# vnminin/phylomap

Measured on AMD Instinct MI355X. Metric: stochastic-map realisations/sec (branches x sites sampled/s), higher is better.
Workload: dtype f64; 1 GPU; C3: sumstatMCMC_bigtree sweep, 4-state Q, 10000-tip synthetic tree, Omega*mean(t_b)=4; n_states=4, n_tips=10000, branches=19998, replicas_total=16384, max_iters_provisioned=63, parallelism=replica-sharded x1 (weak), one RCCL all-reduce of the statistics

## Files before the change

### include/phylomap_hip.h

```cpp
#ifndef PHYLOMAP_HIP_H
#define PHYLOMAP_HIP_H

#include <stdint.h>

#ifdef __cplusplus
extern "C" {
#endif

#define PHM_VERSION 300
#define PHM_MAX_DEVICES 8

typedef enum phm_status {
  PHM_OK = 0,
  PHM_ERR_BAD_INPUT = 1,
  PHM_ERR_UNSUPPORTED = 2,
  PHM_ERR_NO_DEVICE = 3,
  PHM_ERR_OOM = 4,
  PHM_ERR_ZERO_PROB = 5,
  PHM_ERR_CAPACITY = 6,
  PHM_ERR_UNIF_CAP = 7,
  PHM_ERR_STATE = 8
} phm_status;

typedef enum phm_variant {
  PHM_MCMC = 0,
  PHM_MCMC_BIGTREE = 1,
  PHM_MCMC_SPARSE = 2,
  PHM_MCMC_KS = 3
  ,
  PHM_MCMC_BF = 4
  ,
  PHM_MCMC_MT = 5
  ,
  PHM_MCMC_KSMT = 6
} phm_variant;

typedef struct phm_tree {
  int32_t n_tips;
  int32_t n_node;
  int32_t n_edge;
  const int32_t* edge;
  const double*  edge_length;
  const int32_t* states;
  const int32_t* map_off;
  const double*  maps;
  const int32_t* mapnames;
} phm_tree;

typedef struct phm_model {
  int32_t n_states;
  const double* Q;
  const double* pid;
  const double* B;
  double Omega;
  int32_t variant;
} phm_model;

typedef enum phm_mapping { PHM_MAP_AUTO = 0, PHM_MAP_REPLICAS = 1, PHM_MAP_BRANCHES = 2, PHM_MAP_TILES = 3 } phm_mapping;

typedef struct phm_options {
  uint64_t seed;
  int32_t n_replicas;
  int32_t replica_offset;
  int32_t reduce;
  int32_t tips_per_replica;
  int32_t device;
  int32_t iters_per_launch;
  double  cap_tail;
  int32_t mapping;
  int32_t storage;
  int32_t rescale_pruning;
  int32_t no_recovery;
  int32_t sparse_chains;
  int32_t n_devices;
  int32_t devices[PHM_MAX_DEVICES];
  int32_t reserved[3];
} phm_options;

typedef struct phm_debug_options {
  int32_t pruning_form;
  int32_t phase_timing;
  int32_t fail_recovery;
  int32_t branch_group;
  int32_t level_groups;
  int32_t q_timing;
  double  pade_pivot_min;
  int32_t expect_chunk;
  int32_t reserved[3];
} phm_debug_options;

typedef struct phm_info {
  int32_t n_states, n_edge, n_replicas, n_replicas_padded, n_cols, max_iters;
  int64_t device_bytes;
  int64_t rows_per_replica;
  int64_t seg_read;
  int64_t seg_written;
  double  last_run_ms;
  int32_t last_run_launches;
  int32_t iters_done;
  int32_t recoveries;
  int32_t mapping;
  int32_t sparse_chains;
  int32_t reserved;
} phm_info;

typedef struct phm_engine phm_engine;

int32_t     phm_version(void);
int32_t     phm_struct_size(int32_t which);
int32_t     phm_device_count(void);
const char* phm_last_error(void);
const char* phm_status_string(int32_t status);
int32_t     phm_set_debug_options(const phm_debug_options* dbg);
double      phm_last_kernel_ms(void);

int32_t phm_maketreelistMCMC(
    const phm_tree* x, int32_t n_states, const double* Q, const double* pid, const double* B, double Omega,
    const int32_t* nen, const int32_t* nodelist, int32_t root, int32_t N,
    const phm_options* opt, double* out);
int32_t phm_maketreelistMCMC_bigtree(
    const phm_tree* x, int32_t n_states, const double* Q, const double* pid, const double* B, double Omega,
    const int32_t* nen, const int32_t* nodelist, int32_t root, int32_t N,
    const phm_options* opt, double* out);
int32_t phm_SPARSEmaketreelistMCMC(
    const phm_tree* x, int32_t n_states, const double* Q, const double* pid, const double* B, double Omega,
    const int32_t* nen, const int32_t* nodelist, int32_t root, int32_t N,
    const phm_options* opt, double* out);
int32_t phm_maketreelistMCMCks_sweep(
    const phm_tree* x, int32_t n_states, const double* Q, const double* pid, const double* B, double Omega,
    const int32_t* nen, const int32_t* nodelist, int32_t root, int32_t N,
    const phm_options* opt, double* out);
int32_t phm_maketreelistMCMCbf_sweep(
    const phm_tree* x, int32_t n_states, const double* Q, const double* pid, const double* B, double Omega,
    const int32_t* nen, const int32_t* nodelist, int32_t root, int32_t N,
    const phm_options* opt, double* out);
int32_t phm_maketreelistMCMCbf(
    const phm_tree* x, int32_t n_states, const double* Q, const double* pid, const double* B, double Omega,
    const int32_t* nen, const int32_t* nodelist, int32_t root, int32_t N, const double* prior, int32_t n_prior,
    const phm_options* opt, double* out);
int32_t phm_maketreelistMCMCks(
    const phm_tree* x, int32_t n_states, const double* Q, const double* pid, const double* B, double Omega,
    const int32_t* nen, const int32_t* nodelist, int32_t root, int32_t N, const double* prior, int32_t n_prior,
    const phm_options* opt, double* out);
int32_t phm_maketreelistMCMC2sDICt(
    const phm_tree* x, int32_t n_states, const double* Q, const double* pid, const double* B, double Omega,
    const int32_t* nen, const int32_t* nodelist, int32_t root, int32_t N, const double* prior, int32_t n_prior,
    const phm_options* opt, double* out);
int32_t phm_maketreelistMCMCksDICt(
    const phm_tree* x, int32_t n_states, const double* Q, const double* pid, const double* B, double Omega,
    const int32_t* nen, const int32_t* nodelist, int32_t root, int32_t N, const double* prior, int32_t n_prior,
    const phm_options* opt, double* out);
int32_t phm_maketreelistMCMCmt(
    const phm_tree* trees, int32_t n_trees, int32_t n_states, const double* Q, const double* pid, const double* B,
    double Omega, const int32_t* nen_m, const int32_t* nodelist_m, const int32_t* roots, int32_t N, const double* prior,
    int32_t n_prior, const phm_options* opt, double* out);
int32_t phm_maketreelistMCMCksmt(
    const phm_tree* trees, int32_t n_trees, int32_t n_states, const double* Q, const double* pid, const double* B,
    double Omega, const int32_t* nen_m, const int32_t* nodelist_m, const int32_t* roots, int32_t N, const double* prior,
    int32_t n_prior, const phm_options* opt, double* out);
int32_t phm_maketreelistEXP(
    const phm_tree* x, int32_t n_states, const double* Q, const double* pid,
    const int32_t* nen, const int32_t* nodelist, int32_t root, int32_t N,
    const double* lefts, const double* rights, const double* d,
    const phm_options* opt, double* out);

int32_t phm_simulate_histories(const phm_tree* x, int32_t n_states, const double* Q, const double* pid,
                               const int32_t* observe, const phm_options* opt,
                               int32_t* tips, int32_t* nodes, double* stats);

int32_t phm_simulate_histories_maps(const phm_tree* x, int32_t n_states, const double* Q, const double* pid,
                                    const int32_t* observe, const phm_options* opt,
                                    int32_t* tips, int32_t* nodes, double* stats,
                                    int64_t* map_off, int64_t map_cap, double* map_dwell, int32_t* map_state);
int32_t phm_maketreelistEXP_maps(const phm_tree* x, int32_t n, const double* Q, const double* pid, const int32_t* nen,
                                 const int32_t* nodelist, int32_t root, int32_t N, const double* lefts, const double* rights,
                                 const double* d, const phm_options* opt, double* out,
                                 int64_t* map_off, int64_t map_cap, double* map_dwell, int32_t* map_state);

int32_t phm_maketreelistMCMC_maps(int32_t variant, const phm_tree* x, int32_t n_states, const double* Q, const double* pid,
                                  const double* B, double Omega, const int32_t* nen, const int32_t* nodelist, int32_t root, int32_t N,
                                  const int32_t* map_iters, int32_t n_map_iters, const phm_options* opt, double* out,
                                  int64_t* map_off, int64_t map_cap, double* map_dwell, int32_t* map_state);

int32_t phm_expected_stats(const phm_tree* x, int32_t n_states, const double* Q, const double* pid,
                           const int32_t* observe, const phm_options* opt,
                           double* stats, double* loglik, double* branch_stats, double* node_post);

int32_t phm_expected_through_time(const phm_tree* x, int32_t n_states, const double* Q, const double* pid,
                                  const int32_t* observe, const phm_options* opt,
                                  int32_t n_bounds, const double* bounds,
                                  double* occupancy,
                                  double* bin_stats,
                                  int64_t n_points, const int32_t* point_edge, const double* point_pos,
                                  double* point_post,
                                  double* loglik);

int32_t phm_loglik_models(const phm_tree* x, int32_t n_states, int32_t n_models, const double* Q, const double* pid, int32_t n_pid,
                          const int32_t* observe, const int32_t* site_of_model, const phm_options* opt, double* out);

int32_t phm_expected_stats_models(const phm_tree* x, int32_t n_states, int32_t n_models, const double* Q, const double* pid,
                                  int32_t n_pid, const int32_t* observe, const int32_t* site_of_model, const phm_options* opt,
                                  double* stats, double* loglik);

int32_t phm_sample_histories_models(const phm_tree* x, int32_t n_states, int32_t n_models, const double* Q, const double* pid,
                                    int32_t n_pid, const int32_t* observe, const int32_t* site_of_model, int32_t draws,
                                    const phm_options* opt, double* stats, double* loglik, int32_t* nodes,
                                    int64_t* map_off, int64_t map_cap, double* map_dwell, int32_t* map_state);

int32_t phm_ancestral_models(const phm_tree* x, int32_t n_states, int32_t n_models, const double* Q, const double* pid,
                             int32_t n_pid, const int32_t* observe, const int32_t* site_of_model,
                             const int32_t* node_sel, int32_t n_sel, const phm_options* opt,
                             double* loglik, double* node_post, int32_t* joint_states, double* joint_logp);

int32_t phm_simulate_histories_models(const phm_tree* x, int32_t n_states, int32_t n_models, const double* Q, const double* pid,
                                      int32_t n_pid, const int32_t* observe, int32_t replicates, const phm_options* opt,
                                      int32_t* tips, int32_t* nodes, double* stats,
                                      int64_t* map_off, int64_t map_cap, double* map_dwell, int32_t* map_state);

int32_t phm_gibbs_rates(const phm_tree* x, int32_t n_states, const int32_t* index, int32_t n_params, int32_t n_chains,
                        const double* theta0, const double* prior, int32_t n_prior, double theta_max, const double* pid,
                        int32_t n_pid, const int32_t* observe, const int32_t* site_of_chain, int32_t iters, int32_t thin,
                        const phm_options* opt, double* theta, double* loglik, double* stats, int32_t* rejected,
                        int32_t* chain_status);

int32_t phm_qupdate_apply(int32_t variant, int32_t n_states, double* Q, double Omega, const double* prior, int32_t n_prior,
                          const double* row, uint64_t seed, uint32_t iter);

int32_t phm_sparse_kernel_source(int32_t n_states, const double* M, char* buf, int32_t cap);

int32_t phm_tree_orders(int32_t n_tips, int32_t n_edge, const int32_t* edge, int32_t* nen, int32_t* nodelist,
                        int32_t* root);

int32_t phm_expm_eigen(int32_t n_states, const double* lefts, const double* rights, const double* d,
                       const double* t, int32_t n_t, int32_t device, double* out, double* kernel_ms);
int32_t phm_expm_eigen_mfma(int32_t n_states, const double* lefts, const double* rights, const double* d,
                            const double* t, int32_t n_t, int32_t device, double* out, double* kernel_ms);
int32_t phm_expm_pade(int32_t n_states, const double* Q, const double* t, int32_t n_t, int32_t device,
                      double* out, double* kernel_ms);

int32_t phm_expm_pade_mfma(int32_t n_states, const double* Q, const double* t, int32_t n_t, int32_t device,
                           double* out, double* kernel_ms);

int32_t phm_engine_create(const phm_tree* x, const phm_model* model, const phm_options* opt,
                          int32_t max_iters, phm_engine** out);
int32_t phm_engine_create_multi(const phm_tree* trees, int32_t n_trees, const phm_model* model, const phm_options* opt,
                                int32_t max_iters, phm_engine** out);
int32_t phm_engine_run(phm_engine* e, int32_t n_iters, void* hip_stream);
int32_t phm_engine_sync(phm_engine* e);
int32_t phm_engine_read_stats(phm_engine* e, int32_t iter0, int32_t n, double* out);
int32_t phm_engine_reduced_stats_device(phm_engine* e, int32_t iter0, int32_t n, void* hip_stream, void** out_dev);
int32_t phm_engine_time_pruning(phm_engine* e, int32_t n_iters, void* hip_stream, double* ms_out);
int32_t phm_engine_set_model(phm_engine* e, const double* Q);
int32_t phm_engine_dump(phm_engine* e, int32_t replica, int32_t* seg_count, double* seg_dwell, int32_t seg_cap,
                        int32_t* node_states, double* PL);
int32_t phm_engine_info(phm_engine* e, phm_info* info);
int32_t phm_engine_phase_ms(phm_engine* e, double* out4);
void    phm_engine_destroy(phm_engine* e);

#ifdef __cplusplus
}
#endif
#endif
```

### phylomap_amd/_lib.py

```python
from __future__ import annotations

import ctypes as C
import os

import numpy as np

_HERE = os.path.dirname(os.path.abspath(__file__))
LIB_PATH = os.environ.get("PHM_LIB", os.path.join(_HERE, "libphylomap_hip.so"))

PHM_OK = 0
STATUS = {0: "PHM_OK", 1: "PHM_ERR_BAD_INPUT", 2: "PHM_ERR_UNSUPPORTED", 3: "PHM_ERR_NO_DEVICE", 4: "PHM_ERR_OOM",
          5: "PHM_ERR_ZERO_PROB", 6: "PHM_ERR_CAPACITY", 7: "PHM_ERR_UNIF_CAP", 8: "PHM_ERR_STATE"}
PHM_MCMC, PHM_MCMC_BIGTREE, PHM_MCMC_SPARSE, PHM_MCMC_KS, PHM_MCMC_BF, PHM_MCMC_MT, PHM_MCMC_KSMT = 0, 1, 2, 3, 4, 5, 6

EXPORTS = [
    "phm_version", "phm_struct_size", "phm_device_count", "phm_last_error", "phm_status_string",
    "phm_maketreelistMCMC", "phm_maketreelistMCMC_bigtree", "phm_SPARSEmaketreelistMCMC", "phm_maketreelistEXP",
    "phm_maketreelistMCMCks_sweep", "phm_maketreelistMCMCbf_sweep", "phm_maketreelistMCMCbf", "phm_maketreelistMCMCks", "phm_maketreelistMCMC2sDICt", "phm_maketreelistMCMCksDICt", "phm_engine_set_model", "phm_qupdate_apply",
    "phm_expm_eigen", "phm_expm_eigen_mfma", "phm_expm_pade", "phm_expm_pade_mfma",
    "phm_engine_create", "phm_engine_run", "phm_engine_sync", "phm_engine_read_stats", "phm_engine_dump",
    "phm_engine_info", "phm_engine_destroy", "phm_engine_reduced_stats_device",
    "phm_engine_time_pruning", "phm_tree_orders",
    "phm_engine_create_multi", "phm_maketreelistMCMCmt", "phm_maketreelistMCMCksmt", "phm_engine_phase_ms",
    "phm_last_kernel_ms", "phm_set_debug_options", "phm_sparse_kernel_source", "phm_simulate_histories",
    "phm_expected_stats", "phm_simulate_histories_maps", "phm_maketreelistEXP_maps", "phm_maketreelistMCMC_maps",
    "phm_expected_through_time", "phm_loglik_models", "phm_expected_stats_models", "phm_sample_histories_models",
    "phm_gibbs_rates", "phm_ancestral_models", "phm_simulate_histories_models",
]


class PhmError(RuntimeError):
    def __init__(self, status, message):
        super().__init__(f"{STATUS.get(status, status)}: {message}")
        self.status = status


class Tree(C.Structure):
    _fields_ = [("n_tips", C.c_int32), ("n_node", C.c_int32), ("n_edge", C.c_int32),
                ("edge", C.POINTER(C.c_int32)), ("edge_length", C.POINTER(C.c_double)),
                ("states", C.POINTER(C.c_int32)), ("map_off", C.POINTER(C.c_int32)),
                ("maps", C.POINTER(C.c_double)), ("mapnames", C.POINTER(C.c_int32))]


class Model(C.Structure):
    _fields_ = [("n_states", C.c_int32), ("Q", C.POINTER(C.c_double)), ("pid", C.POINTER(C.c_double)),
                ("B", C.POINTER(C.c_double)), ("Omega", C.c_double), ("variant", C.c_int32)]


PHM_MAX_DEVICES = 8


class Options(C.Structure):
    _fields_ = [("seed", C.c_uint64), ("n_replicas", C.c_int32), ("replica_offset", C.c_int32),
                ("reduce", C.c_int32), ("tips_per_replica", C.c_int32), ("device", C.c_int32),
                ("iters_per_launch", C.c_int32), ("cap_tail", C.c_double), ("mapping", C.c_int32), ("storage", C.c_int32),
                ("rescale_pruning", C.c_int32), ("no_recovery", C.c_int32), ("sparse_chains", C.c_int32),
                ("n_devices", C.c_int32), ("devices", C.c_int32 * PHM_MAX_DEVICES), ("reserved", C.c_int32 * 3)]


class DebugOptions(C.Structure):
    _fields_ = [("pruning_form", C.c_int32), ("phase_timing", C.c_int32), ("fail_recovery", C.c_int32),
                ("branch_group", C.c_int32), ("level_groups", C.c_int32), ("q_timing", C.c_int32),
                ("pade_pivot_min", C.c_double), ("expect_chunk", C.c_int32), ("reserved", C.c_int32 * 3)]


class Info(C.Structure):
    _fields_ = [("n_states", C.c_int32), ("n_edge", C.c_int32), ("n_replicas", C.c_int32),
                ("n_replicas_padded", C.c_int32), ("n_cols", C.c_int32), ("max_iters", C.c_int32),
                ("device_bytes", C.c_int64), ("rows_per_replica", C.c_int64), ("seg_read", C.c_int64),
                ("seg_written", C.c_int64), ("last_run_ms", C.c_double), ("last_run_launches", C.c_int32),
                ("iters_done", C.c_int32), ("recoveries", C.c_int32), ("mapping", C.c_int32), ("sparse_chains", C.c_int32),
                ("reserved", C.c_int32)]


def _p(a, t):
    return a.ctypes.data_as(C.POINTER(t)) if a is not None else None


_lib = None


def load():
    global _lib
    if _lib is None:
        if not os.path.exists(LIB_PATH):
            raise RuntimeError(f"{LIB_PATH} is missing: run `python -c 'import __graft_entry__ as g; g.build()'` "
                               "or `make`; phylomap_amd has no CPU fallback")
        L = C.CDLL(LIB_PATH)
        L.phm_last_error.restype = C.c_char_p
        L.phm_status_string.restype = C.c_char_p
        L.phm_status_string.argtypes = [C.c_int32]
        L.phm_last_kernel_ms.restype = C.c_double
        L.phm_engine_create.argtypes = [C.POINTER(Tree), C.POINTER(Model), C.POINTER(Options), C.c_int32,
                                        C.POINTER(C.c_void_p)]
        L.phm_engine_create_multi.argtypes = [C.POINTER(Tree), C.c_int32, C.POINTER(Model), C.POINTER(Options), C.c_int32,
                                              C.POINTER(C.c_void_p)]
        L.phm_engine_run.argtypes = [C.c_void_p, C.c_int32, C.c_void_p]
        L.phm_engine_sync.argtypes = [C.c_void_p]
        L.phm_engine_read_stats.argtypes = [C.c_void_p, C.c_int32, C.c_int32, C.POINTER(C.c_double)]
        L.phm_engine_dump.argtypes = [C.c_void_p, C.c_int32, C.POINTER(C.c_int32), C.POINTER(C.c_double), C.c_int32,
                                      C.POINTER(C.c_int32), C.POINTER(C.c_double)]
        L.phm_engine_info.argtypes = [C.c_void_p, C.POINTER(Info)]
        L.phm_tree_orders.argtypes = [C.c_int32, C.c_int32, C.POINTER(C.c_int32), C.POINTER(C.c_int32),
                                      C.POINTER(C.c_int32), C.POINTER(C.c_int32)]
        L.phm_engine_time_pruning.argtypes = [C.c_void_p, C.c_int32, C.c_void_p, C.POINTER(C.c_double)]
        L.phm_engine_reduced_stats_device.argtypes = [C.c_void_p, C.c_int32, C.c_int32, C.c_void_p,
                                                      C.POINTER(C.c_void_p)]
        L.phm_engine_phase_ms.argtypes = [C.c_void_p, C.POINTER(C.c_double)]
        L.phm_engine_destroy.argtypes = [C.c_void_p]
        L.phm_engine_destroy.restype = None
        mc = [C.POINTER(Tree), C.c_int32, C.POINTER(C.c_double), C.POINTER(C.c_double), C.POINTER(C.c_double),
              C.c_double, C.POINTER(C.c_int32), C.POINTER(C.c_int32), C.c_int32, C.c_int32, C.POINTER(Options),
              C.POINTER(C.c_double)]
        L.phm_maketreelistMCMC.argtypes = mc
        L.phm_maketreelistMCMC_bigtree.argtypes = mc
        L.phm_SPARSEmaketreelistMCMC.argtypes = mc
        L.phm_maketreelistMCMCks_sweep.argtypes = mc
        L.phm_maketreelistMCMCbf_sweep.argtypes = mc
        mcq = mc[:10] + [C.POINTER(C.c_double), C.c_int32] + mc[10:]
        L.phm_maketreelistMCMCbf.argtypes = mcq
        L.phm_maketreelistMCMCks.argtypes = mcq
        L.phm_maketreelistMCMC2sDICt.argtypes = mcq
        L.phm_maketreelistMCMCksDICt.argtypes = mcq
        mt = [C.POINTER(Tree), C.c_int32, C.c_int32, C.POINTER(C.c_double), C.POINTER(C.c_double), C.POINTER(C.c_double),
              C.c_double, C.POINTER(C.c_int32), C.POINTER(C.c_int32), C.POINTER(C.c_int32), C.c_int32,
              C.POINTER(C.c_double), C.c_int32, C.POINTER(Options), C.POINTER(C.c_double)]
        L.phm_maketreelistMCMCmt.argtypes = mt
        L.phm_maketreelistMCMCksmt.argtypes = mt
        L.phm_engine_set_model.argtypes = [C.c_void_p, C.POINTER(C.c_double)]
        L.phm_qupdate_apply.argtypes = [C.c_int32, C.c_int32, C.POINTER(C.c_double), C.c_double, C.POINTER(C.c_double),
                                        C.c_int32, C.POINTER(C.c_double), C.c_uint64, C.c_uint32]
        L.phm_maketreelistEXP.argtypes = [C.POINTER(Tree), C.c_int32, C.POINTER(C.c_double), C.POINTER(C.c_double),
                                          C.POINTER(C.c_int32), C.POINTER(C.c_int32), C.c_int32, C.c_int32,
                                          C.POINTER(C.c_double), C.POINTER(C.c_double), C.POINTER(C.c_double),
                                          C.POINTER(Options), C.POINTER(C.c_double)]
        L.phm_expm_eigen.argtypes = [C.c_int32, C.POINTER(C.c_double), C.POINTER(C.c_double), C.POINTER(C.c_double),
                                     C.POINTER(C.c_double), C.c_int32, C.c_int32, C.POINTER(C.c_double),
                                     C.POINTER(C.c_double)]
        L.phm_expm_eigen_mfma.argtypes = L.phm_expm_eigen.argtypes
        L.phm_expm_pade_mfma.argtypes = [C.c_int32, C.POINTER(C.c_double), C.POINTER(C.c_double), C.c_int32, C.c_int32,
                                         C.POINTER(C.c_double), C.POINTER(C.c_double)]
        L.phm_expm_pade.argtypes = [C.c_int32, C.POINTER(C.c_double), C.POINTER(C.c_double), C.c_int32, C.c_int32,
                                    C.POINTER(C.c_double), C.POINTER(C.c_double)]
        L.phm_set_debug_options.argtypes = [C.POINTER(DebugOptions)]
        L.phm_simulate_histories.argtypes = [C.POINTER(Tree), C.c_int32, C.POINTER(C.c_double), C.POINTER(C.c_double),
                                             C.POINTER(C.c_int32), C.POINTER(Options), C.POINTER(C.c_int32),
                                             C.POINTER(C.c_int32), C.POINTER(C.c_double)]
        L.phm_simulate_histories_maps.argtypes = L.phm_simulate_histories.argtypes + [
            C.POINTER(C.c_int64), C.c_int64, C.POINTER(C.c_double), C.POINTER(C.c_int32)]
        L.phm_maketreelistEXP_maps.argtypes = L.phm_maketreelistEXP.argtypes + [
            C.POINTER(C.c_int64), C.c_int64, C.POINTER(C.c_double), C.POINTER(C.c_int32)]
        L.phm_maketreelistMCMC_maps.argtypes = [C.c_int32] + mc[:10] + [C.POINTER(C.c_int32), C.c_int32] + mc[10:] + [
            C.POINTER(C.c_int64), C.c_int64, C.POINTER(C.c_double), C.POINTER(C.c_int32)]
        L.phm_expected_stats.argtypes = [C.POINTER(Tree), C.c_int32, C.POINTER(C.c_double), C.POINTER(C.c_double),
                                         C.POINTER(C.c_int32), C.POINTER(Options), C.POINTER(C.c_double),
                                         C.POINTER(C.c_double), C.POINTER(C.c_double), C.POINTER(C.c_double)]
        L.phm_expected_through_time.argtypes = [C.POINTER(Tree), C.c_int32, C.POINTER(C.c_double), C.POINTER(C.c_double),
                                                C.POINTER(C.c_int32), C.POINTER(Options), C.c_int32, C.POINTER(C.c_double),
                                                C.POINTER(C.c_double), C.POINTER(C.c_double), C.c_int64, C.POINTER(C.c_int32),
                                                C.POINTER(C.c_double), C.POINTER(C.c_double), C.POINTER(C.c_double)]
        L.phm_loglik_models.argtypes = [C.POINTER(Tree), C.c_int32, C.c_int32, C.POINTER(C.c_double), C.POINTER(C.c_double),
                                        C.c_int32, C.POINTER(C.c_int32), C.POINTER(C.c_int32), C.POINTER(Options),
                                        C.POINTER(C.c_double)]
        L.phm_expected_stats_models.argtypes = [C.POINTER(Tree), C.c_int32, C.c_int32, C.POINTER(C.c_double),
                                                C.POINTER(C.c_double), C.c_int32, C.POINTER(C.c_int32), C.POINTER(C.c_int32),
                                                C.POINTER(Options), C.POINTER(C.c_double), C.POINTER(C.c_double)]
        L.phm_sample_histories_models.argtypes = [C.POINTER(Tree), C.c_int32, C.c_int32, C.POINTER(C.c_double),
                                                  C.POINTER(C.c_double), C.c_int32, C.POINTER(C.c_int32), C.POINTER(C.c_int32),
                                                  C.c_int32, C.POINTER(Options), C.POINTER(C.c_double), C.POINTER(C.c_double),
                                                  C.POINTER(C.c_int32), C.POINTER(C.c_int64), C.c_int64, C.POINTER(C.c_double),
                                                  C.POINTER(C.c_int32)]
        L.phm_gibbs_rates.argtypes = [C.POINTER(Tree), C.c_int32, C.POINTER(C.c_int32), C.c_int32, C.c_int32,
                                      C.POINTER(C.c_double), C.POINTER(C.c_double), C.c_int32, C.c_double, C.POINTER(C.c_double),
                                      C.c_int32, C.POINTER(C.c_int32), C.POINTER(C.c_int32), C.c_int32, C.c_int32,
                                      C.POINTER(Options), C.POINTER(C.c_double), C.POINTER(C.c_double), C.POINTER(C.c_double),
                                      C.POINTER(C.c_int32), C.POINTER(C.c_int32)]
        L.phm_ancestral_models.argtypes = [C.POINTER(Tree), C.c_int32, C.c_int32, C.POINTER(C.c_double), C.POINTER(C.c_double),
                                           C.c_int32, C.POINTER(C.c_int32), C.POINTER(C.c_int32), C.POINTER(C.c_int32), C.c_int32,
                                           C.POINTER(Options), C.POINTER(C.c_double), C.POINTER(C.c_double),
                                           C.POINTER(C.c_int32), C.POINTER(C.c_double)]
        L.phm_simulate_histories_models.argtypes = [C.POINTER(Tree), C.c_int32, C.c_int32, C.POINTER(C.c_double),
                                                    C.POINTER(C.c_double), C.c_int32, C.POINTER(C.c_int32), C.c_int32,
                                                    C.POINTER(Options), C.POINTER(C.c_int32), C.POINTER(C.c_int32),
                                                    C.POINTER(C.c_double), C.POINTER(C.c_int64), C.c_int64,
                                                    C.POINTER(C.c_double), C.POINTER(C.c_int32)]
        L.phm_sparse_kernel_source.argtypes = [C.c_int32, C.POINTER(C.c_double), C.c_char_p, C.c_int32]
        for which, mirror in enumerate((Options, Info, Tree, Model, DebugOptions)):
            if L.phm_struct_size(which) != C.sizeof(mirror):
                raise RuntimeError(f"{LIB_PATH}: {mirror.__name__} is {L.phm_struct_size(which)} bytes in the library, "
                                   f"{C.sizeof(mirror)} in phylomap_amd/_lib.py (stale build? run make)")
        _lib = L
    return _lib


def check(status):
    if status != PHM_OK:
        raise PhmError(status, load().phm_last_error().decode())


class FlatTree:

    def __init__(self, z, states=None):
        edge = np.asarray(z["edge"], dtype=np.int32)
        if edge.ndim != 2 or edge.shape[1] != 2:
            raise ValueError("z['edge'] must be E x 2")
        self.E = edge.shape[0]
        st = z["states"] if states is None else states
        self.states = np.ascontiguousarray(np.asarray(st).round(), dtype=np.int32)
        self.T = int(np.asarray(z["states"]).shape[-1])
        self.edge = np.asfortranarray(edge).reshape(-1, order="F").copy()
        el = z.get("edge.length")
        self.edge_length = None if el is None else np.ascontiguousarray(el, dtype=np.float64)
        lens = [len(m) for m in z["maps"]]
        self.map_off = np.concatenate([[0], np.cumsum(lens)]).astype(np.int32)
        self.maps = np.ascontiguousarray(np.concatenate([np.asarray(m, dtype=np.float64) for m in z["maps"]]))
        self.mapnames = np.ascontiguousarray(np.concatenate([np.asarray(m) for m in z["mapnames"]]), dtype=np.int32)
        self.c = Tree(self.T, int(z["Nnode"]), self.E, _p(self.edge, C.c_int32), _p(self.edge_length, C.c_double),
                      _p(self.states.reshape(-1), C.c_int32), _p(self.map_off, C.c_int32), _p(self.maps, C.c_double),
                      _p(self.mapnames, C.c_int32))


class FlatTreeList:

    def __init__(self, treelist):
        if len(treelist) < 1:
            raise ValueError("treelist is empty")
        self.trees = [FlatTree(z) for z in treelist]
        self.n = len(self.trees)
        self.c = (Tree * self.n)(*[t.c for t in self.trees])
        self.E, self.T = self.trees[0].E, self.trees[0].T


def tree_orders(z):
    edge = np.asarray(z["edge"], dtype=np.int32)
    E = edge.shape[0]
    flat = np.asfortranarray(edge).reshape(-1, order="F").copy()
    T = int(z["Nnode"]) + 1
    nen = np.zeros(E, dtype=np.int32)
    nodelist = np.zeros(max(int(z["Nnode"]) - 1, 1), dtype=np.int32)
    root = C.c_int32(0)
    check(load().phm_tree_orders(T, E, _p(flat, C.c_int32), _p(nen, C.c_int32), _p(nodelist, C.c_int32), C.byref(root)))
    return nen, nodelist[: int(z["Nnode"]) - 1], int(root.value)


def sparse_kernel_source(M):
    Mf = np.asfortranarray(np.asarray(M, dtype=np.float64))
    L = load()
    need = L.phm_sparse_kernel_source(Mf.shape[0], _p(Mf, C.c_double), None, 0)
    if need < 0:
        check(1)
    buf = C.create_string_buffer(need)
    L.phm_sparse_kernel_source(Mf.shape[0], _p(Mf, C.c_double), buf, need)
    return buf.value.decode()


MAPPING = {"auto": 0, "replicas": 1, "branches": 2, "tiles": 3}


def set_debug_options(**kw):
    d = DebugOptions()
    for k, v in kw.items():
        setattr(d, k, float(v) if k == "pade_pivot_min" else int(v))
    check(load().phm_set_debug_options(C.byref(d)))


_DEBUG_KEYS = ("pruning_form", "phase_timing", "fail_recovery", "branch_group", "level_groups", "q_timing", "pade_pivot_min",
               "expect_chunk")


def make_options(seed=0, n_replicas=1, replica_offset=0, reduce=False, tips_per_replica=False, device=-1,
                 iters_per_launch=0, cap_tail=0.0, storage=0, mapping="auto", rescale=False, recover=True,
                 sparse_chains=0, devices=None, **debug):
    unknown = set(debug) - set(_DEBUG_KEYS)
    if unknown:
        raise TypeError(f"unknown option(s) {sorted(unknown)}")
    set_debug_options(**debug)
    o = Options()
    o.seed = int(seed) & 0xFFFFFFFFFFFFFFFF
    o.n_replicas, o.replica_offset, o.reduce = int(n_replicas), int(replica_offset), int(bool(reduce))
    o.storage = int(storage)
    o.mapping = MAPPING[mapping] if isinstance(mapping, str) else int(mapping)
    o.rescale_pruning = int(bool(rescale))
    o.no_recovery = 0 if recover else 1
    o.sparse_chains = int(sparse_chains)
    o.tips_per_replica, o.device, o.iters_per_launch, o.cap_tail = int(bool(tips_per_replica)), int(device), int(iters_per_launch), float(cap_tail)
    if devices is not None:
        devs = list(range(int(devices))) if np.isscalar(devices) else [int(d) for d in devices]
        if len(devs) > PHM_MAX_DEVICES:
            raise ValueError(f"at most {PHM_MAX_DEVICES} devices")
        o.n_devices = len(devs)
        for i, d in enumerate(devs):
            o.devices[i] = d
    return o


class Engine:

    def __init__(self, z, Q, pid, Omega, max_iters, variant=PHM_MCMC, B=None, states=None, **opt):
        L = load()
        self.Q = np.asfortranarray(np.asarray(Q, dtype=np.float64))
        self.n = self.Q.shape[0]
        self.pid = np.ascontiguousarray(pid, dtype=np.float64)
        self.B = None if B is None else np.asfortranarray(np.asarray(B, dtype=np.float64))
        self.opt = make_options(**opt)
        self.model = Model(self.n, _p(self.Q, C.c_double), _p(self.pid, C.c_double), _p(self.B, C.c_double),
                           float(Omega), int(variant))
        self.h = C.c_void_p()
        n_trees = 1
        if isinstance(z, (list, tuple)):
            if states is not None:
                raise ValueError("a list of trees carries its own tip states")
            self.ft = FlatTreeList(z)
            n_trees = self.ft.n
            check(L.phm_engine_create_multi(self.ft.c, n_trees, C.byref(self.model), C.byref(self.opt), int(max_iters),
                                            C.byref(self.h)))
        else:
            self.ft = FlatTree(z, states)
            check(L.phm_engine_create(C.byref(self.ft.c), C.byref(self.model), C.byref(self.opt), int(max_iters),
                                      C.byref(self.h)))
        self.cols = self.n + self.n * (self.n - 1)
        if int(variant) in (PHM_MCMC_KS, PHM_MCMC_KSMT):
            self.cols = self.n + self.n * self.n + 2 + 3 * (self.n // 2 - 1) + 1
        if int(variant) in (PHM_MCMC_BF, PHM_MCMC_MT):
            self.cols = self.n + self.n * self.n + 3
        self.S = max(1, int(self.opt.n_replicas)) * n_trees
        self.reduce = bool(self.opt.reduce)

    def run(self, n_iters, stream=None):
        check(load().phm_engine_run(self.h, int(n_iters), C.c_void_p(stream) if stream else None))

    def set_model(self, Q):
        Qc = np.asfortranarray(np.asarray(Q, dtype=np.float64))
        check(load().phm_engine_set_model(self.h, _p(Qc, C.c_double)))

    def sync(self):
        check(load().phm_engine_sync(self.h))

    def info(self):
        i = Info()
        check(load().phm_engine_info(self.h, C.byref(i)))
        return i

    def stats(self, iter0, n):
        if self.reduce:
            out = np.zeros((n, self.cols), order="F")
            check(load().phm_engine_read_stats(self.h, int(iter0), int(n), _p(out, C.c_double)))
            return out
        buf = np.zeros((self.S, self.cols, n))
        check(load().phm_engine_read_stats(self.h, int(iter0), int(n), _p(buf, C.c_double)))
        return buf.transpose(0, 2, 1)

    def reduced_stats_device(self, iter0, n, stream=None):
        ptr = C.c_void_p()
        check(load().phm_engine_reduced_stats_device(self.h, int(iter0), int(n), C.c_void_p(stream) if stream else None,
                                                     C.byref(ptr)))
        return ptr.value

    def phase_ms(self):
        out = (C.c_double * 4)()
        check(load().phm_engine_phase_ms(self.h, out))
        return [float(v) for v in out]

    def time_pruning(self, n_iters, stream=None):
        ms = C.c_double(0.0)
        check(load().phm_engine_time_pruning(self.h, int(n_iters), C.c_void_p(stream) if stream else None, C.byref(ms)))
        return ms.value

    def dump(self, replica=0, seg_cap=512):
        E, T, n = self.ft.E, self.ft.T, self.n
        seg_count = np.zeros(E, dtype=np.int32)
        seg_dwell = np.zeros((E, seg_cap))
        node_states = np.zeros(2 * T - 1, dtype=np.int32)
        PL = np.zeros((2 * T - 1, n))
        check(load().phm_engine_dump(self.h, int(replica), _p(seg_count, C.c_int32), _p(seg_dwell, C.c_double),
                                     int(seg_cap), _p(node_states, C.c_int32), _p(PL, C.c_double)))
        return {"seg_count": seg_count, "seg_dwell": seg_dwell, "node_states": node_states, "PL": PL}

    def close(self):
        if self.h:
            load().phm_engine_destroy(self.h)
            self.h = C.c_void_p()

    def __del__(self):
        try:
            self.close()
        except Exception:
            pass
```

### phylomap_amd/csrc/phm_engine.cpp

```cpp
#include "phm_internal.h"

namespace {

int tree_levels(const phm::Schedule& s) {
  std::vector<int32_t> depth(s.n_node, 0);
  int levels = 1;
  for (const phm::DownStep& d : s.down)
    if (d.child >= 0) { depth[d.child] = depth[d.parent] + 1; levels = std::max(levels, depth[d.child] + 1); }
  return levels;
}
bool deep_tree(const phm::Schedule& s) {
  int lg2 = 0;
  while ((1 << lg2) < s.n_node + 1) ++lg2;
  return tree_levels(s) > 4 * lg2 + 32;
}

inline int narrow_auto_max_replicas(const phm::Schedule& s) {
  const int levels = tree_levels(s);
  const double E = (double)s.n_edge;
  const double cap = (0.0048 * levels + 6e-6 * E - 0.01) / (6.5e-7 * E);
  return (int)std::max(8.0, std::min(4096.0, cap));
}
constexpr int TILES_AUTO_MAX_REPLICAS = 262144;
inline int wbranch_auto_max_replicas(const phm::Schedule& s) {
// ... 223 lines not shown
        for (int t = 0; t < nt; ++t) th.emplace_back(rows_of, (int)((int64_t)ktab * t / nt), (int)((int64_t)ktab * (t + 1) / nt));
        for (std::thread& t : th) t.join();
      }
      HIPCHK(hipMemcpy(e->d_wt_totL.p, blk.data(), sizeof(double) * blk.size(), hipMemcpyHostToDevice));
    }
    {
      const bool ks = ks_layout(e->variant);
      std::vector<int16_t> pair_slot((size_t)n * n, (int16_t)-1);
      std::vector<int32_t> slot_col;
      for (int a = 0; a < n; ++a)
        for (int c = 0; c < n; ++c)
          if ((ks || a != c) && e->hB2[(size_t)a * n + c] != 0.0) {
            pair_slot[(size_t)a * n + c] = (int16_t)slot_col.size();
            slot_col.push_back(ks ? a * n + c : a * (n - 1) + (c > a ? c - 1 : c));
          }
      int n_slots = (int)slot_col.size();
      if (n > 32 || n_slots > phm::WT_MAX_SLOTS) { n_slots = 0; std::fill(pair_slot.begin(), pair_slot.end(), (int16_t)-1); }
      slot_col.resize(phm::WT_MAX_SLOTS, 0);
      e->pwt.n_slots = n_slots;
      HIPCHK(hipMemcpy(e->d_wt_pair_slot.p, pair_slot.data(), sizeof(int16_t) * pair_slot.size(), hipMemcpyHostToDevice));
      HIPCHK(hipMemcpy(e->d_wt_slot_col.p, slot_col.data(), sizeof(int32_t) * slot_col.size(), hipMemcpyHostToDevice));
    }
    HIPCHK(hipMemcpy(e->d_Bc.p, e->hBc.data(), sizeof(double) * n * n, hipMemcpyHostToDevice));
    HIPCHK(hipMemcpy(e->d_scale.p, e->hscale.data(), sizeof(double) * n, hipMemcpyHostToDevice));
    {
      auto half_bandwidth = [&](const std::vector<double>& M) {
        int hb = 0;
        for (int i = 0; i < n; ++i)
          for (int j = 0; j < n; ++j) if (M[(size_t)i * n + j] != 0.0) hb = std::max(hb, std::abs(i - j));
        return hb;
      };
      auto usable = [&](int hb) { return e->sparse_req != 2 && n <= phm::WT_BAND_NMAX && hb >= 1 && hb <= phm::WT_BAND_MAX && 2 * hb + 1 < n; };
      const int hbc = half_bandwidth(e->hBc), hb2 = half_bandwidth(e->hB2);
      e->pwt.band_up = usable(hbc) ? hbc : 0;
      e->pwt.band_draw = usable(hb2) ? hb2 : 0;
      e->wt_sparse.kernel = nullptr;
      if (!e->pwt.band_up && e->sparse_req != 2 && n <= phm::RTC_SPARSE_NMAX) {
        std::vector<int32_t> rp(1, 0), cj;
        std::vector<double> cv;
        for (int i = 0; i < n; ++i) {
          for (int j = 0; j < n; ++j) if (e->hBc[(size_t)i * n + j] != 0.0) { cj.push_back(j); cv.push_back(e->hBc[(size_t)i * n + j]); }
          rp.push_back((int32_t)cj.size());
        }
        if ((double)cj.size() <= phm::RTC_SPARSE_MAX_FILL * n * n) {
          std::string rerr;
          const phm::SparseUpKernel* k = phm::rtc_sparse_up_kernel(n, rp, cj, rerr);
          if (!k && e->sparse_req == 1) return fail(PHM_ERR_UNSUPPORTED, "sparse_chains = 1: " + rerr);
          if (k) {
            if (!e->d_wt_coef.p) HIPCHK(e->d_wt_coef.alloc(sizeof(double) * (size_t)n * n));
            HIPCHK(hipMemcpy(e->d_wt_coef.p, cv.data(), sizeof(double) * cv.size(), hipMemcpyHostToDevice));
            phm::RtcUpParams& r = e->wt_sparse.params;
            const phm::WtParams& w = e->pwt;
            r.n_states = n; r.ldt = w.ldt; r.n_tips = w.n_tips; r.n_node = w.n_node; r.n_edge = w.n_edge; r.n_tiles = w.n_tiles;
            r.normalise = w.normalise; r.tips_per_replica = w.tips_per_replica; r.tip_masks = w.tip_masks; r.klong = w.klong;
            r.up = reinterpret_cast<const phm::RtcUpStep*>(w.up); r.up_order = w.up_order; r.colL = w.colL; r.maskL = w.maskL; r.tips = w.tips;
            r.mcount = w.mcount; r.PL = w.PL; r.err = w.err; r.coef = e->d_wt_coef.as<double>();
            e->wt_sparse.kernel = k;
          }
        }
      }
      if (e->sparse_req == 1 && !e->pwt.band_up && !e->wt_sparse.kernel)
        return fail(PHM_ERR_UNSUPPORTED, "sparse_chains = 1: the sparse pruning kernels take n <= 32 states and a chain matrix that is banded (half-bandwidth <= 2) or at most half full");
      std::memset(&e->wt_band, 0, sizeof e->wt_band);
      if (e->pwt.band_up) {
        const int hb = e->pwt.band_up, w = 2 * hb + 1;
        for (int i = 0; i < n; ++i)
          for (int d = 0; d < w; ++d) { const int j = i + d - hb; if (j >= 0 && j < n) e->wt_band.c[i * w + d] = e->hBc[(size_t)i * n + j]; }
      }
      std::vector<double> b2band((size_t)n * (2 * phm::WT_BAND_MAX + 1), 0.0);
      if (e->pwt.band_draw) {
        const int hb = e->pwt.band_draw, w = 2 * hb + 1;
        for (int i = 0; i < n; ++i)
          for (int d = 0; d < w; ++d) { const int j = i + d - hb; if (j >= 0 && j < n) b2band[(size_t)i * w + d] = e->hB2[(size_t)i * n + j]; }
      }
      HIPCHK(hipMemcpy(e->d_wt_B2band.p, b2band.data(), sizeof(double) * b2band.size(), hipMemcpyHostToDevice));
    }
    return PHM_OK;
  }
  if (replicas) {
    HIPCHK(hipMemcpy(e->d_col.p, col.data(), sizeof(double) * col.size(), hipMemcpyHostToDevice));
    HIPCHK(hipMemcpy(e->d_row.p, row.data(), sizeof(double) * row.size(), hipMemcpyHostToDevice));
    HIPCHK(hipMemcpy(e->d_mask.p, maskpow.data(), sizeof(double) * maskpow.size(), hipMemcpyHostToDevice));
  } else {
    const size_t nc = col.size(), nr = row.size(), nm = maskpow.size();
    HIPCHK(e->pin_up.reserve(sizeof(double) * (nc + nr + nm)));
    double* stage = e->pin_up.as<double>();
    std::memcpy(stage, col.data(), sizeof(double) * nc);
    std::memcpy(stage + nc, row.data(), sizeof(double) * nr);
    std::memcpy(stage + nc + nr, maskpow.data(), sizeof(double) * nm);
    if (e->mapping == PHM_MAP_BRANCHES && !e->wide()) {
      HIPCHK(hipMemcpyAsync(e->d_nw_colL.p, stage, sizeof(double) * (nc + nr + nm), hipMemcpyHostToDevice, e->last_stream));
    } else {
      HIPCHK(hipMemcpyAsync(e->d_nw_colL.p, stage, sizeof(double) * nc, hipMemcpyHostToDevice, e->last_stream));
      HIPCHK(hipMemcpyAsync(e->d_nw_rowL.p, stage + nc, sizeof(double) * nr, hipMemcpyHostToDevice, e->last_stream));
      HIPCHK(hipMemcpyAsync(e->d_nw_maskL.p, stage + nc + nr, sizeof(double) * nm, hipMemcpyHostToDevice, e->last_stream));
    }
    HIPCHK(wait_stream(e->last_stream));
  }
  if (e->wide()) {
    HIPCHK(hipMemcpy(e->d_B2.p, e->hB2.data(), sizeof(double) * n * n, hipMemcpyHostToDevice));
    HIPCHK(hipMemcpy(e->d_Bc.p, e->hBc.data(), sizeof(double) * n * n, hipMemcpyHostToDevice));
    HIPCHK(hipMemcpy(e->d_scale.p, e->hscale.data(), sizeof(double) * n, hipMemcpyHostToDevice));
  }
  if (e->wide() && !replicas) {
    auto ellpack = [&](const std::vector<double>& M, DevBuf& dcol, DevBuf& dval, int32_t& w_out) -> int32_t {
      int w = 0;
      for (int i = 0; i < n; ++i) {
        int cnt = 0;
        for (int j = 0; j < n; ++j) cnt += M[(size_t)i * n + j] != 0.0;
        w = std::max(w, cnt);
      }
      w_out = (w >= 1 && w <= phm::WB_ELL_MAX && 3 * w <= n) ? w : 0;
      if (!w_out) return PHM_OK;
      std::vector<int32_t> ec((size_t)n * w);
      std::vector<double> ev((size_t)n * w, 0.0);
      for (int i = 0; i < n; ++i) {
        int t = 0;
        for (int j = 0; j < n; ++j) if (M[(size_t)i * n + j] != 0.0) { ec[(size_t)i * w + t] = j; ev[(size_t)i * w + t] = M[(size_t)i * n + j]; ++t; }
        for (; t < w; ++t) ec[(size_t)i * w + t] = i;
      }
      HIPCHK(hipMemcpy(dcol.p, ec.data(), sizeof(int32_t) * ec.size(), hipMemcpyHostToDevice));
      HIPCHK(hipMemcpy(dval.p, ev.data(), sizeof(double) * ev.size(), hipMemcpyHostToDevice));
      return PHM_OK;
    };
    { int32_t st = ellpack(e->hBc, e->d_ell_col, e->d_ell_val, e->pwb.ell_w); if (st) return st; }
    {
      int hb = 0;
      for (int i = 0; i < n; ++i)
        for (int j = 0; j < n; ++j) if (e->hBc[(size_t)i * n + j] != 0.0) hb = std::max(hb, std::abs(i - j));
      e->pwb.band_hb = (e->pwb.ell_w > 0 && hb >= 1 && hb <= 2 && e->sparse_req != 2) ? hb : 0;
    }
    { int32_t st = ellpack(e->hB2, e->d_ell2_col, e->d_ell2_val, e->pwb.ell2_w); if (st) return st; }
  }
  auto refresh = [&](auto& p) {
    for (int i = 0; i < n * n; ++i) { p.B2[i] = e->hB2[i]; p.Bc[i] = e->hBc[i]; }
    for (int i = 0; i < n; ++i) { p.scale[i] = e->hscale[i]; p.pid[i] = e->hpid[i]; }
  };
  small_n(e, [&](auto& sp) { refresh(sp.rep); refresh(sp.br); refresh(sp.tl); });
  return PHM_OK;
}

template <int NS>
void fill_narrow_params(phm_engine* e, phm::NarrowParams<NS>& p, const phm_options& o) {
  fill_common(e, o, p);
  p.klong = e->nw_klong; p.n_wide = e->nw_n_wide; p.cluster_async = e->nw_cluster_async;
  p.total_cap = e->nw_total_cap;
  p.cl_nodes = e->d_nw_cl_nodes.as<phm::ClusterNode>(); p.cl_item_off = e->d_nw_cl_item_off.as<int32_t>();
  p.cl_lvl_ptr = e->d_nw_cl_lvl_ptr.as<int32_t>(); p.cl_lvl_off = e->d_nw_cl_lvl_off.as<int32_t>();
  p.down_lv = e->d_nw_down_lv.as<phm::DownStep>(); p.walk_off = e->d_nw_walk_off.as<int32_t>();
  p.edge_parent = e->d_nw_edge_parent.as<int32_t>(); p.dmap_edge = e->d_nw_dmap_edge.as<uint16_t>();
  p.branch_order = e->d_nw_border.as<int32_t>(); p.off = e->d_nw_off.as<int64_t>();
  {
    const size_t tab = (size_t)e->nw_klong * NS * NS;
    p.colL = e->d_nw_colL.as<double>(); p.rowL = p.colL + tab; p.maskL = p.colL + 2 * tab;
  }
  p.tips = e->d_tips.as<uint8_t>();
  p.mcount = e->d_nw_mcount.as<int32_t>(); p.dw[0] = e->d_nw_dwA.as<double>(); p.dw[1] = e->d_nw_dwB.as<double>();
  p.PL = e->d_PL.as<double>(); p.nstate = e->d_nstate.as<uint8_t>(); p.part = e->d_nw_part.as<double>();
  p.rowbuf = e->d_nw_rowbuf.as<double>();
  p.dmap = e->d_nw_dmap.as<uint16_t>();
  p.host_row = nullptr;
  if (e->S == 1 && !e->reduce && e->pin_row.reserve(sizeof(double) * (e->dcols + 2)) == hipSuccess) {
    void* dp = nullptr;
    if (hipHostGetDevicePointer(&dp, e->pin_row.p, 0) == hipSuccess) p.host_row = reinterpret_cast<double*>(dp);
  }
}

int32_t build_level_orders(phm_engine* e) {
  const phm::Schedule& s = e->sched;
  const int E = s.n_edge;
  std::vector<int32_t> up_order, down_order, node_order;
  phm::height_levels(s.up, up_order, e->nw_up_off);
  phm::depth_levels(s, down_order, e->nw_down_off);
  phm::node_depth_levels(s, node_order, e->nw_node_off);
  HIPCHK(upload(e->d_nw_up_order, up_order)); HIPCHK(upload(e->d_nw_down_order, down_order)); HIPCHK(upload(e->d_nw_node_order, node_order));
  if (!e->wide()) {
    std::vector<int32_t> walk;
    phm::depth_levels(s, walk, e->nw_walk_off, true);
    std::vector<phm::DownStep> walk_lv;
    walk_lv.reserve(E);
    for (int k : walk) walk_lv.push_back(s.down[k]);
    for (int k : down_order) if (s.down[k].child < 0) walk_lv.push_back(s.down[k]);
    std::vector<int32_t> edge_parent(E);
    for (int i = 0; i < E; ++i) edge_parent[s.down[i].edge] = s.down[i].parent;
    HIPCHK(upload(e->d_nw_down_lv, walk_lv));
    HIPCHK(upload(e->d_nw_walk_off, e->nw_walk_off));
    HIPCHK(upload(e->d_nw_edge_parent, edge_parent));
  }
  HIPCHK(upload(e->d_nw_up_off, e->nw_up_off)); HIPCHK(upload(e->d_nw_down_off, e->nw_down_off));
  return PHM_OK;
}

int32_t narrow_setup(phm_engine* e, const phm_tree* x, const phm_model* model, const phm_options& o, int32_t max_iters) {
  const phm::Schedule& s = e->sched;
  const int E = s.n_edge, T = s.n_tips, Nn = s.n_node, n = e->n, S = e->S;
  const SlotPlan sp = plan_slots(e, x, model->Omega, o, max_iters);
  e->nw_off = sp.off;
  int n_wide = 0;
  for (int b = 0; b < E; ++b)
    if (expected_segments(x, b, model->Omega) >= phm::NARROW_WIDE_SEGMENTS) ++n_wide;
  e->nw_n_wide = std::max(n_wide, std::min(E / 16, phm::NARROW_LONG));
  e->nw_cluster_async = e->dbg.pruning_form == 2 || (e->dbg.pruning_form == 0 && n_wide > 0);

  if (e->tips_per_replica) {
    e->tips_host.resize((size_t)S * T);
    for (int r = 0; r < S; ++r) for (int t = 0; t < T; ++t) e->tips_host[(size_t)r * T + t] = (uint8_t)(x->states[(size_t)r * T + t] - 1);
  } else {
    single_tree_tips(e, x);
  }

  const size_t dw_bytes = sizeof(double) * (size_t)S * e->nw_total_cap;
  const size_t tab = (size_t)e->nw_klong * n * n;
  size_t free_b = 0, total_b = 0;
  HIPCHK(hipMemGetInfo(&free_b, &total_b));
  const size_t part_cols = e->wide() ? (size_t)n + 1 : (size_t)n + n * n + 1;
  const size_t n_dw = e->wide() ? 3 : 2;
  const size_t dmap_bytes = e->wide() ? (((size_t)S * E * n <= (256u << 20)) ? (size_t)S * E * n : 0) : 2 * sizeof(uint16_t) * (size_t)S * E;
  const size_t small_bytes = (size_t)S * (E * (sizeof(int32_t) + 2) + (size_t)Nn * (sizeof(double) * n + 1)) + sizeof(phm::ClusterNode) * (size_t)Nn + 16 * (size_t)E;
  const size_t need = n_dw * dw_bytes + (e->wide() ? (size_t)S * e->nw_total_cap : 0) + stats_bytes(e) + dmap_bytes + small_bytes +
                      sizeof(double) * (3 * tab + (size_t)S * E * part_cols + (e->wide() ? 2 * (size_t)S * e->dcols : 0));
  if (int32_t st = check_hbm(need, free_b)) return st;
  HIPCHK(upload(e->d_up, s.up)); HIPCHK(upload(e->d_down, s.down));
  if (int32_t st = build_level_orders(e)) return st;
  HIPCHK(upload(e->d_nw_border, sp.order)); HIPCHK(upload(e->d_nw_off, e->nw_off));
  if (e->wide()) {
    HIPCHK(e->d_nw_colL.alloc(sizeof(double) * tab)); HIPCHK(e->d_nw_rowL.alloc(sizeof(double) * tab));
    HIPCHK(e->d_nw_maskL.alloc(sizeof(double) * (size_t)e->nw_klong * 2 * n));
  } else {
    HIPCHK(e->d_nw_colL.alloc(sizeof(double) * (2 * tab + (size_t)e->nw_klong * 2 * n)));
  }
  HIPCHK(upload(e->d_tips, e->tips_host));
  HIPCHK(e->d_nw_mcount.alloc(sizeof(int32_t) * (size_t)S * E));
  HIPCHK(e->d_nw_dwA.alloc(dw_bytes)); HIPCHK(e->d_nw_dwB.alloc(dw_bytes));
  if (e->wide()) {
    HIPCHK(e->d_nw_mstate.alloc((size_t)S * e->nw_total_cap));
    HIPCHK(e->d_nw_mlen.alloc(dw_bytes));
    HIPCHK(e->d_nw_estate.alloc((size_t)S * E * 2));
  }
  HIPCHK(e->d_PL.alloc(sizeof(double) * (size_t)S * Nn * n));
  HIPCHK(e->d_nstate.alloc((size_t)S * Nn));
  HIPCHK(e->d_nw_part.alloc(sizeof(double) * (size_t)S * E * part_cols));
  HIPCHK(e->d_nw_rowbuf.alloc(sizeof(double) * (size_t)S * e->dcols));
  if (!e->wide()) {
    HIPCHK(e->d_nw_dmap.alloc(sizeof(uint16_t) * (size_t)S * E));
    HIPCHK(e->d_nw_dmap_edge.alloc(sizeof(uint16_t) * (size_t)S * E));
    phm::ClusterPlan plan;
    phm::build_cluster_plan(s, phm::NARROW_CLUSTER_NODES, plan);
    if (int32_t st = upload_cluster_plan(e, plan, true)) return st;
  }
  if (int32_t st = alloc_stats(e)) return st;
  e->bytes = (int64_t)(n_dw * dw_bytes + e->d_nw_mstate.bytes + e->d_nw_part.bytes + e->d_PL.bytes + e->d_stats.bytes + e->d_red.bytes +
                       sizeof(double) * 3 * tab + e->d_nw_mcount.bytes + e->d_nw_dmap.bytes + e->d_nw_dmap_edge.bytes + e->d_nw_cl_nodes.bytes +
                       (e->wide() ? dmap_bytes : 0));
  HIPCHK(hipMemset(e->d_nstate.p, 0, e->d_nstate.bytes));
  {
    std::vector<double> init((size_t)e->nw_total_cap, 0.0);
    std::vector<int32_t> m0(E);
    for (int b = 0; b < E; ++b) {
      m0[b] = x->map_off[b + 1] - x->map_off[b];
      std::memcpy(&init[(size_t)e->nw_off[b]], x->maps + x->map_off[b], sizeof(double) * m0[b]);
    }
    for (int r = 0; r < S; ++r) {
      HIPCHK(hipMemcpy(e->d_nw_dwA.as<double>() + (size_t)r * e->nw_total_cap, init.data(), sizeof(double) * init.size(), hipMemcpyHostToDevice));
      HIPCHK(hipMemcpy(e->d_nw_mcount.as<int32_t>() + (size_t)r * E, m0.data(), sizeof(int32_t) * E, hipMemcpyHostToDevice));
    }
  }
  small_n(e, [&](auto& p) { fill_narrow_params(e, p.br, o); });
  if (e->wide()) {
    HIPCHK(e->d_wb_cnt.alloc(sizeof(double) * (size_t)S * e->dcols));
    if ((size_t)S * s.n_edge * n <= (256u << 20)) HIPCHK(e->d_nw_dmap.alloc((size_t)S * s.n_edge * n));
    HIPCHK(hipMemset(e->d_wb_cnt.p, 0, e->d_wb_cnt.bytes));
    HIPCHK(e->d_B2.alloc(sizeof(double) * n * n)); HIPCHK(e->d_Bc.alloc(sizeof(double) * n * n));
    HIPCHK(e->d_ell_col.alloc(sizeof(int32_t) * n * phm::WB_ELL_MAX)); HIPCHK(e->d_ell_val.alloc(sizeof(double) * n * phm::WB_ELL_MAX));
    HIPCHK(e->d_ell2_col.alloc(sizeof(int32_t) * n * phm::WB_ELL_MAX)); HIPCHK(e->d_ell2_val.alloc(sizeof(double) * n * phm::WB_ELL_MAX));
    HIPCHK(e->d_scale.alloc(sizeof(double) * n)); HIPCHK(upload(e->d_pid, e->hpid));
    phm::WideBranchParams& p = e->pwb;
    fill_common(e, o, p);
    p.n_states = n; p.sparse = (e->variant == PHM_MCMC_SPARSE); p.count_self = p.ks; p.klong = e->nw_klong;
    p.total_cap = e->nw_total_cap;
    p.B2 = e->d_B2.as<double>(); p.Bc = e->d_Bc.as<double>(); p.scale = e->d_scale.as<double>(); p.pid = e->d_pid.as<double>();
    p.ell_w = 0; p.band_hb = 0; p.ell_col = e->d_ell_col.as<int32_t>(); p.ell_val = e->d_ell_val.as<double>();
    p.ell2_w = 0; p.ell2_col = e->d_ell2_col.as<int32_t>(); p.ell2_val = e->d_ell2_val.as<double>();
    p.up = e->d_up.as<phm::UpStep>(); p.down = e->d_down.as<phm::DownStep>();
    p.up_order = e->d_nw_up_order.as<int32_t>(); p.down_order = e->d_nw_down_order.as<int32_t>();
    p.up_off = e->d_nw_up_off.as<int32_t>(); p.down_off = e->d_nw_down_off.as<int32_t>();
    p.branch_order = e->d_nw_border.as<int32_t>(); p.off = e->d_nw_off.as<int64_t>();
    p.colL = e->d_nw_colL.as<double>(); p.rowL = e->d_nw_rowL.as<double>(); p.maskL = e->d_nw_maskL.as<double>();
    p.tips = e->d_tips.as<uint8_t>(); p.mcount = e->d_nw_mcount.as<int32_t>();
    p.dw[0] = e->d_nw_dwA.as<double>(); p.dw[1] = e->d_nw_dwB.as<double>(); p.mlen = e->d_nw_mlen.as<double>();
    p.mstate = e->d_nw_mstate.as<uint8_t>(); p.estate = e->d_nw_estate.as<uint8_t>();
    p.PL = e->d_PL.as<double>(); p.nstate = e->d_nstate.as<uint8_t>(); p.part = e->d_nw_part.as<double>();
    p.cnt = e->d_wb_cnt.as<double>(); p.rowbuf = e->d_nw_rowbuf.as<double>();
    p.dmap = e->d_nw_dmap.as<uint8_t>();
  }
  return PHM_OK;
}

inline int tiles_cnt_copies(int tiles) {
  int c = 1;
  while (c < 64 && c * tiles < 512) c *= 2;
  return c;
}

template <int NS>
void fill_tile_params(phm_engine* e, phm::TileParams<NS>& p, const phm_options& o) {
  fill_common(e, o, p);
  p.klong = e->nw_klong;
  p.group = (int32_t)std::max<int64_t>(1, std::min<int64_t>(16, (int64_t)e->tiles * p.n_edge / 65536));
  p.n_groups = (p.n_edge + p.group - 1) / p.group;
  p.n_chunks = (p.n_groups + phm::TILES_CHUNK - 1) / phm::TILES_CHUNK;
  p.rows = e->nw_total_cap;
  p.up = e->d_up.as<phm::UpStep>();
  p.up_order = e->d_nw_up_order.as<int32_t>(); p.node_order = e->d_nw_node_order.as<int32_t>();
  p.branch_order = e->d_nw_border.as<int32_t>(); p.slot = e->d_tl_slot.as<int32_t>();
  p.cl_nodes = e->d_nw_cl_nodes.as<phm::ClusterNode>();
  p.cl_lvl_ptr = e->d_nw_cl_lvl_ptr.as<int32_t>(); p.cl_lvl_off = e->d_nw_cl_lvl_off.as<int32_t>();
  p.colL = e->d_nw_colL.as<double>(); p.rowL = e->d_nw_rowL.as<double>(); p.maskL = e->d_nw_maskL.as<double>();
  p.tips = e->d_tips.as<uint8_t>(); p.mcount = e->d_mcount.as<uint16_t>();
  p.dw[0] = e->d_dw0.as<double>(); p.dw[1] = e->d_dw1.as<double>();
  p.estate = e->d_tl_estate.as<uint8_t>(); p.PL = e->d_PL.as<double>(); p.nstate = e->d_nstate.as<uint8_t>();
  p.mstate = e->d_wt_mstate.p ? e->d_wt_mstate.as<uint8_t>() : nullptr;
  p.pdw = e->d_tl_pdw.as<double>(); p.pchunk = e->d_tl_pchunk.as<double>(); p.cnt = e->d_tl_cnt.as<uint32_t>();
  p.cnt_copies = tiles_cnt_copies(e->tiles);
  p.pseg = e->d_tl_pseg.as<uint32_t>(); p.segprev = e->d_tl_segprev.as<uint32_t>();
}

int32_t tile_slots(phm_engine* e, const SlotPlan& sp) {
  const int E = e->sched.n_edge;
  e->tl_slot.assign(E + 1, 0);
  for (int b = 0; b < E; ++b) {
    if (sp.cap[b] >= (1 << 23)) return fail(PHM_ERR_UNSUPPORTED, "branch too long: a slot of the (tile, branch) mapping exceeds 4 GB");
    if (sp.off[b + 1] > 0x7fffff00ll / 64) return fail(PHM_ERR_UNSUPPORTED, "tree too large: dwell rows per replica tile exceed 32-bit indexing");
    e->tl_slot[b + 1] = (int32_t)sp.off[b + 1];
  }
  return PHM_OK;
}

int32_t tiles_setup(phm_engine* e, const phm_tree* x, const phm_model* model, const phm_options& o, int32_t max_iters) {
  const phm::Schedule& s = e->sched;
  const int E = s.n_edge, Nn = s.n_node, n = e->n, tiles = e->tiles;
  const SlotPlan sp = plan_slots(e, x, model->Omega, o, max_iters);
  if (int32_t st = tile_slots(e, sp)) return st;
  const int64_t rows = e->rows;
  single_tree_tips(e, x);

  const int n_chunks = (E + phm::TILES_CHUNK - 1) / phm::TILES_CHUNK;
  const size_t dw_bytes = sizeof(double) * (size_t)tiles * rows * 64;
  const size_t tab = (size_t)e->nw_klong * n * n;
  const size_t pdw_bytes = sizeof(double) * (size_t)tiles * E * n * 64;
  const size_t pl_bytes = sizeof(double) * (size_t)tiles * Nn * n * 64;
#ifndef PHM_TILES_LONG_SEGMENTS
#define PHM_TILES_LONG_SEGMENTS 48.0
#endif
  const bool long_paths = sp.max_seg > PHM_TILES_LONG_SEGMENTS;
  const size_t ms_bytes = long_paths ? (size_t)tiles * rows * 64 : 0;
  size_t free_b = 0, total_b = 0;
  HIPCHK(hipMemGetInfo(&free_b, &total_b));
  const size_t need = 2 * dw_bytes + ms_bytes + pdw_bytes + pl_bytes + stats_bytes(e) + sizeof(double) * 3 * tab + (size_t)tiles * (4 * (size_t)E + Nn) * 64;
  if (int32_t st = check_hbm(need, free_b)) return st;
  HIPCHK(upload(e->d_up, s.up)); HIPCHK(upload(e->d_down, s.down));
  if (int32_t st = build_level_orders(e)) return st;
  HIPCHK(upload(e->d_nw_border, sp.order)); HIPCHK(upload(e->d_tl_slot, e->tl_slot));
  HIPCHK(e->d_nw_colL.alloc(sizeof(double) * tab)); HIPCHK(e->d_nw_rowL.alloc(sizeof(double) * tab));
  HIPCHK(e->d_nw_maskL.alloc(sizeof(double) * (size_t)e->nw_klong * 2 * n));
  HIPCHK(upload(e->d_tips, e->tips_host));
  HIPCHK(e->d_mcount.alloc(sizeof(uint16_t) * (size_t)tiles * E * 64));
  HIPCHK(e->d_dw0.alloc(dw_bytes)); HIPCHK(e->d_dw1.alloc(dw_bytes));
  if (long_paths) HIPCHK(e->d_wt_mstate.alloc(ms_bytes));
  HIPCHK(e->d_tl_estate.alloc((size_t)tiles * E * 64));
  HIPCHK(e->d_PL.alloc(pl_bytes));
  HIPCHK(e->d_nstate.alloc((size_t)tiles * Nn * 64));
  HIPCHK(e->d_tl_pdw.alloc(pdw_bytes));
  HIPCHK(e->d_tl_pchunk.alloc(sizeof(double) * (size_t)tiles * n_chunks * n * 64));
  HIPCHK(e->d_tl_cnt.alloc(sizeof(uint32_t) * (size_t)tiles * tiles_cnt_copies(tiles) * n * n * 64));
  HIPCHK(e->d_tl_pseg.alloc(sizeof(uint32_t) * (size_t)tiles * n_chunks * 64)); HIPCHK(e->d_tl_segprev.alloc(sizeof(uint32_t) * tiles));
  if (int32_t st = alloc_stats(e)) return st;
  e->bytes = (int64_t)(2 * dw_bytes + ms_bytes + pdw_bytes + pl_bytes + e->d_stats.bytes + e->d_red.bytes + e->d_mcount.bytes + e->d_tl_pchunk.bytes +
                       sizeof(double) * 3 * tab);
  HIPCHK(hipMemset(e->d_nstate.p, 0, e->d_nstate.bytes));
  HIPCHK(hipMemset(e->d_tl_cnt.p, 0, e->d_tl_cnt.bytes));
  if (int32_t st = init_tile_paths(e, x)) return st;
  {
    std::vector<uint32_t> segprev(tiles);
    for (int t = 0; t < tiles; ++t) segprev[t] = (uint32_t)((int64_t)x->map_off[E] * std::min(64, e->S - t * 64));
    HIPCHK(hipMemcpy(e->d_tl_segprev.p, segprev.data(), e->d_tl_segprev.bytes, hipMemcpyHostToDevice));
  }
  e->nw_tier_off.clear();
  const bool deep = deep_tree(s);
  if (e->dbg.level_groups >= 2 || (e->dbg.level_groups == 0 && (deep || (int64_t)tiles * Nn <= phm::TILES_CL_MAX_WORK))) {
    phm::ClusterPlan plan;
    if (e->dbg.level_groups == 3 || (e->dbg.level_groups == 0 && deep)) phm::build_cluster_plan(s, phm::TILES_CL_NODES, plan);
    else phm::build_band_plan(s, TILES_CL_BAND, plan);
    if (int32_t st = upload_cluster_plan(e, plan, false)) return st;
  }
  small_n(e, [&](auto& p) { fill_tile_params(e, p.tl, o); });
  return PHM_OK;
}

int32_t wtiles_setup(phm_engine* e, const phm_tree* x, const phm_model* model, const phm_options& o, int32_t max_iters) {
  const phm::Schedule& s = e->sched;
  const int E = s.n_edge, Nn = s.n_node, n = e->n, tiles = e->tiles;
  const SlotPlan sp = plan_slots(e, x, model->Omega, o, max_iters);
  if (int32_t st = tile_slots(e, sp)) return st;
  const int64_t rows = e->rows;
  single_tree_tips(e, x);

  const int ldt = (n + 1) & ~1;
  if ((uint64_t)e->nw_klong * n * ldt * sizeof(double) >= (1ull << 32))
    return fail(PHM_ERR_UNSUPPORTED, "branch too long for the lane-per-replica mapping: a chain table would exceed 4 GB");
  const size_t dw_bytes = sizeof(double) * (size_t)tiles * rows * 64;
  const size_t tab = (size_t)e->nw_klong * n * ldt;
  const size_t pl_bytes = sizeof(double) * (size_t)tiles * Nn * n * 64;
  const size_t cnt_bytes = sizeof(uint32_t) * (size_t)tiles * n * n * 64;
  size_t free_b = 0, total_b = 0;
  HIPCHK(hipMemGetInfo(&free_b, &total_b));
  const int nblk = (n + 7) / 8, ldb = (nblk + 1) & ~1;
  const size_t tot_bytes = sizeof(double) * (size_t)e->nw_klong * n * n * ldb;
  const size_t acc_bytes = sizeof(unsigned long long) * (size_t)tiles * (n + 1) * 64;
  const size_t red_bytes = e->reduce ? sizeof(double) * (size_t)max_iters * e->dcols : 0;
  const size_t need = 2 * dw_bytes + dw_bytes / 8 + pl_bytes + cnt_bytes + stats_bytes(e) + tot_bytes + acc_bytes + red_bytes + sizeof(double) * 3 * tab +
                      (size_t)tiles * (5 * (size_t)E + Nn + 8 * (size_t)n) * 64;
  if (int32_t st = check_hbm(need, free_b)) return st;
  HIPCHK(upload(e->d_up, s.up)); HIPCHK(upload(e->d_down, s.down));
  if (int32_t st = build_level_orders(e)) return st;
  e->nw_tier_off.clear();
  if (n <= 32 && (e->dbg.level_groups >= 2 || (e->dbg.level_groups == 0 && deep_tree(s)))) {
    phm::ClusterPlan plan;
    phm::build_cluster_plan(s, phm::TILES_CL_NODES, plan);
    if (int32_t st = upload_cluster_plan(e, plan, false)) return st;
  }
  HIPCHK(upload(e->d_nw_border, sp.order)); HIPCHK(upload(e->d_tl_slot, e->tl_slot));
  HIPCHK(e->d_nw_colL.alloc(sizeof(double) * tab)); HIPCHK(e->d_nw_rowL.alloc(sizeof(double) * tab));
  HIPCHK(e->d_nw_maskL.alloc(sizeof(double) * (size_t)e->nw_klong * 2 * ldt));
  HIPCHK(e->d_wt_B2.alloc(sizeof(double) * (size_t)n * ldt)); HIPCHK(e->d_Bc.alloc(sizeof(double) * n * n));
  HIPCHK(e->d_wt_B2band.alloc(sizeof(double) * (size_t)n * (2 * phm::WT_BAND_MAX + 1)));
  HIPCHK(e->d_wt_totL.alloc(tot_bytes));
  HIPCHK(e->d_wt_pair_slot.alloc(sizeof(int16_t) * (size_t)n * n)); HIPCHK(e->d_wt_slot_col.alloc(sizeof(int32_t) * phm::WT_MAX_SLOTS));
  HIPCHK(e->d_scale.alloc(sizeof(double) * n)); HIPCHK(upload(e->d_pid, e->hpid));
  HIPCHK(upload(e->d_tips, e->tips_host));
  HIPCHK(e->d_mcount.alloc(sizeof(uint16_t) * (size_t)tiles * E * 64));
  HIPCHK(e->d_dw0.alloc(dw_bytes)); HIPCHK(e->d_dw1.alloc(dw_bytes));
  HIPCHK(e->d_tl_estate.alloc(sizeof(uint16_t) * (size_t)tiles * E * 64));
  HIPCHK(e->d_wt_mstate.alloc((size_t)tiles * rows * 64));
  HIPCHK(e->d_PL.alloc(pl_bytes));
  HIPCHK(e->d_nstate.alloc((size_t)tiles * Nn * 64));
  HIPCHK(e->d_tl_cnt.alloc(cnt_bytes));
  HIPCHK(e->d_wt_dwfx.alloc(sizeof(unsigned long long) * (size_t)tiles * n * 64));
  HIPCHK(e->d_wt_segacc.alloc(sizeof(unsigned long long) * (size_t)tiles * 64));
  if (e->reduce) {
    HIPCHK(e->d_wt_dwfx_tile.alloc(sizeof(unsigned long long) * (size_t)tiles * n * 16));
    HIPCHK(e->d_wt_cnt_tile.alloc(sizeof(uint32_t) * (size_t)tiles * n * n));
    HIPCHK(hipMemset(e->d_wt_dwfx_tile.p, 0, e->d_wt_dwfx_tile.bytes));
    HIPCHK(hipMemset(e->d_wt_cnt_tile.p, 0, e->d_wt_cnt_tile.bytes));
  }
  if (int32_t st = alloc_stats(e)) return st;
  e->bytes = (int64_t)(2 * dw_bytes + e->d_wt_mstate.bytes + pl_bytes + cnt_bytes + e->d_stats.bytes + e->d_red.bytes + e->d_mcount.bytes + e->d_tl_estate.bytes +
                       e->d_nstate.bytes + e->d_wt_dwfx.bytes + e->d_wt_segacc.bytes + e->d_wt_totL.bytes + sizeof(double) * 3 * tab);
  HIPCHK(hipMemset(e->d_nstate.p, 0, e->d_nstate.bytes));
  HIPCHK(hipMemset(e->d_tl_cnt.p, 0, e->d_tl_cnt.bytes));
  HIPCHK(hipMemset(e->d_wt_dwfx.p, 0, e->d_wt_dwfx.bytes));
  HIPCHK(hipMemset(e->d_wt_segacc.p, 0, e->d_wt_segacc.bytes));
  if (int32_t st = init_tile_paths(e, x)) return st;
  phm::WtParams& p = e->pwt;
  fill_common(e, o, p);
  p.n_states = n; p.ldt = ldt;
  p.klong = e->nw_klong;
  p.group = (int32_t)std::max<int64_t>(1, std::min<int64_t>(8, (int64_t)tiles * E / 65536));
  if (e->dbg.branch_group > 0) p.group = std::min(64, (int)e->dbg.branch_group);
  p.n_groups = (E + p.group - 1) / p.group;
  p.up_form = e->dbg.pruning_form & 3; p.band_up = 0; p.band_draw = 0; p.B2band = e->d_wt_B2band.as<double>();
  p.cl_nodes = e->nw_tier_off.empty() ? nullptr : e->d_nw_cl_nodes.as<phm::ClusterNode>();
  p.cl_lvl_ptr = e->d_nw_cl_lvl_ptr.as<int32_t>(); p.cl_lvl_off = e->d_nw_cl_lvl_off.as<int32_t>();
  e->sparse_req = o.sparse_chains;
  p.rows = rows;
  {
    int ex = 0;
    (void)std::frexp(std::max(sp.tree_len, 1.0), &ex);
    p.fx_scale = std::ldexp(1.0, 60 - ex); p.fx_inv = std::ldexp(1.0, ex - 60);
  }
  p.B2 = e->d_wt_B2.as<double>(); p.Bc = e->d_Bc.as<double>(); p.scale = e->d_scale.as<double>(); p.pid = e->d_pid.as<double>();
  p.up = e->d_up.as<phm::UpStep>(); p.down = e->d_down.as<phm::DownStep>();
  p.up_order = e->d_nw_up_order.as<int32_t>(); p.down_order = e->d_nw_down_order.as<int32_t>();
  p.branch_order = e->d_nw_border.as<int32_t>(); p.slot = e->d_tl_slot.as<int32_t>();
  p.colL = e->d_nw_colL.as<double>(); p.rowL = e->d_nw_rowL.as<double>(); p.maskL = e->d_nw_maskL.as<double>();
  p.blkL = e->d_wt_totL.as<double>(); p.nblk = nblk; p.ldb = ldb;
  p.n_slots = 0; p.pair_slot = e->d_wt_pair_slot.as<int16_t>(); p.slot_col = e->d_wt_slot_col.as<int32_t>();
  p.tips = e->d_tips.as<uint8_t>(); p.mcount = e->d_mcount.as<uint16_t>();
  p.dw[0] = e->d_dw0.as<double>(); p.dw[1] = e->d_dw1.as<double>();
  p.estate = e->d_tl_estate.as<uint16_t>(); p.PL = e->d_PL.as<double>(); p.nstate = e->d_nstate.as<uint8_t>();
  p.mstate = e->d_wt_mstate.as<uint8_t>();
  p.dwfx = e->d_wt_dwfx.as<unsigned long long>(); p.cnt = e->d_tl_cnt.as<uint32_t>();
  p.segacc = e->d_wt_segacc.as<unsigned long long>();
  p.dwfx_tile = e->reduce ? e->d_wt_dwfx_tile.as<unsigned long long>() : nullptr;
  p.cnt_tile = e->reduce ? e->d_wt_cnt_tile.as<uint32_t>() : nullptr;
  return PHM_OK;
}

int32_t replicas_setup(phm_engine* e, const phm_tree* trees, const phm_model* model, const phm_options& o) {
  const phm::Schedule& s = e->sched;
  const phm_tree* x = trees;
  const int E = s.n_edge, T = s.n_tips, n = e->n, n_trees = e->n_trees, max_iters = e->max_iters;
  int64_t rows = 0;
  std::vector<std::vector<int32_t>> init_row(n_trees, std::vector<int32_t>(E));
  std::vector<int64_t> init_rows(n_trees, 0);
  for (int j = 0; j < n_trees; ++j) {
    const phm_tree* xt = &trees[j];
    int64_t rows_j = 0, max_q = 0;
    double sum_lambda = 0.0;
    for (int k = 0; k < E; ++k) {
      const phm::DownStep& d = e->scheds[j].down[k];
      double tb = 0.0;
      for (int i = xt->map_off[d.edge]; i < xt->map_off[d.edge + 1]; ++i) tb += xt->maps[i];
      int m0 = xt->map_off[d.edge + 1] - xt->map_off[d.edge];
      if (e->wide() && m0 > phm::wide_maxseg(n))
        return fail(PHM_ERR_UNSUPPORTED, "the replica mapping for 5..64 states holds at most " + std::to_string(phm::wide_maxseg(n)) +
                                         " segments per branch (a path of " + std::to_string(m0) + " was given); use PHM_MAP_TILES or PHM_MAP_BRANCHES (the automatic choice for one tree)");
      init_row[j][k] = (int32_t)init_rows[j];
      init_rows[j] += m0;
      int q = phm::poisson_capacity(model->Omega * tb, o.cap_tail > 0.0 ? o.cap_tail : 1e-3);
      rows_j += (int64_t)std::max(q, m0 + q - 1) * e->cap_boost;
      max_q = std::max<int64_t>(max_q, (int64_t)std::max(q, m0 + q - 1) * e->cap_boost);
      sum_lambda += model->Omega * tb;
    }
    rows_j = std::max(rows_j, init_rows[j]) + max_q + (int64_t)(6.0 * 0.7 * std::sqrt(sum_lambda)) + 64;
    rows = std::max(rows, rows_j);
  }
  if (rows * 64 > 0x7fffff00ll) return fail(PHM_ERR_UNSUPPORTED, "tree too large: dwell rows per replica tile exceed 32-bit indexing");
  e->rows = rows;

  if (e->wide() && n_trees == 1) {
    size_t free_now = 0, total_now = 0;
    HIPCHK(hipMemGetInfo(&free_now, &total_now));
    int rpt = 64;
    while (rpt > 1 && (e->S + rpt / 2 - 1) / (rpt / 2) <= 8192) rpt /= 2;
    auto tile_bytes = [&](int r) {
      const size_t tl = (size_t)(e->S + r - 1) / r;
      return tl * (sizeof(double) * ((size_t)rows * 64 + (size_t)s.n_node * n * 64) + 3 * (size_t)E * 64) +
             sizeof(double) * (size_t)max_iters * e->dcols * (e->reduce ? tl : tl * 64);
    };
    while (rpt < 64 && tile_bytes(rpt) > free_now / 4) rpt *= 2;
    e->rpt = rpt;
    e->tiles = (e->S + rpt - 1) / rpt; e->S_pad = e->tiles * 64; e->tpt = e->tiles;
  }

  if (n_trees > 1) {
    e->tips_host.assign((size_t)e->tiles * T * 64, 0);
    for (int tl = 0; tl < e->tiles; ++tl)
      for (int t = 0; t < T; ++t)
        std::memset(&e->tips_host[((size_t)tl * T + t) * 64], trees[tl / e->tpt].states[t] - 1, 64);
  } else {
    single_tree_tips(e, x);
  }

  if (!e->wide() && ((uint64_t)rows * 512u >= (1ull << 32) || (uint64_t)s.n_node * n * 512u >= (1ull << 32) ||
                   (uint64_t)s.n_edge * 128u >= (1ull << 32)))
    return fail(PHM_ERR_UNSUPPORTED, "tree too large for the replica layout (a tile's dwell stream or PL rows exceed 4 GB); use mapping=tiles");

  e->nw_klong = e->wide() ? phm::wide_maxseg(n) + 1 : (int)std::min<int64_t>(65536, rows + 1);
  const size_t ktab = std::max(e->nw_klong, e->wide() ? phm::WIDE_KTAB : phm::MCMC_KTAB);

  const size_t dw_bytes = sizeof(double) * (size_t)e->tiles * rows * 64;
  size_t free_b = 0, total_b = 0;
  HIPCHK(hipMemGetInfo(&free_b, &total_b));
  e->ring = e->wide() || n_trees > 1 || o.storage == 1 || (o.storage != 2 && 2 * dw_bytes > free_b / 3);
  size_t need = (e->ring ? 1 : 2) * dw_bytes + stats_bytes(e) + sizeof(double) * (size_t)e->tiles * s.n_node * n * 64 +
                (size_t)e->tiles * (s.n_node + 2 * (size_t)E) * 64 + e->tips_host.size();
  if (int32_t st = check_hbm(need, free_b)) return st;
  HIPCHK(e->d_up.alloc(sizeof(phm::UpStep) * s.up.size() * n_trees));
  HIPCHK(e->d_down.alloc(sizeof(phm::DownStep) * s.down.size() * n_trees));
  HIPCHK(e->d_roots.alloc(sizeof(int32_t) * n_trees));
  HIPCHK(e->d_col.alloc(sizeof(double) * ktab * n * n));
  HIPCHK(e->d_row.alloc(sizeof(double) * ktab * n * n));
  HIPCHK(e->d_mask.alloc(sizeof(double) * ktab * 2 * n));

  HIPCHK(upload(e->d_tips, e->tips_host));
  HIPCHK(e->d_mcount.alloc(sizeof(uint16_t) * (size_t)e->tiles * E * 64));
  HIPCHK(e->d_dw0.alloc(dw_bytes));
  HIPCHK(e->d_cursor.alloc(sizeof(int32_t) * 2 * e->tiles));
  if (!e->ring) HIPCHK(e->d_dw1.alloc(dw_bytes));
  HIPCHK(e->d_PL.alloc(sizeof(double) * (size_t)e->tiles * s.n_node * n * 64));
  HIPCHK(e->d_nstate.alloc((size_t)e->tiles * s.n_node * 64));
  if (int32_t st = alloc_stats(e)) return st;
  e->bytes = (int64_t)(e->d_up.bytes + e->d_down.bytes + e->d_col.bytes + e->d_row.bytes + e->d_tips.bytes + e->d_mcount.bytes +
                       e->d_dw0.bytes + e->d_dw1.bytes + e->d_cursor.bytes + e->d_PL.bytes + e->d_nstate.bytes + e->d_stats.bytes + e->d_red.bytes);

  for (int j = 0; j < n_trees; ++j) {
    const phm::Schedule& sj = e->scheds[j];
    HIPCHK(hipMemcpy(e->d_up.as<phm::UpStep>() + (size_t)j * sj.up.size(), sj.up.data(), sizeof(phm::UpStep) * sj.up.size(), hipMemcpyHostToDevice));
    HIPCHK(hipMemcpy(e->d_down.as<phm::DownStep>() + (size_t)j * sj.down.size(), sj.down.data(), sizeof(phm::DownStep) * sj.down.size(), hipMemcpyHostToDevice));
    HIPCHK(hipMemcpy(e->d_roots.as<int32_t>() + j, &sj.root, sizeof(int32_t), hipMemcpyHostToDevice));
  }
  HIPCHK(hipMemset(e->d_nstate.p, 0, e->d_nstate.bytes));

  {
    std::vector<int32_t> cur(2 * (size_t)e->tiles);
    for (int j = 0; j < n_trees; ++j) {
      const phm_tree* xt = &trees[j];
      DevBuf d_off, d_maps, d_irow;
      HIPCHK(upload(d_irow, init_row[j]));
      HIPCHK(upload(d_off, xt->map_off, E + 1)); HIPCHK(upload(d_maps, xt->maps, xt->map_off[E]));
      const size_t tile0 = (size_t)j * e->tpt;
      HIPCHK(phm::launch_mcmc_init(E, e->tpt, rows, e->d_down.as<phm::DownStep>() + (size_t)j * E, d_irow.as<int32_t>(), d_off.as<int32_t>(),
                                   d_maps.as<double>(), e->d_dw0.as<double>() + tile0 * rows * 64, e->d_mcount.as<uint16_t>() + tile0 * E * 64, nullptr));
      HIPCHK(hipDeviceSynchronize());
      for (int t = 0; t < e->tpt; ++t) { cur[2 * (tile0 + t)] = 0; cur[2 * (tile0 + t) + 1] = e->ring ? (int32_t)(init_rows[j] % rows) : 0; }
    }
    HIPCHK(hipMemcpy(e->d_cursor.p, cur.data(), e->d_cursor.bytes, hipMemcpyHostToDevice));
  }

  if (e->wide()) {
    HIPCHK(upload(e->d_B2, e->hB2)); HIPCHK(upload(e->d_Bc, e->hBc));
    HIPCHK(upload(e->d_scale, e->hscale)); HIPCHK(upload(e->d_pid, e->hpid));
    phm::WideParams& p = e->pw;
    fill_common(e, o, p);
    p.n_rep = n_trees > 1 ? e->S_tree : e->S;
    p.tiles_per_tree = n_trees > 1 ? e->tpt : 0; p.roots = e->d_roots.as<int32_t>(); p.rep_stride = e->rpt;
    p.n_states = n; p.ktab = std::max(e->nw_klong, phm::WIDE_KTAB); p.sparse = (e->variant == PHM_MCMC_SPARSE); p.count_self = p.ks;
    p.maskpow = e->d_mask.as<double>();
    p.rows = e->rows;
    p.B2 = e->d_B2.as<double>(); p.Bc = e->d_Bc.as<double>(); p.scale = e->d_scale.as<double>(); p.pid = e->d_pid.as<double>();
    p.up = e->d_up.as<phm::UpStep>(); p.down = e->d_down.as<phm::DownStep>();
    p.colpow = e->d_col.as<double>(); p.rowpow = e->d_row.as<double>();
    p.tips = e->d_tips.as<uint8_t>(); p.mcount = e->d_mcount.as<uint16_t>();
    p.dwell0 = e->d_dw0.as<double>(); p.cursor = e->d_cursor.as<int32_t>();
    p.PL = e->d_PL.as<double>(); p.nstate = e->d_nstate.as<uint8_t>();
  }
  small_n(e, [&](auto& p) { fill_params(e, p.rep, o); });
  return PHM_OK;
}

phm_engine* live(phm_engine* e) {
  while (e && e->fwd) e = e->fwd;
  return e;
}
inline int32_t dead_engine() { return fail(PHM_ERR_CAPACITY, "the engine outgrew its dwell capacity and could not be rebuilt; destroy it and create a new one (larger cap_tail margin, fewer replicas)"); }

std::shared_ptr<SavedInput> save_input(const phm_tree* trees, int32_t n_trees, const phm_model* model, const phm_options& o, int32_t max_iters) {
  auto sv = std::make_shared<SavedInput>();
  const int n = model->n_states;
  sv->trees.resize(n_trees);
  sv->flat.resize(n_trees);
  for (int j = 0; j < n_trees; ++j) {
    const phm_tree& x = trees[j];
    SavedInput::TreeCopy& c = sv->trees[j];
    const size_t E = (size_t)x.n_edge, nt = (size_t)x.n_tips * (o.tips_per_replica ? std::max(1, o.n_replicas) : 1);
    c.edge.assign(x.edge, x.edge + 2 * E);
    c.states.assign(x.states, x.states + nt);
    c.map_off.assign(x.map_off, x.map_off + E + 1);
    c.maps.assign(x.maps, x.maps + x.map_off[E]);
    c.mapnames.assign(x.mapnames, x.mapnames + x.map_off[E]);
    if (x.edge_length) c.edge_length.assign(x.edge_length, x.edge_length + E);
    c.t = x;
    c.t.edge = c.edge.data(); c.t.states = c.states.data(); c.t.map_off = c.map_off.data(); c.t.maps = c.maps.data();
    c.t.mapnames = c.mapnames.data(); c.t.edge_length = x.edge_length ? c.edge_length.data() : nullptr;
    sv->flat[j] = c.t;
  }
  sv->Q.assign(model->Q, model->Q + (size_t)n * n);
  sv->pid.assign(model->pid, model->pid + n);
  if (model->B) sv->B.assign(model->B, model->B + (size_t)n * n);
  sv->model = *model;
  sv->model.Q = sv->Q.data(); sv->model.pid = sv->pid.data(); sv->model.B = model->B ? sv->B.data() : nullptr;
  sv->opt = o;
  sv->max_iters = max_iters;
  return sv;
}

}

extern "C" {

int32_t phm_version(void) { return PHM_VERSION; }

int32_t phm_struct_size(int32_t which) {
  switch (which) {
    case 0: return (int32_t)sizeof(phm_options);
    case 1: return (int32_t)sizeof(phm_info);
    case 2: return (int32_t)sizeof(phm_tree);
    case 3: return (int32_t)sizeof(phm_model);
    case 4: return (int32_t)sizeof(phm_debug_options);
    default: return -1;
  }
}

int32_t phm_set_debug_options(const phm_debug_options* dbg) {
  if (dbg) g_phm_debug = *dbg; else g_phm_debug = phm_debug_options{};
  return PHM_OK;
}

int32_t phm_device_count(void) {
  int n = 0;
  if (hipGetDeviceCount(&n) != hipSuccess) return 0;
  return n;
}

const char* phm_last_error(void) { return g_phm_err.c_str(); }

const char* phm_status_string(int32_t s) {
  switch (s) {
    case PHM_OK: return "ok";
    case PHM_ERR_BAD_INPUT: return "bad input";
    case PHM_ERR_UNSUPPORTED: return "unsupported";
    case PHM_ERR_NO_DEVICE: return "no HIP device / HIP failure";
    case PHM_ERR_OOM: return "out of device memory";
    case PHM_ERR_ZERO_PROB: return "zero probability vector";
    case PHM_ERR_CAPACITY: return "branch capacity exceeded";
    case PHM_ERR_UNIF_CAP: return "uniformisation jump cap exceeded";
    case PHM_ERR_STATE: return "invalid engine state";
    default: return "unknown";
  }
}

int32_t phm_engine_create(const phm_tree* x, const phm_model* model, const phm_options* opt_in, int32_t max_iters,
                          phm_engine** out) {
  return phm_engine_create_multi(x, 1, model, opt_in, max_iters, out);
}

int32_t phm_engine_create_multi(const phm_tree* trees, int32_t n_trees, const phm_model* model, const phm_options* opt_in,
                                int32_t max_iters, phm_engine** out) {
  return phm_engine_create_impl(trees, n_trees, model, opt_in, g_phm_debug, 0, max_iters, out);
}

}

int32_t phm_engine_create_impl(const phm_tree* trees, int32_t n_trees, const phm_model* model, const phm_options* opt_in,
                               const phm_debug_options& dbg, int boost_log2, int32_t max_iters, phm_engine** out) {
  if (!out) return fail(PHM_ERR_BAD_INPUT, "out is NULL");
  *out = nullptr;
  if (!trees || !model) return fail(PHM_ERR_BAD_INPUT, "tree/model is NULL");
  if (n_trees < 1) return fail(PHM_ERR_BAD_INPUT, "n_trees must be >= 1");
  const phm_tree* x = trees;
  phm_options o = resolve_options(opt_in);
  if (o.n_replicas <= 0) o.n_replicas = 1;
  const int n = model->n_states;
  if (n < 2) return fail(PHM_ERR_BAD_INPUT, "n_states must be >= 2");
  if (n > 64) return fail(PHM_ERR_UNSUPPORTED, "this build has MCMC kernels for n_states <= 64 only");
  if (!model->Q || !model->pid) return fail(PHM_ERR_BAD_INPUT, "model: Q/pid missing");
  if (model->variant < PHM_MCMC || model->variant > PHM_MCMC_KSMT) return fail(PHM_ERR_BAD_INPUT, "unknown variant");
  if (hidden_rates(model->variant) && (n & 1)) return fail(PHM_ERR_BAD_INPUT, "sumstatMCMCks needs a hidden-rates Q of even size n = 2k+2 (src/phylomap.cpp:1820)");
  if (model->variant == PHM_MCMC_MT && n != 2) return fail(PHM_ERR_BAD_INPUT, "sumstatMCMCmt is a two-state model (hard-wired columns, src/phylomap.cpp:2169-2173)");
  if (n_trees > 1 && (o.reduce || o.tips_per_replica)) return fail(PHM_ERR_UNSUPPORTED, "a list of trees takes neither reduce nor tips_per_replica");
  if (max_iters < 1) return fail(PHM_ERR_BAD_INPUT, "max_iters must be >= 1");
  if (!(model->Omega > 0.0) || !std::isfinite(model->Omega)) return fail(PHM_ERR_BAD_INPUT, "Omega must be positive");
  int32_t st = PHM_OK;
  for (int j = 0; j < n_trees; ++j) {
    if (trees[j].n_tips != x->n_tips || trees[j].n_edge != x->n_edge || trees[j].n_node != x->n_node)
      return fail(PHM_ERR_BAD_INPUT, "every tree of the list must have the same number of tips and edges (src/phylomap.cpp:2275-2287)");
    st = validate_tree_paths(&trees[j], n, o.tips_per_replica ? o.n_replicas : 1);
    if (st) return st;
  }

  std::vector<double> B2v, Bcv, scalev, pidv(n), qp;
  st = compute_model(model->variant, n, model->Q, model->B, model->Omega, B2v, Bcv, scalev, qp);
  if (st) return st;
  for (int i = 0; i < n; ++i) {
    pidv[i] = model->pid[i];
    if (!(pidv[i] >= 0.0) || !std::isfinite(pidv[i])) return fail(PHM_ERR_BAD_INPUT, "pid must be non-negative");
  }

  phm_engine* e = new phm_engine();
  std::unique_ptr<phm_engine> guard(e);
  e->n = n; e->cols = n + n * (n - 1); e->variant = model->variant;
  e->dcols = e->cols;
  if (ks_layout(e->variant)) {
    const int k = hidden_rates(e->variant) ? n / 2 - 1 : 0;
    e->cols = n + n * n + 2 + 3 * k + 1;
    e->dcols = n + n * n + 1;
  }
  e->qparams = qp;
  e->Omega = model->Omega;
  e->hB2 = B2v; e->hBc = Bcv; e->hscale = scalev; e->hpid = pidv;
  e->n_trees = n_trees; e->S_tree = o.n_replicas; e->tpt = (o.n_replicas + 63) / 64;
  e->S = n_trees * o.n_replicas; e->tiles = n_trees * e->tpt; e->S_pad = e->tiles * 64;
  e->max_iters = max_iters; e->reduce = o.reduce ? 1 : 0;
  e->ipl = o.iters_per_launch > 0 ? o.iters_per_launch : 8;
  e->tips_per_replica = o.tips_per_replica != 0 || n_trees > 1;
  e->dbg = dbg;
  e->phase_timing = dbg.phase_timing != 0;
  e->normalise = normalised_variant(e->variant) || (o.rescale_pruning != 0 && (e->variant == PHM_MCMC || e->variant == PHM_MCMC_SPARSE));
  e->cap_boost = 1 << std::max(0, std::min(10, boost_log2));
  e->recover = o.no_recovery == 0;
  if (e->recover) { e->saved = save_input(trees, n_trees, model, o, max_iters); e->saved->dbg = dbg; }

  std::string serr;
  e->scheds.resize(n_trees);
  for (int j = 0; j < n_trees; ++j)
    if (!phm::build_schedule(x->n_tips, x->n_node, x->n_edge, trees[j].edge, e->scheds[j], serr)) return fail(PHM_ERR_BAD_INPUT, "tree: " + serr);
  e->sched = e->scheds[0];
  phm::Schedule& s = e->sched;
  st = select_device(o.device);
  if (st) return st;
  HIPCHK(hipGetDevice(&e->device));
  const int E = s.n_edge;

  const bool one_small = !e->wide() && n_trees == 1;
  const int map_req = o.mapping;
  const bool auto_map = map_req == PHM_MAP_AUTO && o.storage == 0;
  if ((map_req == 2 || map_req == 3) && n_trees != 1) return fail(PHM_ERR_UNSUPPORTED, "the branch-parallel mappings take a single tree");
  int mapping = PHM_MAP_REPLICAS;
  if (e->wide()) {
    if (n_trees == 1 && (map_req == 3 || (auto_map && e->S > wbranch_auto_max_replicas(s)))) mapping = PHM_MAP_TILES;
    else if (n_trees == 1 && (map_req == 2 || auto_map)) mapping = PHM_MAP_BRANCHES;
  } else {
    int narrow_cap = narrow_auto_max_replicas(s);
    bool long_paths = false;
    if (one_small && auto_map) {
      double max_seg = 0.0, tot_seg = 0.0;
      for (int b = 0; b < E; ++b) {
        const double seg = expected_segments(x, b, model->Omega);
        max_seg = std::max(max_seg, seg); tot_seg += seg;
      }
      if (max_seg > 64.0) narrow_cap = std::max(narrow_cap, (int)std::min(65535.0, 1.35e-3 * max_seg / (4.4e-8 * tot_seg)));
      long_paths = max_seg > 64.0;
    }
    if (one_small && (map_req == 2 || (auto_map && e->S <= narrow_cap))) mapping = PHM_MAP_BRANCHES;
    else if (one_small && (map_req == 3 || (auto_map && (long_paths || e->S <= TILES_AUTO_MAX_REPLICAS)))) mapping = PHM_MAP_TILES;
  }
  if (mapping == PHM_MAP_BRANCHES && e->S > 65535) {
    if (!auto_map) return fail(PHM_ERR_UNSUPPORTED, "the one-lane-per-branch / wave-per-(replica, branch) mappings take at most 65 535 replicas");
    mapping = (e->wide() || e->S <= TILES_AUTO_MAX_REPLICAS) ? PHM_MAP_TILES : PHM_MAP_REPLICAS;
  }
  if (mapping == PHM_MAP_BRANCHES) {
    st = narrow_setup(e, x, model, o, max_iters);
    if (st == PHM_ERR_OOM && auto_map) { mapping = PHM_MAP_TILES; st = PHM_OK; }
  }
  if (mapping == PHM_MAP_TILES) {
    st = e->wide() ? wtiles_setup(e, x, model, o, max_iters) : tiles_setup(e, x, model, o, max_iters);
    if (st == PHM_ERR_OOM && auto_map) { mapping = PHM_MAP_REPLICAS; st = PHM_OK; }
  }
  e->mapping = mapping;
  if (mapping == PHM_MAP_REPLICAS) st = replicas_setup(e, trees, model, o);
  if (st) return st;
  st = upload_model(e);
  if (st) return st;
  HIPCHK(hipEventCreate(&e->ev0));
  HIPCHK(hipEventCreate(&e->ev1));
  *out = guard.release();
  return PHM_OK;
}

extern "C" {

int32_t phm_engine_run(phm_engine* e, int32_t n_iters, void* hip_stream) {
  e = live(e);
  if (!e) return fail(PHM_ERR_STATE, "engine is NULL");
  if (e->dead) return dead_engine();
  if (n_iters < 0 || e->iters_done + n_iters > e->max_iters) return fail(PHM_ERR_STATE, "iteration range exceeds max_iters");
  HIPCHK(hipSetDevice(e->device));
  hipStream_t stream = reinterpret_cast<hipStream_t>(hip_stream);
  HIPCHK(hipEventRecord(e->ev0, stream));
  int launches = 0;
  hipError_t le = hipSuccess;
  if (e->mapping == PHM_MAP_BRANCHES) {
    for (int i = 0; i < n_iters && le == hipSuccess; ++i) {
      const int it = e->iters_done + i;
      small_n(e, [&](auto& p) { le = phm::launch_narrow_sweep(p.br, e->nw_tier_off, e->nw_walk_off, it, stream, i > 0); });
      if (e->wide()) le = phm::launch_wbranch_sweep(e->pwb, e->nw_up_off, e->nw_down_off, it, stream);
      launches += (int)(e->nw_up_off.size() + e->nw_down_off.size()) + 2;
    }
    if (n_iters > 0 && le == hipSuccess)
      small_n(e, [&](auto& p) { le = phm::launch_narrow_stats(p.br, e->iters_done + n_iters - 1, stream); });
    HIPCHK(le);
  } else if (e->mapping == PHM_MAP_TILES) {
    e->phase_iters = 0;
    if (e->phase_timing) {
      while ((int)e->phase_ev.size() < 5 * n_iters) { hipEvent_t ev; HIPCHK(hipEventCreate(&ev)); e->phase_ev.push_back(ev); }
      e->phase_iters = n_iters;
    }
    for (int i = 0; i < n_iters && le == hipSuccess; ++i) {
      const int it = e->iters_done + i;
      hipEvent_t* pev = e->phase_timing ? &e->phase_ev[5 * (size_t)i] : nullptr;
      phm::McmcMapsLaunch ml;
      const bool rec = e->maps.mode != phm::MAPS_OFF && it < (int)e->maps.j_of_iter.size() && e->maps.j_of_iter[it] >= 0;
      if (rec) { ml.mode = e->maps.mode; ml.j = e->maps.j_of_iter[it]; ml.J = e->maps.J; ml.dev = e->maps.dev; ++launches; }
      const phm::McmcMapsLaunch* mlp = rec ? &ml : nullptr;
      small_n(e, [&](auto& p) { le = phm::launch_tiles_sweep(p.tl, e->nw_up_off, e->nw_node_off, e->nw_tier_off, it, stream, pev, mlp); });
      if (e->wide()) le = phm::launch_wtiles_sweep(e->pwt, e->wt_band, e->wt_sparse, e->nw_up_off, e->nw_down_off, e->nw_tier_off, it, stream, pev, mlp);
      const bool clusters = !e->nw_tier_off.empty();
      const int tiers = (int)e->nw_tier_off.size() - 1;
      if (clusters && e->wide())
        launches += (e->pwt.band_up > 0 && !e->wt_sparse.kernel ? tiers : (int)e->nw_up_off.size() - 1) + tiers + 4;
      else
        launches += clusters ? 2 * tiers + 3
                             : (int)(e->nw_up_off.size() + e->nw_down_off.size()) + 2;
    }
    HIPCHK(le);
  } else {
    for (int done = 0; done < n_iters;) {
      int chunk = std::min(e->ipl, n_iters - done);
      small_n(e, [&](auto& p) { le = phm::launch_mcmc(p.rep, e->iters_done + done, chunk, stream); });
      if (e->wide()) le = phm::launch_mcmc_wide(e->pw, e->iters_done + done, chunk, stream);
      HIPCHK(le);
      done += chunk;
      ++launches;
    }
  }
  HIPCHK(hipEventRecord(e->ev1, stream));
  for (int i = 0; i < n_iters; ++i) e->qhist.push_back(e->qparams);
  e->iters_done += n_iters;
  bool host_row = false;
  if (e->mapping == PHM_MAP_BRANCHES) small_n(e, [&](auto& p) { host_row = p.br.host_row != nullptr; });
  e->epi_iter = (host_row && n_iters > 0) ? e->iters_done - 1 : -1;
  e->last_stream = stream;
  e->timing_pending = true;
  e->last_launches = launches;
  return PHM_OK;
}

static int32_t recover_capacity(phm_engine* e) {
  const int T = e->iters_done;
  std::shared_ptr<SavedInput> sv = e->saved;
  hipStream_t stream = e->last_stream;
  int boost_log2 = 0;
  while ((1 << boost_log2) < e->cap_boost) ++boost_log2;
  if (boost_log2 >= 8) return fail(PHM_ERR_CAPACITY, "a branch outgrew its dwell capacity after 8 doublings of the slots");
  e->release_device();
  e->dead = true;
  phm_options o = sv->opt;
  phm_engine* r = nullptr;
  const std::vector<std::pair<int32_t, std::vector<double>>> hist = sv->model_hist;
  int32_t st = phm_engine_create_impl(sv->flat.data(), (int32_t)sv->flat.size(), &sv->model, &o, sv->dbg, boost_log2 + 1, sv->max_iters, &r);
  if (!st && sv->dbg.fail_recovery) {
    delete r; r = nullptr;
    st = fail(PHM_ERR_OOM, "phm_debug_options.fail_recovery is set");
  }
  if (st) return (st == PHM_ERR_OOM) ? fail(PHM_ERR_CAPACITY, "a branch outgrew its dwell capacity and larger slots do not fit in HBM: " + g_phm_err) : st;
  r->recoveries = e->recoveries + 1;
  r->maps = e->maps;
  if (r->maps.mode == phm::MAPS_WRITE && r->maps.dev.bad_row)
    st = hipMemsetAsync(r->maps.dev.bad_row, 0xFF, sizeof(unsigned long long), stream) == hipSuccess ? PHM_OK : fail(PHM_ERR_NO_DEVICE, "hipMemsetAsync failed");
  size_t h = 0;
  for (int it = 0; it < T && !st;) {
    while (!st && h < hist.size() && hist[h].first <= it) { st = phm_engine_set_model(r, hist[h].second.data()); ++h; }
    if (st) break;
    const int next = (h < hist.size()) ? std::min(T, hist[h].first) : T;
    st = phm_engine_run(r, next - it, stream);
    it = next;
  }
  while (!st && h < hist.size()) { st = phm_engine_set_model(r, hist[h].second.data()); ++h; }
  if (!st) st = phm_engine_sync(r);
  if (st) { const std::string msg = g_phm_err; delete r; return fail(st, "capacity recovery failed, the engine is no longer usable: " + msg); }
  e->fwd = r;
  e->dead = false;
  return PHM_OK;
}

int32_t phm_engine_sync(phm_engine* e) {
  e = live(e);
  if (!e) return fail(PHM_ERR_STATE, "engine is NULL");
  if (e->dead) return dead_engine();
  HIPCHK(hipSetDevice(e->device));
  HIPCHK(wait_stream(e->last_stream));
  if (e->timing_pending) {
    float ms = 0.f;
    HIPCHK(hipEventElapsedTime(&ms, e->ev0, e->ev1));
    e->last_ms = ms;
    e->timing_pending = false;
    for (double& v : e->phase_ms) v = 0.0;
    for (int i = 0; i < e->phase_iters; ++i)
      for (int ph = 0; ph < 4; ++ph) {
        float pm = 0.f;
        HIPCHK(hipEventElapsedTime(&pm, e->phase_ev[5 * (size_t)i + ph], e->phase_ev[5 * (size_t)i + ph + 1]));
        e->phase_ms[ph] += pm;
      }
  }
  if (e->epi_iter == e->iters_done - 1 && e->epi_iter >= 0) {
    const double* hr = e->pin_row.as<double>();
    const uint32_t derr = (uint32_t)hr[e->dcols + 1];
    e->seg_total = (unsigned long long)hr[e->dcols];
    if ((derr & phm::DERR_CAPACITY) && !(derr & ~phm::DERR_CAPACITY) && e->recover && e->saved) return recover_capacity(e);
    return device_status(derr);
  }
  HIPCHK(e->pin_status.reserve(16));
  HIPCHK(hipMemcpyAsync(e->pin_status.p, e->d_err.p, sizeof(uint32_t), hipMemcpyDeviceToHost, e->last_stream));
  HIPCHK(hipMemcpyAsync(e->pin_status.as<unsigned char>() + 8, e->d_seg.p, sizeof(unsigned long long), hipMemcpyDeviceToHost, e->last_stream));
  HIPCHK(wait_stream(e->last_stream));
  uint32_t derr = 0;
  std::memcpy(&derr, e->pin_status.p, sizeof derr);
  std::memcpy(&e->seg_total, e->pin_status.as<unsigned char>() + 8, sizeof(unsigned long long));
  const bool wide_replicas = e->wide() && e->mapping == PHM_MAP_REPLICAS;
  if ((derr & phm::DERR_CAPACITY) && !(derr & ~phm::DERR_CAPACITY) && e->recover && e->saved && !wide_replicas) return recover_capacity(e);
  if ((derr & phm::DERR_CAPACITY) && wide_replicas)
    return fail(PHM_ERR_CAPACITY, "a branch outgrew the replica mapping for 5..64 states (at most " + std::to_string(phm::wide_maxseg(e->n)) +
                                  " segments per branch and replica, or the dwell ring); use PHM_MAP_TILES or PHM_MAP_BRANCHES (the automatic choice for one tree)");
  return device_status(derr);
}

int32_t phm_engine_read_stats(phm_engine* e, int32_t iter0, int32_t n, double* out) {
  e = live(e);
  if (!e || !out) return fail(PHM_ERR_STATE, "engine/out is NULL");
  if (e->dead) return dead_engine();
  if (iter0 < 0 || n < 0 || iter0 + n > e->iters_done) return fail(PHM_ERR_STATE, "statistics requested for iterations that have not run");
  if (n == 0) return PHM_OK;
  HIPCHK(hipSetDevice(e->device));
  HIPCHK(wait_stream(e->last_stream));
  const int cols = e->cols, dcols = e->dcols;
  if (e->reduce) {
    HIPCHK(phm::launch_stats_reduce(e->d_stats.as<double>() + (size_t)iter0 * e->tiles * dcols, n, e->tiles, dcols,
                                      e->d_red.as<double>(), e->last_stream));
    std::vector<double> h((size_t)n * dcols);
    HIPCHK(hipMemcpyAsync(h.data(), e->d_red.p, sizeof(double) * h.size(), hipMemcpyDeviceToHost, e->last_stream));
    HIPCHK(hipStreamSynchronize(e->last_stream));
    result_matrix(e, iter0, n, out, [&](int i, int c) { return h[(size_t)i * dcols + c]; });
  } else {
    const size_t hn = (size_t)n * dcols * e->S_pad;
    std::vector<double> hv;
    const double* h;
    if (n == 1 && iter0 == e->epi_iter && e->S == 1) {
      hv.assign(hn, 0.0);
      for (int c = 0; c < dcols; ++c) hv[(size_t)c * e->S_pad + e->pad_index(0)] = e->pin_row.as<double>()[c];
      h = hv.data();
    } else if (sizeof(double) * hn <= (1u << 20)) {
      HIPCHK(e->pin_down.reserve(sizeof(double) * hn));
      HIPCHK(hipMemcpyAsync(e->pin_down.p, e->d_stats.as<double>() + (size_t)iter0 * dcols * e->S_pad, sizeof(double) * hn, hipMemcpyDeviceToHost, e->last_stream));
      HIPCHK(wait_stream(e->last_stream));
      h = e->pin_down.as<double>();
    } else if (2 * (int64_t)e->S <= e->S_pad) {
      std::vector<int32_t> pick(e->S);
      for (int r = 0; r < e->S; ++r) pick[r] = e->pad_index(r);
      DevBuf d_pick, d_pack;
      const size_t n_rows = (size_t)n * dcols;
      HIPCHK(d_pick.alloc(sizeof(int32_t) * pick.size())); HIPCHK(d_pack.alloc(sizeof(double) * n_rows * e->S));
      HIPCHK(hipMemcpyAsync(d_pick.p, pick.data(), d_pick.bytes, hipMemcpyHostToDevice, e->last_stream));
      HIPCHK(phm::launch_stats_gather(e->d_stats.as<double>() + (size_t)iter0 * dcols * e->S_pad, (int64_t)n_rows, e->S_pad, e->S, d_pick.as<int32_t>(),
                                      d_pack.as<double>(), e->last_stream));
      hv.resize(n_rows * e->S);
      HIPCHK(hipMemcpyAsync(hv.data(), d_pack.p, sizeof(double) * hv.size(), hipMemcpyDeviceToHost, e->last_stream));
      HIPCHK(hipStreamSynchronize(e->last_stream));
      for (int r = 0; r < e->S; ++r)
        result_matrix(e, iter0, n, out + (size_t)r * cols * n, [&](int i, int c) { return hv[((size_t)i * dcols + c) * e->S + r]; });
      return PHM_OK;
    } else {
      hv.resize(hn);
      HIPCHK(hipMemcpy(hv.data(), e->d_stats.as<double>() + (size_t)iter0 * dcols * e->S_pad, sizeof(double) * hn, hipMemcpyDeviceToHost));
      h = hv.data();
    }
    for (int r = 0; r < e->S; ++r) {
      const int pr = e->pad_index(r);
      result_matrix(e, iter0, n, out + (size_t)r * cols * n, [&](int i, int c) { return h[((size_t)i * dcols + c) * e->S_pad + pr]; });
    }
  }
  return PHM_OK;
}

}

int32_t phm_engine_fold_reduced(phm_engine* e, int32_t iter0, int32_t n, std::vector<double>& acc) {
  e = live(e);
  if (!e) return fail(PHM_ERR_STATE, "engine is NULL");
  if (e->dead) return dead_engine();
  if (!e->reduce) return fail(PHM_ERR_STATE, "engine was not created with reduce = 1");
  if (iter0 < 0 || n < 1 || iter0 + n > e->iters_done) return fail(PHM_ERR_STATE, "statistics requested for iterations that have not run");
  HIPCHK(hipSetDevice(e->device));
  HIPCHK(wait_stream(e->last_stream));
  const size_t cnt = (size_t)n * e->dcols;
  if (!acc.empty() && acc.size() != cnt) return fail(PHM_ERR_STATE, "fold: accumulator size mismatch");
  const double* init = nullptr;
  DevBuf dinit;
  if (!acc.empty()) {
    HIPCHK(dinit.alloc(sizeof(double) * cnt));
    HIPCHK(hipMemcpyAsync(dinit.p, acc.data(), sizeof(double) * cnt, hipMemcpyHostToDevice, e->last_stream));
    init = dinit.as<double>();
  }
  HIPCHK(phm::launch_stats_reduce(e->d_stats.as<double>() + (size_t)iter0 * e->tiles * e->dcols, n, e->tiles, e->dcols,
                                    e->d_red.as<double>() + (size_t)iter0 * e->dcols, e->last_stream, init));
  acc.resize(cnt);
  HIPCHK(hipMemcpyAsync(acc.data(), e->d_red.as<double>() + (size_t)iter0 * e->dcols, sizeof(double) * cnt, hipMemcpyDeviceToHost, e->last_stream));
  HIPCHK(hipStreamSynchronize(e->last_stream));
  return PHM_OK;
}

int32_t phm_engine_finish_reduced(phm_engine* e, int32_t iter0, int32_t n, const std::vector<double>& acc, double* out) {
  e = live(e);
  if (!e || !out) return fail(PHM_ERR_STATE, "engine/out is NULL");
  const int dcols = e->dcols;
  if (acc.size() != (size_t)n * dcols) return fail(PHM_ERR_STATE, "fold: accumulator size mismatch");
  result_matrix(e, iter0, n, out, [&](int i, int c) { return acc[(size_t)i * dcols + c]; });
  return PHM_OK;
}

extern "C" {

int32_t phm_engine_dump(phm_engine* e, int32_t replica, int32_t* seg_count, double* seg_dwell, int32_t seg_cap,
                        int32_t* node_states, double* PL) {
  e = live(e);
  if (!e) return fail(PHM_ERR_STATE, "engine is NULL");
  if (e->dead) return dead_engine();
  if (replica < 0 || replica >= e->S) return fail(PHM_ERR_BAD_INPUT, "replica out of range");
  HIPCHK(hipSetDevice(e->device));
  HIPCHK(hipStreamSynchronize(e->last_stream));
  const bool branches = e->mapping == PHM_MAP_BRANCHES;
  const int padded = branches ? replica : e->pad_index(replica), L = branches ? 1 : 64, blk = padded / L, lane = padded % L;
  const phm::Schedule& s = e->scheds[e->n_trees > 1 ? blk / e->tpt : 0];
  const int E = s.n_edge, T = s.n_tips, n = e->n;
  if (branches) {
    std::vector<int32_t> mc(E);
    HIPCHK(hipMemcpy(mc.data(), e->d_nw_mcount.as<int32_t>() + (size_t)replica * E, sizeof(int32_t) * E, hipMemcpyDeviceToHost));
    if (seg_count) for (int b = 0; b < E; ++b) seg_count[b] = mc[b];
    if (seg_dwell) {
      std::vector<double> dw((size_t)e->nw_total_cap);
      const double* src = ((e->iters_done & 1) ? e->d_nw_dwB.as<double>() : e->d_nw_dwA.as<double>()) + (size_t)replica * e->nw_total_cap;
      HIPCHK(hipMemcpy(dw.data(), src, sizeof(double) * dw.size(), hipMemcpyDeviceToHost));
      for (int b = 0; b < E; ++b)
        for (int i = 0; i < std::min<int>(mc[b], seg_cap); ++i) seg_dwell[(size_t)b * seg_cap + i] = dw[(size_t)e->nw_off[b] + i];
    }
  } else {
    std::vector<uint16_t> mc((size_t)E * 64);
    HIPCHK(hipMemcpy(mc.data(), e->d_mcount.as<uint16_t>() + (size_t)blk * E * 64, sizeof(uint16_t) * mc.size(), hipMemcpyDeviceToHost));
    if (seg_count) for (int b = 0; b < E; ++b) seg_count[b] = mc[(size_t)b * 64 + lane];
    if (seg_dwell && e->mapping == PHM_MAP_TILES) {
      std::vector<double> dw((size_t)e->rows * 64);
      const double* src = ((e->iters_done & 1) ? e->d_dw1.as<double>() : e->d_dw0.as<double>()) + (size_t)blk * e->rows * 64;
      HIPCHK(hipMemcpy(dw.data(), src, sizeof(double) * dw.size(), hipMemcpyDeviceToHost));
      for (int b = 0; b < E; ++b)
        for (int i = 0; i < std::min<int>(mc[(size_t)b * 64 + lane], seg_cap); ++i)
          seg_dwell[(size_t)b * seg_cap + i] = dw[((size_t)e->tl_slot[b] + i) * 64 + lane];
    } else if (seg_dwell) {
      std::vector<double> dw((size_t)e->rows * 64);
      int32_t cur[2];
      HIPCHK(hipMemcpy(cur, e->d_cursor.as<int32_t>() + 2 * blk, sizeof cur, hipMemcpyDeviceToHost));
      const double* src = ((!e->ring && cur[0]) ? e->d_dw1.as<double>() : e->d_dw0.as<double>()) + (size_t)blk * e->rows * 64;
      HIPCHK(hipMemcpy(dw.data(), src, sizeof(double) * dw.size(), hipMemcpyDeviceToHost));
      size_t row = e->ring ? (size_t)cur[0] : 0;
      for (int k = 0; k < E; ++k) {
        const phm::DownStep& d = s.down[k];
        int m = std::min<int>(mc[(size_t)d.edge * 64 + lane], seg_cap);
        for (int i = 0; i < m; ++i) seg_dwell[(size_t)d.edge * seg_cap + i] = dw[((row + i) % (size_t)e->rows) * 64 + lane];
        int mx = 0;
        for (int l = 0; l < 64; ++l) mx = std::max<int>(mx, mc[(size_t)d.edge * 64 + l]);
        row += mx;
      }
    }
  }
  auto tip_state = [&](int t) -> int { return e->tips_per_replica ? e->tips_host[((size_t)blk * T + t) * L + lane] : e->tips_host[t]; };
  if (node_states) {
    std::vector<uint8_t> ns((size_t)s.n_node * L);
    HIPCHK(hipMemcpy(ns.data(), e->d_nstate.as<uint8_t>() + (size_t)blk * s.n_node * L, ns.size(), hipMemcpyDeviceToHost));
    for (int t = 0; t < T; ++t) node_states[t] = tip_state(t) + 1;
    for (int v = 0; v < s.n_node; ++v) node_states[T + v] = ns[(size_t)v * L + lane] + 1;
  }
  if (PL) {
    std::vector<double> pl((size_t)s.n_node * n * L);
    HIPCHK(hipMemcpy(pl.data(), e->d_PL.as<double>() + (size_t)blk * s.n_node * n * L, sizeof(double) * pl.size(), hipMemcpyDeviceToHost));
    for (int t = 0; t < T; ++t)
      for (int c = 0; c < n; ++c) PL[(size_t)t * n + c] = (c == tip_state(t)) ? 1.0 : 0.0;
    for (int v = 0; v < s.n_node; ++v)
      for (int c = 0; c < n; ++c)
        PL[(size_t)(T + v) * n + c] = (e->wide() && e->mapping == PHM_MAP_REPLICAS) ? pl[((size_t)v * L + lane) * n + c] : pl[((size_t)v * n + c) * L + lane];
  }
  return PHM_OK;
}

int32_t phm_engine_info(phm_engine* e, phm_info* info) {
  e = live(e);
  if (!e || !info) return fail(PHM_ERR_STATE, "engine/info is NULL");
  if (e->dead) return dead_engine();
  std::memset(info, 0, sizeof(*info));
  info->n_states = e->n; info->n_edge = e->sched.n_edge; info->n_replicas = e->S; info->n_replicas_padded = e->S_pad;
  info->n_cols = e->cols; info->max_iters = e->max_iters; info->device_bytes = e->bytes;
  info->rows_per_replica = e->rows;
  info->seg_read = (int64_t)e->seg_total; info->seg_written = 0;
  info->last_run_ms = e->last_ms; info->last_run_launches = e->last_launches; info->iters_done = e->iters_done;
  info->recoveries = e->recoveries;
  info->mapping = e->mapping;
  info->sparse_chains = (e->mapping == PHM_MAP_TILES && e->wide()) ? (e->pwt.band_up > 0 || e->wt_sparse.kernel != nullptr) + 2 * (e->pwt.band_draw > 0) + 4 * (e->wt_sparse.kernel != nullptr) : 0;
  return PHM_OK;
}

void phm_engine_destroy(phm_engine* e) { delete e; }

int32_t phm_engine_phase_ms(phm_engine* e, double* out4) {
  e = live(e);
  if (!e || !out4) return fail(PHM_ERR_STATE, "engine/out is NULL");
  if (e->dead) return dead_engine();
  if (!e->phase_timing || e->mapping != PHM_MAP_TILES) return fail(PHM_ERR_STATE, "phase timing needs phm_options.phase_timing = 1 and a (tile, item) mapping");
  for (int i = 0; i < 4; ++i) out4[i] = e->phase_ms[i];
  return PHM_OK;
}

}


extern "C" int32_t phm_engine_reduced_stats_device(phm_engine* e, int32_t iter0, int32_t n, void* hip_stream,
                                                   void** out_dev) {
  e = live(e);
  if (!e || !out_dev) return fail(PHM_ERR_STATE, "engine/out is NULL");
  if (e->dead) return dead_engine();
  if (!e->reduce) return fail(PHM_ERR_STATE, "engine was not created with reduce = 1");
  if (iter0 < 0 || n < 1 || iter0 + n > e->iters_done) return fail(PHM_ERR_STATE, "statistics requested for iterations that have not run");
  HIPCHK(hipSetDevice(e->device));
  if (!e->d_red_out.p) HIPCHK(e->d_red_out.alloc(sizeof(double) * (size_t)e->max_iters * e->dcols));
  HIPCHK(phm::launch_stats_reduce(e->d_stats.as<double>() + (size_t)iter0 * e->tiles * e->dcols, n, e->tiles, e->dcols,
                                    e->d_red_out.as<double>(), reinterpret_cast<hipStream_t>(hip_stream)));
  *out_dev = e->d_red_out.p;
  return PHM_OK;
}

extern "C" int32_t phm_engine_time_pruning(phm_engine* e, int32_t n_iters, void* hip_stream, double* ms_out) {
  e = live(e);
  if (!e || !ms_out) return fail(PHM_ERR_STATE, "engine/ms_out is NULL");
  if (e->dead) return dead_engine();
  const bool wt = e->wide() && e->mapping == PHM_MAP_TILES;
  if (!wt && (e->wide() || e->mapping != PHM_MAP_REPLICAS || e->n_trees > 1)) return fail(PHM_ERR_UNSUPPORTED, "pruning-only timing is implemented for the replica mapping with n_states <= 4 and the lane-per-replica mapping of 5..64 states");
  if (n_iters < 1) return fail(PHM_ERR_BAD_INPUT, "n_iters must be >= 1");
  HIPCHK(hipSetDevice(e->device));
  hipStream_t stream = reinterpret_cast<hipStream_t>(hip_stream);
  HIPCHK(hipEventRecord(e->ev0, stream));
  hipError_t le = hipSuccess;
  if (wt) for (int i = 0; i < n_iters && le == hipSuccess; ++i) le = phm::launch_wtiles_up(e->pwt, e->wt_band, e->wt_sparse, e->nw_up_off, e->nw_tier_off, stream);
  small_n(e, [&](auto& sp) { auto p = sp.rep; p.prune_only = 1; for (int i = 0; i < n_iters && le == hipSuccess; ++i) le = phm::launch_mcmc(p, e->iters_done, 1, stream); });
  HIPCHK(le);
  HIPCHK(hipEventRecord(e->ev1, stream));
  HIPCHK(hipStreamSynchronize(stream));
  float ms = 0.f;
  HIPCHK(hipEventElapsedTime(&ms, e->ev0, e->ev1));
  *ms_out = ms;
  e->last_stream = stream;
  e->timing_pending = false;
  return PHM_OK;
}

extern "C" int32_t phm_engine_set_model(phm_engine* e, const double* Q) {
  e = live(e);
  if (!e || !Q) return fail(PHM_ERR_STATE, "engine/Q is NULL");
  if (e->dead) return dead_engine();
  if (e->saved) {
    auto& hist = e->saved->model_hist;
    if (!hist.empty() && hist.back().first == e->iters_done) hist.pop_back();
    const size_t entry = sizeof(double) * (size_t)e->n * e->n;
    if ((hist.size() + 1) * entry > (256u << 20)) { e->saved.reset(); e->recover = false; }
    else hist.emplace_back(e->iters_done, std::vector<double>(Q, Q + (size_t)e->n * e->n));
  }
  HIPCHK(hipSetDevice(e->device));
  HIPCHK(wait_stream(e->last_stream));
  std::vector<double> B2, Bc, scale, qp;
  int32_t st = compute_model(e->variant, e->n, Q, nullptr, e->Omega, B2, Bc, scale, qp);
  if (st) return st;
  e->hB2 = B2; e->hBc = Bc; e->hscale = scale; e->qparams = qp;
  return upload_model(e);
}
```

### phylomap_amd/csrc/phm_internal.h

```cpp
#pragma once

#include "../../include/phylomap_hip.h"

#include <hip/hip_runtime.h>

#include <algorithm>
#include <cmath>
#include <cstdio>
#include <chrono>
#include <cstdlib>
#include <cstring>
#include <memory>
#include <string>
#include <thread>
#include <vector>

#include "phm_exp.h"
#include "phm_mcmc.h"
#include "phm_mcmc_maps.h"
#include "phm_narrow.h"
#include "phm_qupdate.h"
#include "phm_sched.h"
#include "phm_tiles.h"
#include "phm_wbranch.h"
// ... 5 lines not shown
inline thread_local phm_debug_options g_phm_debug = {};

inline int32_t fail(int32_t st, const std::string& msg) { g_phm_err = msg; return st; }

#define HIPCHK(call)                                                                              \
  do {                                                                                            \
    hipError_t _e = (call);                                                                       \
    if (_e != hipSuccess) {                                                                       \
      int32_t _st = (_e == hipErrorOutOfMemory) ? PHM_ERR_OOM : PHM_ERR_NO_DEVICE;                \
      return fail(_st, std::string(#call) + ": " + hipGetErrorString(_e));                        \
    }                                                                                             \
  } while (0)

struct DevBuf {
  void* p = nullptr;
  size_t bytes = 0;
  DevBuf() = default;
  DevBuf(const DevBuf&) = delete;
  DevBuf& operator=(const DevBuf&) = delete;
  ~DevBuf() { if (p) (void)hipFree(p); }
  void reset() { if (p) (void)hipFree(p); p = nullptr; bytes = 0; }
  hipError_t alloc(size_t n) {
    reset();
    hipError_t e = hipMalloc(&p, n ? n : 16);
    if (e == hipSuccess) bytes = n; else p = nullptr;
    return e;
  }
  template <typename T> T* as() const { return reinterpret_cast<T*>(p); }
};

template <typename T>
hipError_t upload(DevBuf& d, const T* h, size_t count) {
  hipError_t e = d.alloc(sizeof(T) * count);
  if (e == hipSuccess && count) e = hipMemcpy(d.p, h, sizeof(T) * count, hipMemcpyHostToDevice);
  return e;
}
template <typename T>
hipError_t upload(DevBuf& d, const std::vector<T>& h) { return upload(d, h.data(), h.size()); }

struct KernelTimer {
  hipEvent_t ev[2] = {nullptr, nullptr};
  KernelTimer() = default;
  KernelTimer(const KernelTimer&) = delete;
  KernelTimer& operator=(const KernelTimer&) = delete;
  ~KernelTimer() { for (hipEvent_t x : ev) if (x) (void)hipEventDestroy(x); }
  hipError_t start() {
    for (hipEvent_t& x : ev)
      if (!x) { const hipError_t e = hipEventCreate(&x); if (e != hipSuccess) return e; }
    return hipEventRecord(ev[0], nullptr);
  }
  hipError_t stop() { return hipEventRecord(ev[1], nullptr); }
  hipError_t elapsed(double& ms) {
    float f = 0.f;
    hipError_t e = hipEventSynchronize(ev[1]);
    if (e == hipSuccess) e = hipEventElapsedTime(&f, ev[0], ev[1]);
    if (e == hipSuccess) ms = f;
    return e;
  }
};

struct PinnedBuf {
  void* p = nullptr;
  size_t bytes = 0;
  PinnedBuf() = default;
  PinnedBuf(const PinnedBuf&) = delete;
  PinnedBuf& operator=(const PinnedBuf&) = delete;
  ~PinnedBuf() { if (p) (void)hipHostFree(p); }
  hipError_t reserve(size_t n) {
    if (n <= bytes) return hipSuccess;
    if (p) (void)hipHostFree(p);
    p = nullptr; bytes = 0;
    hipError_t e = hipHostMalloc(&p, n, hipHostMallocDefault);
    if (e == hipSuccess) bytes = n; else p = nullptr;
    return e;
  }
  template <typename T> T* as() const { return reinterpret_cast<T*>(p); }
};

inline hipError_t wait_stream(hipStream_t s) {
  const auto t0 = std::chrono::steady_clock::now();
  for (;;) {
    const hipError_t q = hipStreamQuery(s);
    if (q == hipSuccess) return hipSuccess;
    if (q != hipErrorNotReady) return q;
    if (std::chrono::steady_clock::now() - t0 > std::chrono::microseconds(500)) return hipStreamSynchronize(s);
  }
}

inline int32_t select_device(int32_t device) {
  int n = 0;
  if (hipGetDeviceCount(&n) != hipSuccess || n <= 0) return fail(PHM_ERR_NO_DEVICE, "no HIP device visible (this library has no CPU fallback)");
  if (device >= 0) {
    if (device >= n) return fail(PHM_ERR_NO_DEVICE, "device ordinal out of range");
    HIPCHK(hipSetDevice(device));
  }
  return PHM_OK;
}

inline int32_t device_status(uint32_t derr) {
  if (derr & phm::DERR_ZERO_PROB) return fail(PHM_ERR_ZERO_PROB, "all-zero or non-finite probability vector while sampling a state (RcppArmadillo::sample would throw)");
  if (derr & phm::DERR_CAPACITY) return fail(PHM_ERR_CAPACITY, "a branch outgrew its dwell capacity; lower phm_options.cap_tail");
  if (derr & phm::DERR_UNIF_CAP) return fail(PHM_ERR_UNIF_CAP, "newunifSample needed more than 300 jumps on a branch (src/phylomap.cpp:120)");
  if (derr & phm::DERR_SAMPLEONCE) return fail(PHM_ERR_ZERO_PROB, "sampleOnce ran past the last state (src/phylomap.cpp:85-89)");
  return PHM_OK;
}

inline void cm_to_rm(const double* cm, int n, std::vector<double>& rm) {
  rm.resize((size_t)n * n);
  for (int i = 0; i < n; ++i)
    for (int j = 0; j < n; ++j) rm[(size_t)i * n + j] = cm[i + (size_t)j * n];
}

inline int pade_squarings(const double* Q_rm, int n, double t) {
  double norm = 0.0;
  for (int i = 0; i < n; ++i) {
    double r = 0.0;
    for (int j = 0; j < n; ++j) r += std::fabs(Q_rm[(size_t)i * n + j] * t);
    if (r > norm) norm = r;
  }
  double l2 = (norm > 0.0) ? std::log2(norm) : 0.0;
  int ex = 0;
  (void)std::frexp(l2, &ex);
  return std::max(0, ex + 1);
}

inline void host_chain_matvec(const double* M, int n, const double* x, double* y, bool fused) {
  for (int i = 0; i < n; ++i) {
    if (fused) {
      double acc = 0.0;
      for (int c = 0; c < n; ++c) acc = std::fma(M[(size_t)i * n + c], x[c], acc);
      y[i] = acc;
    } else {
      double acc = M[i * n] * x[0];
      for (int c = 1; c < n; ++c) acc += M[i * n + c] * x[c];
      y[i] = acc;
    }
  }
}
inline void host_chain_matTvec(const double* M, int n, const double* x, double* y, bool fused) {
  for (int c = 0; c < n; ++c) {
    if (fused) {
      double acc = 0.0;
      for (int r = 0; r < n; ++r) acc = std::fma(M[(size_t)r * n + c], x[r], acc);
      y[c] = acc;
    } else {
      double acc = M[c] * x[0];
      for (int r = 1; r < n; ++r) acc += M[r * n + c] * x[r];
      y[c] = acc;
    }
  }
}

inline void build_chain_tables(const double* Bc, int n, int ktab, std::vector<double>& col, std::vector<double>& row, bool fused,
                               bool want_row = true) {
  col.assign((size_t)ktab * n * n, 0.0);
  row.assign(want_row ? (size_t)ktab * n * n : 0, 0.0);
  for (int j = 0; j < n; ++j) { col[(size_t)j * n + j] = 1.0; if (want_row) row[(size_t)j * n + j] = 1.0; }
  auto chains = [&](int j0, int j1) {
    for (int k = 1; k < ktab; ++k)
      for (int j = j0; j < j1; ++j) {
        host_chain_matvec(Bc, n, &col[((size_t)(k - 1) * n + j) * n], &col[((size_t)k * n + j) * n], fused);
        if (want_row) host_chain_matTvec(Bc, n, &row[((size_t)(k - 1) * n + j) * n], &row[((size_t)k * n + j) * n], fused);
      }
  };
  const double work = (double)ktab * n * n * n * (want_row ? 2 : 1);
  const int nt = work < 4e6 ? 1 : std::min<int>({8, n, (int)std::max(1u, std::thread::hardware_concurrency())});
  if (nt <= 1) { chains(0, n); return; }
  std::vector<std::thread> th;
  for (int t = 0; t < nt; ++t) th.emplace_back(chains, (int)((int64_t)n * t / nt), (int)((int64_t)n * (t + 1) / nt));
  for (std::thread& t : th) t.join();
}

inline int32_t validate_tree_paths(const phm_tree* x, int n, int n_tip_vectors) {
  if (!x || !x->edge || !x->states || !x->map_off || !x->maps || !x->mapnames) return fail(PHM_ERR_BAD_INPUT, "tree: missing field");
  for (int64_t i = 0; i < (int64_t)n_tip_vectors * x->n_tips; ++i)
    if (x->states[i] < 1 || x->states[i] > n) return fail(PHM_ERR_BAD_INPUT, "x$states must be in 1..n");
  if (x->map_off[0] != 0) return fail(PHM_ERR_BAD_INPUT, "map_off[0] must be 0");
  for (int b = 0; b < x->n_edge; ++b) {
    int m = x->map_off[b + 1] - x->map_off[b];
    if (m < 1) return fail(PHM_ERR_BAD_INPUT, "every branch needs at least one segment in x$maps");
    if (m > 50000) return fail(PHM_ERR_BAD_INPUT, "more than 50000 segments on one branch");
    for (int i = x->map_off[b]; i < x->map_off[b + 1]; ++i) {
      if (x->mapnames[i] < 1 || x->mapnames[i] > n) return fail(PHM_ERR_BAD_INPUT, "x$mapnames must be in 1..n");
      if (!std::isfinite(x->maps[i]) || x->maps[i] < 0.0) return fail(PHM_ERR_BAD_INPUT, "x$maps must be finite and non-negative");
    }
  }
  return PHM_OK;
}

inline int32_t check_edge_lengths(const phm_tree* x) {
  for (int b = 0; b < x->n_edge; ++b)
    if (!std::isfinite(x->edge_length[b]) || x->edge_length[b] < 0.0)
      return fail(PHM_ERR_BAD_INPUT, "edge.length must be finite and non-negative (edge row " + std::to_string(b + 1) + ")");
  return PHM_OK;
}

inline int32_t check_generator(const double* Q, int n, std::vector<double>& Qr) {
  double qmax = 0.0;
  for (int i = 0; i < n * n; ++i) {
    if (!std::isfinite(Q[i])) return fail(PHM_ERR_BAD_INPUT, "Q must be finite");
    qmax = std::max(qmax, std::fabs(Q[i]));
  }
  cm_to_rm(Q, n, Qr);
  for (int i = 0; i < n; ++i) {
    double row = 0.0;
    for (int j = 0; j < n; ++j) {
      const double q = Qr[(size_t)i * n + j];
      row += q;
      if (j != i && q < 0.0) return fail(PHM_ERR_BAD_INPUT, "Q: off-diagonal entries must be >= 0 (row " + std::to_string(i + 1) + ")");
    }
    if (std::fabs(row) > 1e-12 * qmax) return fail(PHM_ERR_BAD_INPUT, "Q: row " + std::to_string(i + 1) + " does not sum to 0");
  }
  return PHM_OK;
}

inline int32_t check_root_prior(const double* pid, int n, double& psum) {
  psum = 0.0;
  for (int i = 0; i < n; ++i) {
    if (!(pid[i] >= 0.0) || !std::isfinite(pid[i])) return fail(PHM_ERR_ZERO_PROB, "pid must be finite and non-negative");
    psum += pid[i];
  }
  if (!(psum > 0.0)) return fail(PHM_ERR_ZERO_PROB, "pid sums to zero");
  return PHM_OK;
}

inline int32_t check_observe(const int32_t* observe, int n, std::vector<int32_t>& obs) {
  obs.resize(n);
  for (int i = 0; i < n; ++i) {
    obs[i] = observe ? observe[i] : i + 1;
    if (obs[i] < 1 || obs[i] > n) return fail(PHM_ERR_BAD_INPUT, "observe: values must be in 1..n");
  }
  return PHM_OK;
}

struct SavedInput {
  struct TreeCopy {
    phm_tree t;
    std::vector<int32_t> edge, states, map_off, mapnames;
    std::vector<double> edge_length, maps;
  };
  std::vector<TreeCopy> trees;
  std::vector<phm_tree> flat;
  phm_model model;
  std::vector<double> Q, pid, B;
  phm_options opt;
  phm_debug_options dbg = {};
  int32_t max_iters = 0;
  std::vector<std::pair<int32_t, std::vector<double>>> model_hist;
};

struct phm_engine {
  std::shared_ptr<SavedInput> saved;
  phm_engine* fwd = nullptr;
  int cap_boost = 1;
  bool recover = true;
  int recoveries = 0;
  bool dead = false;
  int n = 0, cols = 0, dcols = 0, variant = 0;
  std::vector<double> qparams;
  std::vector<std::vector<double>> qhist;
  double Omega = 0.0;
  std::vector<double> hB2, hBc, hscale, hpid;
  int S = 0, S_pad = 0, tiles = 0, max_iters = 0, iters_done = 0, ipl = 0;
  int reduce = 0, device = 0;
  bool normalise = false;
  phm::Schedule sched;
  std::vector<phm::Schedule> scheds;
  int n_trees = 1, S_tree = 0, tpt = 0;
  DevBuf d_roots;
  int rpt = 64;
  int pad_index(int r) const { return n_trees > 1 ? (r / S_tree) * tpt * 64 + r % S_tree : (r / rpt) * 64 + r % rpt; }
  std::vector<uint8_t> tips_host;
  bool tips_per_replica = false;
  int64_t rows = 0;
  DevBuf d_mask;
  DevBuf d_up, d_down, d_col, d_row, d_tips, d_mcount, d_dw0, d_dw1, d_cursor, d_PL, d_nstate, d_stats, d_err, d_seg, d_red, d_red_out;
  int32_t mapping = PHM_MAP_REPLICAS;
  bool wide() const { return n > 4; }
  template <int NS> struct SmallParams {
    phm::McmcParams<NS> rep;
    phm::NarrowParams<NS> br;
    phm::TileParams<NS> tl;
  };
  SmallParams<2> s2;
  SmallParams<3> s3;
  SmallParams<4> s4;
  bool ring = true;
  phm::WideParams pw;
  DevBuf d_B2, d_Bc, d_scale, d_pid;
  std::vector<int32_t> nw_walk_off;
  std::vector<int32_t> nw_tier_off;
  std::vector<int32_t> nw_up_off, nw_down_off;
  std::vector<int32_t> nw_node_off;
  std::vector<int64_t> nw_off;
  int nw_klong = 0;
  bool nw_cluster_async = false;
  int nw_n_wide = 0;
  int64_t nw_total_cap = 0;
  DevBuf d_nw_up_off, d_nw_down_off, d_nw_up_order, d_nw_down_order, d_nw_node_order, d_nw_border, d_nw_off, d_nw_colL, d_nw_rowL, d_nw_maskL, d_nw_mcount, d_nw_dwA, d_nw_dwB,
      d_nw_mstate, d_nw_mlen, d_nw_estate, d_nw_part, d_nw_rowbuf, d_nw_down_lv, d_nw_dmap, d_nw_dmap_edge, d_nw_walk_off, d_nw_edge_parent, d_nw_cl_nodes, d_nw_cl_item_off, d_nw_cl_lvl_ptr, d_nw_cl_lvl_off, d_ell_col, d_ell_val, d_ell2_col, d_ell2_val;
  DevBuf d_wb_cnt;
  phm::WideBranchParams pwb;
  std::vector<int32_t> tl_slot;
  DevBuf d_tl_slot, d_tl_pdw, d_tl_pchunk, d_tl_cnt, d_tl_estate, d_tl_pseg, d_tl_segprev;
  phm::WtParams pwt;
  DevBuf d_wt_dwfx, d_wt_segacc, d_wt_B2, d_wt_totL, d_wt_pair_slot, d_wt_slot_col, d_wt_B2band, d_wt_mstate, d_wt_dwfx_tile, d_wt_cnt_tile;
  phm::WtBand wt_band;
  phm::WtSparseUp wt_sparse;
  DevBuf d_wt_coef;
  int sparse_req = 0;
  phm_debug_options dbg = {};
  bool phase_timing = false;
  std::vector<hipEvent_t> phase_ev;
  int phase_iters = 0;
  double phase_ms[4] = {0.0, 0.0, 0.0, 0.0};
  hipEvent_t ev0 = nullptr, ev1 = nullptr;
  hipStream_t last_stream = nullptr;
  PinnedBuf pin_up, pin_down, pin_status, pin_row;
  int epi_iter = -1;
  bool timing_pending = false;
  double last_ms = 0.0;
  int last_launches = 0;
  int64_t bytes = 0;
  unsigned long long seg_total = 0;
  struct MapsRequest {
    int mode = phm::MAPS_OFF;
    phm::MapsDev dev;
    std::vector<int32_t> j_of_iter;
    int J = 0;
  } maps;
  void release_device() {
    DevBuf* all[] = {&d_roots, &d_mask, &d_up, &d_down, &d_col, &d_row, &d_tips, &d_mcount, &d_dw0, &d_dw1, &d_cursor, &d_PL, &d_nstate,
                     &d_stats, &d_err, &d_seg, &d_red, &d_red_out, &d_B2, &d_Bc, &d_scale, &d_pid, &d_nw_up_off, &d_nw_down_off,
                     &d_nw_up_order, &d_nw_down_order, &d_nw_node_order, &d_nw_border, &d_nw_off, &d_nw_colL, &d_nw_rowL, &d_nw_maskL, &d_nw_mcount,
                     &d_nw_dwA, &d_nw_dwB, &d_nw_mstate, &d_nw_mlen, &d_nw_estate, &d_nw_part, &d_nw_rowbuf, &d_nw_down_lv, &d_nw_dmap, &d_nw_dmap_edge, &d_nw_walk_off, &d_nw_edge_parent, &d_nw_cl_nodes, &d_nw_cl_item_off, &d_nw_cl_lvl_ptr, &d_nw_cl_lvl_off, &d_ell_col, &d_ell_val,
                     &d_ell2_col, &d_ell2_val, &d_wb_cnt, &d_tl_slot, &d_tl_pdw, &d_tl_pchunk, &d_tl_cnt, &d_tl_estate, &d_tl_pseg,
                     &d_tl_segprev, &d_wt_dwfx, &d_wt_segacc, &d_wt_B2, &d_wt_totL, &d_wt_pair_slot, &d_wt_slot_col, &d_wt_B2band, &d_wt_mstate, &d_wt_dwfx_tile, &d_wt_cnt_tile, &d_wt_coef};
    for (DevBuf* b : all) b->reset();
  }
  ~phm_engine() {
    delete fwd;
    if (ev0) (void)hipEventDestroy(ev0);
    if (ev1) (void)hipEventDestroy(ev1);
    for (hipEvent_t ev : phase_ev) (void)hipEventDestroy(ev);
  }
};

int32_t phm_engine_create_impl(const phm_tree* trees, int32_t n_trees, const phm_model* model, const phm_options* opt_in,
                               const phm_debug_options& dbg, int boost_log2, int32_t max_iters, phm_engine** out);
int32_t phm_engine_fold_reduced(phm_engine* e, int32_t iter0, int32_t n, std::vector<double>& acc);
int32_t phm_engine_finish_reduced(phm_engine* e, int32_t iter0, int32_t n, const std::vector<double>& acc, double* out);

inline phm_options resolve_options(const phm_options* opt) {
  phm_options o;
  std::memset(&o, 0, sizeof(o));
  o.device = -1;
  if (opt) o = *opt;
  if (o.n_devices == 1) { o.device = o.devices[0]; o.n_devices = 0; }
  return o;
}

inline double expected_segments(const phm_tree* x, int b, double Omega) {
  double tb = 0.0;
  for (int i = x->map_off[b]; i < x->map_off[b + 1]; ++i) tb += x->maps[i];
  return std::max(1.0 + Omega * tb, (double)(x->map_off[b + 1] - x->map_off[b]));
}

struct phm_shard { int32_t device; int64_t first, count; };
int32_t phm_plan_shards(const phm_options& o, int64_t units, std::vector<phm_shard>& shards);

template <typename Body>
int32_t run_shards(const std::vector<phm_shard>& shards, Body body) {
  struct Result { int32_t st = PHM_OK; std::string err; double ms = 0.0; };
  std::vector<Result> res(shards.size());
  const phm_debug_options dbg = g_phm_debug;
  auto work = [&](size_t i) {
    g_phm_debug = dbg;
    g_phm_last_kernel_ms = 0.0;
    res[i].st = body(shards[i], i);
    if (res[i].st) res[i].err = g_phm_err;
    res[i].ms = g_phm_last_kernel_ms;
  };
  const bool many = shards.size() > 1;
  int caller_device = -1;
  if (many && hipGetDevice(&caller_device) != hipSuccess) caller_device = -1;
  std::vector<std::thread> th;
  for (size_t i = 1; i < shards.size(); ++i) th.emplace_back(work, i);
  if (!shards.empty()) work(0);
  for (std::thread& t : th) t.join();
  if (caller_device >= 0) (void)hipSetDevice(caller_device);
  double ms = 0.0;
  for (size_t i = 0; i < shards.size(); ++i) {
    if (res[i].st) return fail(res[i].st, many ? "device " + std::to_string(shards[i].device) + ": " + res[i].err : res[i].err);
    ms = std::max(ms, res[i].ms);
  }
  g_phm_last_kernel_ms = ms;
  return PHM_OK;
}
```

### phylomap_amd/csrc/phm_tiles.h

```cpp
#pragma once

#include <hip/hip_runtime.h>
#include <stdint.h>

#include <vector>

#include "phm_device.h"
#include "phm_sched.h"

namespace phm {

constexpr int TILES_BLOCK = 256;
constexpr int TILES_CHUNK = 64;
constexpr int TILES_PERSISTENT_WGS = 2048;
constexpr int TILES_KTAB = 24;
constexpr int TILES_CL_BLOCK = 512;
constexpr int TILES_CL_NODES = 256;
#ifndef TILES_CL_BAND
#define TILES_CL_BAND 8
#endif
constexpr int64_t TILES_CL_MAX_WORK = 65536;

template <int NS>
struct TileParams {
  int32_t n_tips, n_node, n_edge, root;
  int32_t n_tiles, n_rep, n_rep_pad, replica_offset;
  int32_t normalise, tips_per_replica, ks, tip_masks, reduce, n_cols;
  int32_t klong;
  int32_t group, n_groups;
  int32_t n_chunks;
  uint32_t seed_lo, seed_hi;
  int64_t rows;
  double B2[NS * NS], Bc[NS * NS], scale[NS], pid[NS];
  const UpStep* up;
  const int32_t* up_order;
  const int32_t* node_order;
  const ClusterNode* cl_nodes;
  const int32_t* cl_lvl_ptr;
  const int32_t* cl_lvl_off;
  const int32_t* branch_order;
  const int32_t* slot;
  const double* colL;
  const double* rowL;
  const double* maskL;
  const uint8_t* tips;
  uint16_t* mcount;
  double* dw[2];
  uint8_t* estate;
  uint8_t* mstate;
  double* PL;
  uint8_t* nstate;
  double* pdw;
  double* pchunk;
  uint32_t* cnt;
  int32_t cnt_copies;
  uint32_t* pseg;
  uint32_t* segprev;
  double* stats;
  uint32_t* err;
  unsigned long long* segcnt;
};

hipError_t launch_tiles_init(int n_edge, int n_tiles, int64_t rows, const int32_t* slot, const int32_t* map_off,
                             const double* maps, double* dw0, uint16_t* mcount, hipStream_t stream);

struct McmcMapsLaunch;

template <int NS>
hipError_t launch_tiles_sweep(const TileParams<NS>& p, const std::vector<int32_t>& up_off,
                              const std::vector<int32_t>& node_off, const std::vector<int32_t>& tier_off, int it, hipStream_t stream,
                              hipEvent_t* phase_ev = nullptr, const McmcMapsLaunch* maps = nullptr);

}
```

### phylomap_amd/csrc/phm_tiles.hip

```cpp
#include "phm_tiles.h"

#include <type_traits>

#include "phm_mcmc_maps.h"

namespace phm {

namespace {

template <int NS>
__device__ __forceinline__ void child_vec(const TileParams<NS>& p, const double* __restrict__ PLt,
                                          const uint8_t* __restrict__ tips_t, int child, int k, int lane, double (&v)[NS],
                                          uint32_t& err) {
  if (child < 0) {
    const int tip = ~child;
    const int st = p.tips_per_replica ? tips_t[tip * 64 + lane] : p.tips[tip];
    if (k >= p.klong) { err |= DERR_CAPACITY; k = p.klong - 1; }
    const double* src = (p.ks && p.tip_masks) ? p.maskL + ((size_t)k * 2 + (st & 1)) * NS : p.colL + ((size_t)k * NS + st) * NS;
#pragma unroll
    for (int c = 0; c < NS; ++c) v[c] = src[c];
  } else {
#pragma unroll
    for (int c = 0; c < NS; ++c) v[c] = PLt[(child * NS + c) * 64 + lane];
    for (int i = 0; i < k; ++i) matvec_u<NS>(p.Bc, v);
  }
}

template <int NS>
__device__ __forceinline__ void up_node(const TileParams<NS>& p, int tile, int parent, int child0, int child1, int edge0, int edge1, int lane,
                                        uint32_t& err) {
  double* __restrict__ PLt = p.PL + (size_t)tile * p.n_node * NS * 64;
  const uint16_t* __restrict__ mct = p.mcount + (size_t)tile * p.n_edge * 64;
  const uint8_t* __restrict__ tips_t = p.tips_per_replica ? p.tips + (size_t)tile * p.n_tips * 64 : p.tips;
  double x[NS], y[NS];
  child_vec<NS>(p, PLt, tips_t, child1, (int)mct[edge1 * 64 + lane] - 1, lane, x, err);
  child_vec<NS>(p, PLt, tips_t, child0, (int)mct[edge0 * 64 + lane] - 1, lane, y, err);
#pragma unroll
  for (int c = 0; c < NS; ++c) x[c] = x[c] * y[c];
  if (p.normalise) {
    double s = x[0];
#pragma unroll
    for (int c = 1; c < NS; ++c) s += x[c];
#pragma unroll
    for (int c = 0; c < NS; ++c) x[c] = x[c] / s;
  }
#pragma unroll
  for (int c = 0; c < NS; ++c) PLt[(parent * NS + c) * 64 + lane] = x[c];
}

template <int NS>
__device__ __forceinline__ void up_item(const TileParams<NS>& p, int tile, const UpStep& st, uint32_t lane, uint32_t& err) {
  double* __restrict__ PLt = p.PL + (size_t)tile * p.n_node * NS * 64;
  const uint16_t* __restrict__ mct = p.mcount + (size_t)tile * p.n_edge * 64;
  int k[2], tipst[2] = {0, 0};
  double v[2][NS];
#pragma unroll
  for (int s = 0; s < 2; ++s) k[s] = (int)at(mct + (size_t)st.edge[s] * 64, lane * 2u) - 1;
#pragma unroll
  for (int s = 0; s < 2; ++s)
    if (st.child[s] >= 0) {
#pragma unroll
      for (int c = 0; c < NS; ++c) v[s][c] = at(PLt + (size_t)st.child[s] * NS * 64, ((uint32_t)c * 64u + lane) * 8u);
    }
#pragma unroll
  for (int s = 0; s < 2; ++s)
    if (st.child[s] < 0) {
      const int tip = ~st.child[s];
      tipst[s] = p.tips_per_replica ? at(p.tips + ((size_t)tile * p.n_tips + tip) * 64, lane) : p.tips[tip];
    }
#pragma unroll
  for (int s = 1; s >= 0; --s) {
    if (st.child[s] < 0) {
      int kk = k[s];
      if (kk >= p.klong) { err |= DERR_CAPACITY; kk = p.klong - 1; }
      const double* src = (p.ks && p.tip_masks) ? p.maskL + ((size_t)kk * 2 + (tipst[s] & 1)) * NS : p.colL + ((size_t)kk * NS + tipst[s]) * NS;
#pragma unroll
      for (int c = 0; c < NS; ++c) v[s][c] = src[c];
    } else {
      for (int i = 0; i < k[s]; ++i) matvec_u<NS>(p.Bc, v[s]);
    }
  }
  double x[NS];
#pragma unroll
  for (int c = 0; c < NS; ++c) x[c] = v[1][c] * v[0][c];
  if (p.normalise) {
    double sum = x[0];
#pragma unroll
    for (int c = 1; c < NS; ++c) sum += x[c];
#pragma unroll
    for (int c = 0; c < NS; ++c) x[c] = x[c] / sum;
  }
#pragma unroll
  for (int c = 0; c < NS; ++c) at(PLt + (size_t)st.parent * NS * 64, ((uint32_t)c * 64u + lane) * 8u) = x[c];
}

template <int NS>
__global__ __launch_bounds__(TILES_BLOCK) void tiles_up_kernel(TileParams<NS> p, int begin, int end) {
  const uint32_t lane = threadIdx.x & 63;
  const int item = blockIdx.x * (TILES_BLOCK / 64) + __builtin_amdgcn_readfirstlane(threadIdx.x >> 6);
  const int n_lvl = end - begin;
  if (item >= n_lvl * p.n_tiles) return;
  const int tile = item / n_lvl;
  const UpStep st = p.up[p.up_order[begin + item % n_lvl]];
  uint32_t err = 0;
  up_item<NS>(p, tile, st, lane, err);
  if (err) atomicOr(p.err, err);
}

constexpr int TILES_CL_ASYNC_NODES = 256;
template <int NS, bool ASYNC>
__global__ __launch_bounds__(TILES_CL_BLOCK) void tiles_up_cluster_kernel(TileParams<NS> p, int cl_begin, int n_cl) {
  constexpr int W = TILES_CL_BLOCK / 64;
  const int lane = threadIdx.x & 63;
  const int wave = __builtin_amdgcn_readfirstlane(threadIdx.x >> 6);
  const int cl = cl_begin + (int)(blockIdx.x % (unsigned)n_cl);
  const int tile = (int)(blockIdx.x / (unsigned)n_cl);
  const int l0 = p.cl_lvl_ptr[cl], l1 = p.cl_lvl_ptr[cl + 1] - 1;
  uint32_t err = 0;
  if (ASYNC) {
    __shared__ int32_t s_done[TILES_CL_ASYNC_NODES];
    __shared__ int32_t s_next;
    const int first = p.cl_lvl_off[l0], n_items = p.cl_lvl_off[l1] - first;
    if (n_items <= TILES_CL_ASYNC_NODES) {
      for (int i = threadIdx.x; i < TILES_CL_ASYNC_NODES; i += TILES_CL_BLOCK) s_done[i] = 0;
      if (threadIdx.x == 0) s_next = 0;
      __syncthreads();
      for (;;) {
        int idx = 0;
        if (lane == 0) idx = atomicAdd(&s_next, 1);
        idx = __builtin_amdgcn_readfirstlane(idx);
        if (idx >= n_items) break;
        const ClusterNode nd = p.cl_nodes[first + idx];
#pragma unroll
        for (int k = 0; k < 2; ++k)
          if (nd.slot[k] >= 0)
            while (__hip_atomic_load(&s_done[nd.slot[k]], __ATOMIC_RELAXED, __HIP_MEMORY_SCOPE_WORKGROUP) == 0) __builtin_amdgcn_s_sleep(1);
        __builtin_amdgcn_fence(__ATOMIC_ACQUIRE, "workgroup");
        up_node<NS>(p, tile, nd.parent, nd.child[0], nd.child[1], nd.edge[0], nd.edge[1], lane, err);
        __builtin_amdgcn_fence(__ATOMIC_RELEASE, "workgroup");
        if (lane == 0) __hip_atomic_store(&s_done[idx], 1, __ATOMIC_RELAXED, __HIP_MEMORY_SCOPE_WORKGROUP);
      }
      if (err) atomicOr(p.err, err);
      return;
    }
  }
  for (int l = l0; l < l1; ++l) {
    const int i1 = p.cl_lvl_off[l + 1];
    for (int i = p.cl_lvl_off[l] + wave; i < i1; i += W) {
      const ClusterNode nd = p.cl_nodes[i];
      up_node<NS>(p, tile, nd.parent, nd.child[0], nd.child[1], nd.edge[0], nd.edge[1], lane, err);
    }
    __syncthreads();
  }
  if (err) atomicOr(p.err, err);
}

template <int NS>
__device__ __forceinline__ void draw_root(const TileParams<NS>& p, int tile, int it, int lane, uint32_t& err) {
  const double* __restrict__ PLt = p.PL + (size_t)tile * p.n_node * NS * 64;
  const uint32_t rep = (uint32_t)(p.replica_offset + tile * 64 + lane);
  double pr[NS];
#pragma unroll
  for (int c = 0; c < NS; ++c) pr[c] = p.pid[c] * PLt[(p.root * NS + c) * 64 + lane];
  const double u = stream_u(p.seed_lo, p.seed_hi, rep, (uint32_t)it, ENT_NODE | (uint32_t)(p.root + p.n_tips), 0);
  p.nstate[((size_t)tile * p.n_node + p.root) * 64 + lane] = (uint8_t)sample_cat<NS>(pr, u, err);
}

template <int NS>
__global__ __launch_bounds__(TILES_BLOCK) void tiles_root_kernel(TileParams<NS> p, int it) {
  const int lane = threadIdx.x & 63;
  const int tile = blockIdx.x * (TILES_BLOCK / 64) + __builtin_amdgcn_readfirstlane(threadIdx.x >> 6);
  if (tile >= p.n_tiles) return;
  uint32_t err = 0;
  draw_root<NS>(p, tile, it, lane, err);
  if (err) atomicOr(p.err, err);
}

template <int NS>
__device__ __forceinline__ void down_edge(const TileParams<NS>& p, int tile, int it, int b, int parent, int child, int lane, uint32_t& err) {
  const double* __restrict__ PLt = p.PL + (size_t)tile * p.n_node * NS * 64;
  uint8_t* __restrict__ nst = p.nstate + (size_t)tile * p.n_node * 64;
  const uint8_t* __restrict__ tips_t = p.tips_per_replica ? p.tips + (size_t)tile * p.n_tips * 64 : p.tips;
  const uint32_t rep = (uint32_t)(p.replica_offset + tile * 64 + lane);
  const int m = p.mcount[((size_t)tile * p.n_edge + b) * 64 + lane];
  const int ps = nst[parent * 64 + lane];
  int cs;
  if (child >= 0 || (p.ks && p.tip_masks)) {
    int kk = m - 1;
    if (kk >= p.klong) { err |= DERR_CAPACITY; kk = p.klong - 1; }
    const double* src = p.rowL + ((size_t)kk * NS + ps) * NS;
    double w[NS];
    uint32_t node_id;
    if (child >= 0) {
#pragma unroll
      for (int c = 0; c < NS; ++c) w[c] = src[c] * PLt[(child * NS + c) * 64 + lane];
      node_id = (uint32_t)(child + p.n_tips);
    } else {
      const int tip = ~child;
      const int par = (p.tips_per_replica ? tips_t[tip * 64 + lane] : p.tips[tip]) & 1;
#pragma unroll
      for (int c = 0; c < NS; ++c) w[c] = src[c] * (((c & 1) == par) ? 1.0 : 0.0);
      node_id = (uint32_t)tip;
    }
    const double u = stream_u(p.seed_lo, p.seed_hi, rep, (uint32_t)it, ENT_NODE | node_id, 0);
    cs = sample_cat<NS>(w, u, err);
    if (child >= 0) nst[child * 64 + lane] = (uint8_t)cs;
  } else {
    const int tip = ~child;
    cs = p.tips_per_replica ? tips_t[tip * 64 + lane] : p.tips[tip];
  }
  p.estate[((size_t)tile * p.n_edge + b) * 64 + lane] = (uint8_t)(ps | (cs << 4));
}

template <int NS>
struct SideLoads {
  int32_t m, tipst;
  double pl[NS];
};

template <int NS>
struct NodeLoads {
  int32_t tile;
  UpStep st;
  int32_t ps;
  SideLoads<NS> side[2];
};

__device__ __forceinline__ int32_t sched_word(const int32_t* q, int i) {
  return ((const __attribute__((address_space(4))) int32_t*)q)[i];
}

enum : int { SIDE_TIP = 0, SIDE_NODE = 1, SIDE_TIP_DRAWN = 2 };

template <class F>
__device__ __forceinline__ void with_side_kinds(bool draw_tips, int child0, int child1, F&& f) {
  using Tip = std::integral_constant<int, SIDE_TIP>;
  using Node = std::integral_constant<int, SIDE_NODE>;
  using Drawn = std::integral_constant<int, SIDE_TIP_DRAWN>;
  const int code = (child0 >= 0 ? 1 : 0) | (child1 >= 0 ? 2 : 0);
  if (!draw_tips) {
    switch (code) {
      case 0: f(Tip{}, Tip{}); break;
      case 1: f(Node{}, Tip{}); break;
      case 2: f(Tip{}, Node{}); break;
      default: f(Node{}, Node{}); break;
    }
  } else {
    switch (code) {
      case 0: f(Drawn{}, Drawn{}); break;
      case 1: f(Node{}, Drawn{}); break;
      case 2: f(Drawn{}, Node{}); break;
      default: f(Node{}, Node{}); break;
    }
  }
}

template <int NS>
__device__ __forceinline__ void node_record(const TileParams<NS>& p, NodeLoads<NS>& d, int item, int n_lvl, int begin) {
  d.tile = item / n_lvl;
  const int32_t* rec = reinterpret_cast<const int32_t*>(p.up + sched_word(p.node_order, begin + item % n_lvl));
  static_assert(sizeof(UpStep) == 5 * sizeof(int32_t), "UpStep: parent, two children, two edges");
  d.st.parent = sched_word(rec, 0);
  d.st.child[0] = sched_word(rec, 1); d.st.child[1] = sched_word(rec, 2);
  d.st.edge[0] = sched_word(rec, 3); d.st.edge[1] = sched_word(rec, 4);
}

template <int NS, int K0, int K1>
__device__ __forceinline__ void node_request(const TileParams<NS>& p, NodeLoads<NS>& d, uint32_t lane) {
  constexpr int kind[2] = {K0, K1};
  d.ps = at(p.nstate + ((size_t)d.tile * p.n_node + d.st.parent) * 64, lane);
#pragma unroll
  for (int k = 0; k < 2; ++k) {
    if (kind[k] != SIDE_TIP) d.side[k].m = at(p.mcount + ((size_t)d.tile * p.n_edge + d.st.edge[k]) * 64, lane * 2u);
    else d.side[k].m = 1;
  }
#pragma unroll
  for (int k = 0; k < 2; ++k) {
    const double* PLc = p.PL + ((size_t)d.tile * p.n_node + d.st.child[k]) * NS * 64;
#pragma unroll
    for (int c = 0; c < NS; ++c) d.side[k].pl[c] = kind[k] == SIDE_NODE ? at(PLc, ((uint32_t)c * 64u + lane) * 8u) : 0.0;
  }
#pragma unroll
  for (int k = 0; k < 2; ++k) {
    if (kind[k] != SIDE_NODE) {
      const int tip = ~d.st.child[k];
      d.side[k].tipst = p.tips_per_replica ? at(p.tips + ((size_t)d.tile * p.n_tips + tip) * 64, lane) : p.tips[tip];
    } else {
      d.side[k].tipst = 0;
    }
  }
}

template <int NS, int K0, int K1>
__device__ __forceinline__ void node_finish(const TileParams<NS>& p, const NodeLoads<NS>& d, int it, uint32_t lane, uint32_t& err) {
  constexpr int kind[2] = {K0, K1};
  const uint32_t rep = (uint32_t)(p.replica_offset + d.tile * 64) + lane;
  double w[2][NS];
#pragma unroll
  for (int k = 0; k < 2; ++k) {
    const SideLoads<NS>& sd = d.side[k];
    if (kind[k] != SIDE_TIP) {
      int kk = sd.m - 1;
      if (kk >= p.klong) { err |= DERR_CAPACITY; kk = p.klong - 1; }
      const double* src = p.rowL + ((size_t)kk * NS + d.ps) * NS;
      if (kind[k] == SIDE_NODE) {
#pragma unroll
        for (int c = 0; c < NS; ++c) w[k][c] = src[c] * sd.pl[c];
      } else {
        const int par = sd.tipst & 1;
#pragma unroll
        for (int c = 0; c < NS; ++c) w[k][c] = src[c] * (((c & 1) == par) ? 1.0 : 0.0);
      }
    }
  }
#pragma unroll
  for (int k = 0; k < 2; ++k) {
    const int child = d.st.child[k];
    int cs;
    if (kind[k] != SIDE_TIP) {
      const uint32_t node_id = kind[k] == SIDE_NODE ? (uint32_t)(child + p.n_tips) : (uint32_t)(~child);
      const double u = stream_u(p.seed_lo, p.seed_hi, rep, (uint32_t)it, ENT_NODE | node_id, 0);
      cs = sample_cat<NS>(w[k], u, err);
      if (kind[k] == SIDE_NODE) at(p.nstate + ((size_t)d.tile * p.n_node + child) * 64, lane) = (uint8_t)cs;
    } else {
      cs = d.side[k].tipst;
    }
    at(p.estate + ((size_t)d.tile * p.n_edge + d.st.edge[k]) * 64, lane) = (uint8_t)(d.ps | (cs << 4));
  }
}

template <int NS>
__global__ __launch_bounds__(TILES_BLOCK) void tiles_down_kernel(TileParams<NS> p, int it, int begin, int end) {
  const uint32_t lane = threadIdx.x & 63;
  const int n_lvl = end - begin;
  const int n_items = n_lvl * p.n_tiles;
  const int stride = gridDim.x * (TILES_BLOCK / 64);
  const bool draw_tips = p.ks && p.tip_masks;
  uint32_t err = 0;
  for (int item = blockIdx.x * (TILES_BLOCK / 64) + __builtin_amdgcn_readfirstlane(threadIdx.x >> 6); item < n_items; item += stride) {
    NodeLoads<NS> d;
    node_record<NS>(p, d, item, n_lvl, begin);
    with_side_kinds(draw_tips, d.st.child[0], d.st.child[1], [&](auto k0, auto k1) {
      node_request<NS, decltype(k0)::value, decltype(k1)::value>(p, d, lane);
      node_finish<NS, decltype(k0)::value, decltype(k1)::value>(p, d, it, lane, err);
    });
  }
  if (err) atomicOr(p.err, err);
}

template <int NS>
__global__ __launch_bounds__(TILES_CL_BLOCK) void tiles_down_cluster_kernel(TileParams<NS> p, int it, int cl_begin, int n_cl, int with_root) {
  constexpr int W = TILES_CL_BLOCK / 64;
  const int lane = threadIdx.x & 63;
  const int wave = __builtin_amdgcn_readfirstlane(threadIdx.x >> 6);
  const int cl = cl_begin + (int)(blockIdx.x % (unsigned)n_cl);
  const int tile = (int)(blockIdx.x / (unsigned)n_cl);
  const int l0 = p.cl_lvl_ptr[cl], l1 = p.cl_lvl_ptr[cl + 1] - 1;
  uint32_t err = 0;
  if (with_root) {
    if (wave == 0) draw_root<NS>(p, tile, it, lane, err);
    __syncthreads();
  }
  for (int l = l1 - 1; l >= l0; --l) {
    const int i0 = p.cl_lvl_off[l], cnt = 2 * (p.cl_lvl_off[l + 1] - i0);
    for (int j = wave; j < cnt; j += W) {
      const ClusterNode nd = p.cl_nodes[i0 + (j >> 1)];
      down_edge<NS>(p, tile, it, nd.edge[j & 1], nd.parent, nd.child[j & 1], lane, err);
    }
    __syncthreads();
  }
  if (err) atomicOr(p.err, err);
}

template <int NS, bool KS, bool LONG>
__global__ __launch_bounds__(TILES_BLOCK, LONG ? 5 : (KS ? 7 : 8)) void tiles_branch_kernel(TileParams<NS> p, int it) {
  constexpr int NCNT = KS ? NS * NS : NS * (NS - 1);
  __shared__ double s_dw_all[(TILES_BLOCK / 64) * NS * 64];
  __shared__ uint16_t s_cnt_all[(TILES_BLOCK / 64) * NCNT * 64];
  __shared__ double s_B2[NS * NS], s_scale[NS];
  __shared__ double s_col[TILES_KTAB * NS * NS];
  __shared__ __align__(16) double s_ltab[2 * PHM_LOGTAB_N];
  const int lane = threadIdx.x & 63;
  const int wave = __builtin_amdgcn_readfirstlane(threadIdx.x >> 6);
  const int item = blockIdx.x * (TILES_BLOCK / 64) + wave;
  const uint32_t lane8 = (uint32_t)lane * 8u;
  const int ktab = min(TILES_KTAB, p.klong);
  for (int i = threadIdx.x; i < ktab * NS * NS; i += TILES_BLOCK) s_col[i] = p.colL[i];
  for (int i = threadIdx.x; i < 2 * PHM_LOGTAB_N; i += TILES_BLOCK) s_ltab[i] = logtab_entry(i);
  if (threadIdx.x < NS * NS) s_B2[threadIdx.x] = p.B2[threadIdx.x];
  if (threadIdx.x < NS) s_scale[threadIdx.x] = p.scale[threadIdx.x];
  __syncthreads();
  if (item >= p.n_groups * p.n_tiles) return;
  const int tile = item % p.n_tiles;
  const int grp = item / p.n_tiles;
  double* s_dw = s_dw_all + wave * NS * 64;
  uint16_t* s_cnt = s_cnt_all + wave * NCNT * 64;
  const uint32_t rep = (uint32_t)(p.replica_offset + tile * 64 + lane);
  uint16_t* __restrict__ mct = p.mcount + (size_t)tile * p.n_edge * 64;
  uint32_t* gc = p.cnt + (((size_t)tile * p.cnt_copies + (grp & (p.cnt_copies - 1))) * NS * NS) * 64 + lane;
  uint32_t err = 0;
#pragma unroll
  for (int c = 0; c < NS; ++c) s_dw[c * 64 + lane] = 0.0;
#pragma unroll
  for (int c = 0; c < NCNT; ++c) s_cnt[c * 64 + lane] = (uint16_t)0;
  auto flush_counts = [&]() {
#pragma unroll
    for (int c = 0; c < NCNT; ++c) {
      const uint32_t v = s_cnt[c * 64 + lane];
      if (v) { atomicAdd(gc + c * 64, v); s_cnt[c * 64 + lane] = (uint16_t)0; }
    }
  };
  uint32_t pending = 0;
  const int q1 = min((grp + 1) * p.group, p.n_edge);
  for (int q = grp * p.group; q < q1; ++q) {
  const int b = p.branch_order[q];
  const int m = mct[b * 64 + lane];
  if (__any(pending + (uint32_t)m > 65535u)) { flush_counts(); pending = 0; }
  pending += (uint32_t)m;
  const int es = p.estate[((size_t)tile * p.n_edge + b) * 64 + lane];
  const int ps = es & 15, cs = es >> 4;
  const int roff = p.slot[b];
  const int cap = p.slot[b + 1] - roff;
  double* __restrict__ in = p.dw[it & 1] + ((size_t)tile * p.rows + roff) * 64;
  double* __restrict__ out = p.dw[(it & 1) ^ 1] + ((size_t)tile * p.rows + roff) * 64;
  auto IN = [&](int k) -> double& { return at(in, (uint32_t)k * 512u + lane8); };
  uint8_t* __restrict__ msrow = LONG ? p.mstate + ((size_t)tile * p.rows + roff) * 64 + lane : nullptr;
  auto MS = [&](int k) -> uint8_t& { return msrow[(uint32_t)k * 64u]; };

  Stream su, se;
  su.open(ENT_BSTATE | (uint32_t)b, (uint32_t)it, rep, p.seed_lo, p.seed_hi);
  se.open(ENT_BEXP | (uint32_t)b, (uint32_t)it, rep, p.seed_lo, p.seed_hi);
  const int mmax = wave_max_count(m);
  int mnew = 0;

  auto draw_state_w = [&](int i, int sprev, uint32_t word) -> int {
    int kk = m - i - 1;
    if (kk >= p.klong) { err |= DERR_CAPACITY; kk = p.klong - 1; }
    double pr[NS];
    {
      const double* beta = s_col + ((kk < ktab ? kk : ktab - 1) * NS + cs) * NS;
#pragma unroll
      for (int c = 0; c < NS; ++c) pr[c] = beta[c];
    }
    if (kk >= ktab) {
      const double* __restrict__ beta = p.colL + ((size_t)kk * NS + cs) * NS;
#pragma unroll
      for (int c = 0; c < NS; ++c) pr[c] = beta[c];
    }
#pragma unroll
    for (int c = 0; c < NS; ++c) pr[c] = s_B2[sprev * NS + c] * pr[c];
    return sample_cat<NS>(pr, u01(word), err);
  };
  auto draw_state = [&](int i, int sprev) -> int { return draw_state_w(i, sprev, su.draw_word((uint32_t)(i - 1))); };

  if (LONG || mmax <= 64) {
    uint64_t pk0 = 0, pk1 = 0;
    int w = 0;
    int cur_s = (m == 1) ? cs : ps;
    double first_len = 0.0, second_len = 0.0;
    double cur_len = IN(0);
    double dnext = (!LONG && m > 1) ? IN(1) : 0.0;
    double dq[4] = {0.0, 0.0, 0.0, 0.0}, bq[4][NS];
    auto beta_row = [&](int i, double (&bv)[NS]) {
      const int kk = min(max(m - i - 1, 0), p.klong - 1);
      const double* bl = s_col + ((kk < ktab ? kk : ktab - 1) * NS + cs) * NS;
#pragma unroll
      for (int c = 0; c < NS; ++c) bv[c] = bl[c];
      if (kk >= ktab) {
        const double* __restrict__ bg = p.colL + ((size_t)kk * NS + cs) * NS;
#pragma unroll
        for (int c = 0; c < NS; ++c) bv[c] = bg[c];
      }
    };
    if (LONG) {
#pragma unroll
      for (int q = 0; q < 4; ++q) {
#pragma unroll
        for (int c = 0; c < NS; ++c) bq[q][c] = 0.0;
        if (1 + q < m) { dq[q] = IN(1 + q); beta_row(1 + q, bq[q]); }
      }
    }
    for (int i0 = 1; i0 < mmax; i0 += 4) {
      uint32_t wd[4] = {0u, 0u, 0u, 0u};
      if (i0 < mmax - 1)
        philox4x32((uint32_t)((i0 - 1) >> 2), ENT_BSTATE | (uint32_t)b, (uint32_t)it, rep, p.seed_lo, p.seed_hi, wd);
#pragma unroll
      for (int q = 0; q < 4; ++q) {
      const int i = i0 + q;
      if (i < m) {
        int si;
        double di;
        if (LONG) {
          if (m - i - 1 >= p.klong) err |= DERR_CAPACITY;
          double pr[NS];
#pragma unroll
          for (int c = 0; c < NS; ++c) pr[c] = s_B2[cur_s * NS + c] * bq[q][c];
          si = (i == m - 1) ? cs : sample_cat<NS>(pr, u01(wd[q]), err);
          di = dq[q];
          if (i + 4 < m) { dq[q] = IN(i + 4); beta_row(i + 4, bq[q]); }
        } else {
          si = (i == m - 1) ? cs : draw_state_w(i, cur_s, wd[q]);
          di = dnext;
          if (i + 1 < m) dnext = IN(i + 1);
        }
        if (KS) s_cnt[(cur_s * NS + si) * 64 + lane] = (uint16_t)(s_cnt[(cur_s * NS + si) * 64 + lane] + 1u);
        if (si == cur_s) cur_len = cur_len + di;
        else {
          if (w == 0) first_len = cur_len; else if (w == 1) second_len = cur_len; else IN(w) = cur_len;
          if (LONG) MS(w) = (uint8_t)cur_s;
          else if (w < 32) pk0 |= (uint64_t)cur_s << (2 * w); else pk1 |= (uint64_t)cur_s << (2 * (w - 32));
          if (!KS) s_cnt[(cur_s * (NS - 1) + (si > cur_s ? si - 1 : si)) * 64 + lane] = (uint16_t)(s_cnt[(cur_s * (NS - 1) + (si > cur_s ? si - 1 : si)) * 64 + lane] + 1u);
          ++w; cur_s = si; cur_len = di;
        }
      }
      }
    }
    if (LONG) MS(w) = (uint8_t)cur_s;
    else if (w < 32) pk0 |= (uint64_t)cur_s << (2 * w); else pk1 |= (uint64_t)cur_s << (2 * (w - 32));
    const int first_s = (w == 0) ? cur_s : (LONG ? (int)MS(0) : (int)(pk0 & 3u));
    const int nmerged = w + 1;
    const double len0 = (w == 0) ? cur_len : first_len;

    int j = 0;
    int s = first_s;
    int snext = (LONG && nmerged > 1) ? (int)MS(1) : 0;
    double len = len0;
    double lnext = (nmerged > 1) ? ((w == 1) ? cur_len : second_len) : 0.0;
    double tot = 0.0, scale = s_scale[s], acc = s_dw[s * 64 + lane];
    bool stuck = false, done = false;
    for (uint32_t t0 = 0; __any(!done); t0 += 4) {
      uint32_t wd[4];
      philox4x32(t0 >> 2, ENT_BEXP | (uint32_t)b, (uint32_t)it, rep, p.seed_lo, p.seed_hi, wd);
#pragma unroll
      for (int q = 0; q < 4; ++q) {
        if (done) continue;
        double piece;
        bool adv;
        if (stuck || !(0.0 < len)) { stuck = true; piece = len; adv = true; }
        else {
          double rl = scale * neglog_u32(wd[q], s_ltab);
          if ((tot + rl) < len) { piece = rl; tot += rl; adv = false; }
          else { piece = len - tot; adv = true; }
        }
        if (mnew < cap) at(out, (uint32_t)mnew * 512u + lane8) = piece; else err |= DERR_CAPACITY;
        acc += piece;
        ++mnew;
        if (adv) {
          s_dw[s * 64 + lane] = acc;
          ++j;
          if (j >= nmerged) done = true;
          else {
            len = lnext;
            if (j + 1 < w) lnext = IN(j + 1); else lnext = cur_len;
            if (LONG) { s = snext; if (j + 1 < nmerged) snext = (int)MS(j + 1); }
            else s = (int)(((j < 32) ? (pk0 >> (2 * j)) : (pk1 >> (2 * (j - 32)))) & 3u);
            scale = s_scale[s]; tot = 0.0; acc = s_dw[s * 64 + lane];
          }
        }
      }
    }
  } else if (!LONG) {
    uint32_t edraw = 0;
    bool stuck = false;
    auto finalize = [&](int s, double len) {
      if (stuck || !(0.0 < len)) {
        stuck = true;
        if (mnew < cap) at(out, (uint32_t)mnew * 512u + lane8) = len; else err |= DERR_CAPACITY;
        s_dw[s * 64 + lane] += len;
        ++mnew;
        return;
      }
      const double scale = s_scale[s];
      double tot = 0.0;
      double acc = s_dw[s * 64 + lane];
      while (tot < len) {
        double rl = scale * neglog_u32(se.draw_word(edraw++), s_ltab);
        double piece;
        if ((tot + rl) < len) { piece = rl; tot += rl; }
        else { piece = len - tot; tot = len; }
        if (mnew < cap) at(out, (uint32_t)mnew * 512u + lane8) = piece; else err |= DERR_CAPACITY;
        acc += piece;
        ++mnew;
      }
      s_dw[s * 64 + lane] = acc;
    };
    int cur_s = (m == 1) ? cs : ps;
    double cur_len = IN(0);
    for (int i = 1; i <= m; ++i) {
      int si = -1;
      double di = 0.0;
      if (i < m) {
        si = (i == m - 1) ? cs : draw_state(i, cur_s);
        di = IN(i);
      }
      if (KS && si >= 0) s_cnt[(cur_s * NS + si) * 64 + lane] = (uint16_t)(s_cnt[(cur_s * NS + si) * 64 + lane] + 1u);
      if (si == cur_s) cur_len = cur_len + di;
      else {
        finalize(cur_s, cur_len);
        if (!KS && si >= 0) s_cnt[(cur_s * (NS - 1) + (si > cur_s ? si - 1 : si)) * 64 + lane] = (uint16_t)(s_cnt[(cur_s * (NS - 1) + (si > cur_s ? si - 1 : si)) * 64 + lane] + 1u);
        cur_s = si; cur_len = di;
      }
    }
  }
  if (mnew > cap) mnew = cap;
  if (mnew > 65535) { err |= DERR_CAPACITY; mnew = 65535; }
  mct[b * 64 + lane] = (uint16_t)mnew;
  }
  flush_counts();

  double* pd = p.pdw + (((size_t)tile * p.n_edge + grp) * NS) * 64 + lane;
#pragma unroll
  for (int c = 0; c < NS; ++c) pd[c * 64] = s_dw[c * 64 + lane];
  if (err) atomicOr(p.err, err);
}

template <int NS>
__global__ __launch_bounds__(TILES_BLOCK) void tiles_chunk_kernel(TileParams<NS> p) {
  const int lane = threadIdx.x & 63;
  const int item = blockIdx.x * (TILES_BLOCK / 64) + __builtin_amdgcn_readfirstlane(threadIdx.x >> 6);
  if (item >= p.n_chunks * p.n_tiles) return;
  const int tile = item / p.n_chunks, chunk = item % p.n_chunks;
  const int b0 = chunk * TILES_CHUNK, b1 = min(b0 + TILES_CHUNK, p.n_groups);
  double s[NS];
#pragma unroll
  for (int c = 0; c < NS; ++c) s[c] = 0.0;
  const double* src = p.pdw + ((size_t)tile * p.n_edge * NS) * 64 + lane;
  for (int b = b0; b < b1; ++b)
#pragma unroll
    for (int c = 0; c < NS; ++c) s[c] += src[((size_t)b * NS + c) * 64];
  double* dst = p.pchunk + (((size_t)tile * p.n_chunks + chunk) * NS) * 64 + lane;
#pragma unroll
  for (int c = 0; c < NS; ++c) dst[c * 64] = s[c];
  uint32_t segs = 0;
  const uint16_t* mc = p.mcount + ((size_t)tile * p.n_edge) * 64 + lane;
  const int per = (p.n_edge + p.n_chunks - 1) / p.n_chunks;
  for (int b = chunk * per; b < min((chunk + 1) * per, p.n_edge); ++b) segs += mc[(size_t)b * 64];
  p.pseg[((size_t)tile * p.n_chunks + chunk) * 64 + lane] = segs;
}

constexpr int TILES_STATS_WAVES = 8;

template <int NS, bool KS>
__global__ __launch_bounds__(64 * TILES_STATS_WAVES) void tiles_stats_kernel(TileParams<NS> p, int it) {
  constexpr int NCNT = KS ? NS * NS : NS * (NS - 1);
  constexpr int DCOLS = NS + NCNT + (KS ? 1 : 0);
  constexpr int SW = TILES_STATS_WAVES;
  __shared__ double s_dw[SW][NS][64];
  __shared__ uint32_t s_ct[SW][NCNT][64];
  __shared__ uint32_t s_sg[SW][64];
  const int lane = threadIdx.x & 63;
  const int wave = threadIdx.x >> 6;
  const int tile = blockIdx.x;
  const int rep_local = tile * 64 + lane;
  const bool valid = rep_local < p.n_rep;
  {
    const int per = (p.n_chunks + SW - 1) / SW;
    const int c0 = min(wave * per, p.n_chunks), c1 = min(c0 + per, p.n_chunks);
    double part[NS];
#pragma unroll
    for (int c = 0; c < NS; ++c) part[c] = 0.0;
    const double* src = p.pchunk + ((size_t)tile * p.n_chunks * NS) * 64 + lane;
    uint32_t segs = 0;
    for (int ch = c0; ch < c1; ++ch) {
#pragma unroll
      for (int c = 0; c < NS; ++c) part[c] += src[((size_t)ch * NS + c) * 64];
      segs += p.pseg[((size_t)tile * p.n_chunks + ch) * 64 + lane];
    }
#pragma unroll
    for (int c = 0; c < NS; ++c) s_dw[wave][c][lane] = part[c];
    s_sg[wave][lane] = segs;
    uint32_t tot[NCNT];
#pragma unroll
    for (int c = 0; c < NCNT; ++c) tot[c] = 0u;
    for (int k = wave; k < p.cnt_copies; k += SW) {
      uint32_t* gc = p.cnt + (((size_t)tile * p.cnt_copies + k) * NS * NS) * 64 + lane;
#pragma unroll
      for (int c = 0; c < NCNT; ++c) { tot[c] += gc[c * 64]; gc[c * 64] = 0u; }
    }
#pragma unroll
    for (int c = 0; c < NCNT; ++c) s_ct[wave][c][lane] = tot[c];
  }
  __syncthreads();
  if (wave != 0) return;
  double col[DCOLS];
#pragma unroll
  for (int c = 0; c < NS; ++c) {
    double v = s_dw[0][c][lane];
#pragma unroll
    for (int w = 1; w < SW; ++w) v += s_dw[w][c][lane];
    col[c] = v;
  }
#pragma unroll
  for (int c = 0; c < NCNT; ++c) {
    uint32_t v = 0u;
#pragma unroll
    for (int w = 0; w < SW; ++w) v += s_ct[w][c][lane];
    col[NS + c] = (double)v;
  }
  {
    uint32_t segs = 0;
#pragma unroll
    for (int w = 0; w < SW; ++w) segs += s_sg[w][lane];
    if (!valid) segs = 0;
#pragma unroll
    for (int off = 32; off >= 1; off >>= 1) segs += __shfl_xor(segs, off, 64);
    if (lane == 0) { atomicAdd(p.segcnt, (unsigned long long)p.segprev[tile] + segs); p.segprev[tile] = segs; }
  }
  if (KS) col[NS + NCNT] = (double)p.nstate[((size_t)tile * p.n_node + p.root) * 64 + lane];
  if (p.reduce) {
    double* dst = p.stats + ((size_t)it * p.n_tiles + tile) * p.n_cols;
#pragma unroll
    for (int c = 0; c < DCOLS; ++c) {
      double v = valid ? col[c] : 0.0;
#pragma unroll
      for (int off = 32; off >= 1; off >>= 1) v += __shfl_xor(v, off, 64);
      if (lane == c) dst[c] = v;
    }
  } else {
#pragma unroll
    for (int c = 0; c < DCOLS; ++c) p.stats[((size_t)it * p.n_cols + c) * p.n_rep_pad + rep_local] = col[c];
  }
}

__global__ void tiles_init_kernel(int n_edge, int n_tiles, int64_t rows, const int32_t* __restrict__ slot,
                                  const int32_t* __restrict__ map_off, const double* __restrict__ maps,
                                  double* __restrict__ dw0, uint16_t* __restrict__ mcount) {
  const int lane = threadIdx.x & 63;
  const int item = blockIdx.x * (blockDim.x / 64) + (threadIdx.x >> 6);
  if (item >= n_edge * n_tiles) return;
  const int tile = item / n_edge, b = item % n_edge;
  const int o = map_off[b], m = map_off[b + 1] - o;
  double* dst = dw0 + ((size_t)tile * rows + slot[b]) * 64 + lane;
  for (int i = 0; i < m; ++i) dst[(size_t)i * 64] = maps[o + i];
  mcount[((size_t)tile * n_edge + b) * 64 + lane] = (uint16_t)m;
}

}

hipError_t launch_tiles_init(int n_edge, int n_tiles, int64_t rows, const int32_t* slot, const int32_t* map_off,
                             const double* maps, double* dw0, uint16_t* mcount, hipStream_t stream) {
  const int64_t items = (int64_t)n_edge * n_tiles;
  hipLaunchKernelGGL(tiles_init_kernel, dim3((unsigned)((items + 3) / 4)), dim3(256), 0, stream, n_edge, n_tiles, rows, slot, map_off,
                     maps, dw0, mcount);
  return hipGetLastError();
}

template <int NS>
hipError_t launch_tiles_sweep(const TileParams<NS>& p, const std::vector<int32_t>& up_off,
                              const std::vector<int32_t>& node_off, const std::vector<int32_t>& tier_off, int it, hipStream_t stream,
                              hipEvent_t* phase_ev, const McmcMapsLaunch* maps) {
  constexpr int WPB = TILES_BLOCK / 64;
  auto blocks = [&](int64_t items) { return dim3((unsigned)((items + WPB - 1) / WPB)); };
  auto pblocks = [&](int64_t items) { return dim3((unsigned)std::min<int64_t>((items + WPB - 1) / WPB, TILES_PERSISTENT_WGS)); };
  auto mark = [&](int i) { if (phase_ev) (void)hipEventRecord(phase_ev[i], stream); };
  mark(0);
  if (p.cl_nodes) {
    const int n_tiers = (int)tier_off.size() - 1;
    for (int t = 0; t < n_tiers; ++t) {
      const int n_cl = tier_off[t + 1] - tier_off[t];
      if (p.mstate) hipLaunchKernelGGL((tiles_up_cluster_kernel<NS, true>), dim3((unsigned)((int64_t)n_cl * p.n_tiles)), dim3(TILES_CL_BLOCK), 0, stream, p, tier_off[t], n_cl);
      else hipLaunchKernelGGL((tiles_up_cluster_kernel<NS, false>), dim3((unsigned)((int64_t)n_cl * p.n_tiles)), dim3(TILES_CL_BLOCK), 0, stream, p, tier_off[t], n_cl);
    }
    mark(1);
    for (int t = n_tiers - 1; t >= 0; --t) {
      const int n_cl = tier_off[t + 1] - tier_off[t];
      hipLaunchKernelGGL(tiles_down_cluster_kernel<NS>, dim3((unsigned)((int64_t)n_cl * p.n_tiles)), dim3(TILES_CL_BLOCK), 0, stream, p, it, tier_off[t], n_cl,
                         t == n_tiers - 1 ? 1 : 0);
    }
  } else {
    for (size_t l = 0; l + 1 < up_off.size(); ++l) {
      const int n = up_off[l + 1] - up_off[l];
      if (n > 0) hipLaunchKernelGGL(tiles_up_kernel<NS>, blocks((int64_t)n * p.n_tiles), dim3(TILES_BLOCK), 0, stream, p, up_off[l], up_off[l + 1]);
    }
    mark(1);
    hipLaunchKernelGGL(tiles_root_kernel<NS>, blocks(p.n_tiles), dim3(TILES_BLOCK), 0, stream, p, it);
    for (size_t l = 0; l + 1 < node_off.size(); ++l) {
      const int n = node_off[l + 1] - node_off[l];
      if (n > 0) hipLaunchKernelGGL(tiles_down_kernel<NS>, pblocks((int64_t)n * p.n_tiles), dim3(TILES_BLOCK), 0, stream, p, it, node_off[l], node_off[l + 1]);
    }
  }
  mark(2);
  if (maps) {
    const hipError_t me = launch_mcmc_maps_tiles<NS>(p, *maps, it, stream);
    if (me != hipSuccess) return me;
  }
  if (p.mstate) {
    if (p.ks) hipLaunchKernelGGL((tiles_branch_kernel<NS, true, true>), blocks((int64_t)p.n_groups * p.n_tiles), dim3(TILES_BLOCK), 0, stream, p, it);
    else hipLaunchKernelGGL((tiles_branch_kernel<NS, false, true>), blocks((int64_t)p.n_groups * p.n_tiles), dim3(TILES_BLOCK), 0, stream, p, it);
  } else {
    if (p.ks) hipLaunchKernelGGL((tiles_branch_kernel<NS, true, false>), blocks((int64_t)p.n_groups * p.n_tiles), dim3(TILES_BLOCK), 0, stream, p, it);
    else hipLaunchKernelGGL((tiles_branch_kernel<NS, false, false>), blocks((int64_t)p.n_groups * p.n_tiles), dim3(TILES_BLOCK), 0, stream, p, it);
  }
  mark(3);
  hipLaunchKernelGGL(tiles_chunk_kernel<NS>, blocks((int64_t)p.n_chunks * p.n_tiles), dim3(TILES_BLOCK), 0, stream, p);
  if (p.ks) hipLaunchKernelGGL((tiles_stats_kernel<NS, true>), dim3(p.n_tiles), dim3(64 * TILES_STATS_WAVES), 0, stream, p, it);
  else hipLaunchKernelGGL((tiles_stats_kernel<NS, false>), dim3(p.n_tiles), dim3(64 * TILES_STATS_WAVES), 0, stream, p, it);
  mark(4);
  return hipGetLastError();
}

template hipError_t launch_tiles_sweep<2>(const TileParams<2>&, const std::vector<int32_t>&, const std::vector<int32_t>&, const std::vector<int32_t>&, int, hipStream_t, hipEvent_t*,
                                              const McmcMapsLaunch*);
template hipError_t launch_tiles_sweep<3>(const TileParams<3>&, const std::vector<int32_t>&, const std::vector<int32_t>&, const std::vector<int32_t>&, int, hipStream_t, hipEvent_t*,
                                              const McmcMapsLaunch*);
template hipError_t launch_tiles_sweep<4>(const TileParams<4>&, const std::vector<int32_t>&, const std::vector<int32_t>&, const std::vector<int32_t>&, int, hipStream_t, hipEvent_t*,
                                              const McmcMapsLaunch*);

}
```

Baseline: 16.07 billion branch-site realisations/s.

## Split tiles sweep into replica-tile partitions on parallel streams; precompute group segment counts

The tiles sweep is split into up to a few partitions of replica tiles. Each partition runs its full per-iteration kernel chain on its own stream, forked from and joined back to the main stream, so that the serial level-by-level launches of one partition can overlap with another's and fill the GPU better. The branch kernel also writes per-group segment totals into a new buffer, and the chunk kernel sums those instead of rereading every per-branch mcount entry. This costs extra streams and events, more launches, and a little more memory, and partitioning is turned off when maps are active.

```diff
diff --git a/include/phylomap_hip.h b/include/phylomap_hip.h
--- a/include/phylomap_hip.h
+++ b/include/phylomap_hip.h
@@ -86,7 +86,8 @@
   int32_t q_timing;
   double  pade_pivot_min;
   int32_t expect_chunk;
-  int32_t reserved[3];
+  int32_t sweep_parts;
+  int32_t reserved[2];
 } phm_debug_options;
 
 typedef struct phm_info {
diff --git a/phylomap_amd/_lib.py b/phylomap_amd/_lib.py
--- a/phylomap_amd/_lib.py
+++ b/phylomap_amd/_lib.py
@@ -61,7 +61,8 @@
 class DebugOptions(C.Structure):
     _fields_ = [("pruning_form", C.c_int32), ("phase_timing", C.c_int32), ("fail_recovery", C.c_int32),
                 ("branch_group", C.c_int32), ("level_groups", C.c_int32), ("q_timing", C.c_int32),
-                ("pade_pivot_min", C.c_double), ("expect_chunk", C.c_int32), ("reserved", C.c_int32 * 3)]
+                ("pade_pivot_min", C.c_double), ("expect_chunk", C.c_int32), ("sweep_parts", C.c_int32),
+                ("reserved", C.c_int32 * 2)]
 
 
 class Info(C.Structure):
@@ -265,7 +266,7 @@
 
 
 _DEBUG_KEYS = ("pruning_form", "phase_timing", "fail_recovery", "branch_group", "level_groups", "q_timing", "pade_pivot_min",
-               "expect_chunk")
+               "expect_chunk", "sweep_parts")
 
 
 def make_options(seed=0, n_replicas=1, replica_offset=0, reduce=False, tips_per_replica=False, device=-1,
diff --git a/phylomap_amd/csrc/phm_engine.cpp b/phylomap_amd/csrc/phm_engine.cpp
--- a/phylomap_amd/csrc/phm_engine.cpp
+++ b/phylomap_amd/csrc/phm_engine.cpp
@@ -549,11 +549,14 @@
   return c;
 }
 
+int32_t tiles_branch_group(int tiles, int n_edge) { return (int32_t)std::max<int64_t>(1, std::min<int64_t>(16, (int64_t)tiles * n_edge / 65536)); }
+
 template <int NS>
 void fill_tile_params(phm_engine* e, phm::TileParams<NS>& p, const phm_options& o) {
   fill_common(e, o, p);
   p.klong = e->nw_klong;
-  p.group = (int32_t)std::max<int64_t>(1, std::min<int64_t>(16, (int64_t)e->tiles * p.n_edge / 65536));
+  p.tile0 = 0; p.tiles_part = e->tiles;
+  p.group = tiles_branch_group(e->tiles, p.n_edge);
   p.n_groups = (p.n_edge + p.group - 1) / p.group;
   p.n_chunks = (p.n_groups + phm::TILES_CHUNK - 1) / phm::TILES_CHUNK;
   p.rows = e->nw_total_cap;
@@ -569,7 +572,7 @@
   p.mstate = e->d_wt_mstate.p ? e->d_wt_mstate.as<uint8_t>() : nullptr;
   p.pdw = e->d_tl_pdw.as<double>(); p.pchunk = e->d_tl_pchunk.as<double>(); p.cnt = e->d_tl_cnt.as<uint32_t>();
   p.cnt_copies = tiles_cnt_copies(e->tiles);
-  p.pseg = e->d_tl_pseg.as<uint32_t>(); p.segprev = e->d_tl_segprev.as<uint32_t>();
+  p.pseg = e->d_tl_pseg.as<uint32_t>(); p.segprev = e->d_tl_segprev.as<uint32_t>(); p.gseg = e->d_tl_gseg.p ? e->d_tl_gseg.as<uint32_t>() : nullptr;
 }
 
 int32_t tile_slots(phm_engine* e, const SlotPlan& sp) {
@@ -603,7 +606,9 @@
   const size_t ms_bytes = long_paths ? (size_t)tiles * rows * 64 : 0;
   size_t free_b = 0, total_b = 0;
   HIPCHK(hipMemGetInfo(&free_b, &total_b));
-  const size_t need = 2 * dw_bytes + ms_bytes + pdw_bytes + pl_bytes + stats_bytes(e) + sizeof(double) * 3 * tab + (size_t)tiles * (4 * (size_t)E + Nn) * 64;
+  const int group = tiles_branch_group(tiles, E);
+  const size_t gseg_bytes = group > 1 ? sizeof(uint32_t) * (size_t)tiles * ((E + group - 1) / group) * 64 : 0;
+  const size_t need = 2 * dw_bytes + ms_bytes + pdw_bytes + gseg_bytes + pl_bytes + stats_bytes(e) + sizeof(double) * 3 * tab + (size_t)tiles * (4 * (size_t)E + Nn) * 64;
   if (int32_t st = check_hbm(need, free_b)) return st;
   HIPCHK(upload(e->d_up, s.up)); HIPCHK(upload(e->d_down, s.down));
   if (int32_t st = build_level_orders(e)) return st;
@@ -618,11 +623,12 @@
   HIPCHK(e->d_PL.alloc(pl_bytes));
   HIPCHK(e->d_nstate.alloc((size_t)tiles * Nn * 64));
   HIPCHK(e->d_tl_pdw.alloc(pdw_bytes));
+  if (gseg_bytes) HIPCHK(e->d_tl_gseg.alloc(gseg_bytes));
   HIPCHK(e->d_tl_pchunk.alloc(sizeof(double) * (size_t)tiles * n_chunks * n * 64));
   HIPCHK(e->d_tl_cnt.alloc(sizeof(uint32_t) * (size_t)tiles * tiles_cnt_copies(tiles) * n * n * 64));
   HIPCHK(e->d_tl_pseg.alloc(sizeof(uint32_t) * (size_t)tiles * n_chunks * 64)); HIPCHK(e->d_tl_segprev.alloc(sizeof(uint32_t) * tiles));
   if (int32_t st = alloc_stats(e)) return st;
-  e->bytes = (int64_t)(2 * dw_bytes + ms_bytes + pdw_bytes + pl_bytes + e->d_stats.bytes + e->d_red.bytes + e->d_mcount.bytes + e->d_tl_pchunk.bytes +
+  e->bytes = (int64_t)(2 * dw_bytes + ms_bytes + pdw_bytes + gseg_bytes + pl_bytes + e->d_stats.bytes + e->d_red.bytes + e->d_mcount.bytes + e->d_tl_pchunk.bytes +
                        sizeof(double) * 3 * tab);
   HIPCHK(hipMemset(e->d_nstate.p, 0, e->d_nstate.bytes));
   HIPCHK(hipMemset(e->d_tl_cnt.p, 0, e->d_tl_cnt.bytes));
@@ -1085,6 +1091,25 @@
   return PHM_OK;
 }
 
+constexpr int64_t TILES_RESIDENT_WAVES = 8 * 1024;
+constexpr int64_t TILES_PART_MIN_ROUNDS = 4;
+constexpr int TILES_AUTO_PARTS = 2;
+
+static int tiles_sweep_parts(const phm_engine* e, int n_iters) {
+  if (e->mapping != PHM_MAP_TILES || e->wide() || !e->nw_tier_off.empty() || n_iters <= 0) return 1;
+  if (e->maps.mode != phm::MAPS_OFF)
+    for (int it = e->iters_done; it < e->iters_done + n_iters; ++it)
+      if (it < (int)e->maps.j_of_iter.size() && e->maps.j_of_iter[it] >= 0) return 1;
+  int parts = e->dbg.sweep_parts;
+  if (parts <= 0) {
+    const int E = e->sched.n_edge;
+    const int g = tiles_branch_group(e->tiles, E);
+    const int64_t waves = (int64_t)e->tiles * ((E + g - 1) / g);
+    parts = (int)std::min<int64_t>(TILES_AUTO_PARTS, waves / (TILES_PART_MIN_ROUNDS * TILES_RESIDENT_WAVES));
+  }
+  return std::max(1, std::min({parts, (int)phm_engine::MAX_PARTS, e->tiles}));
+}
+
 extern "C" {
 
 int32_t phm_engine_run(phm_engine* e, int32_t n_iters, void* hip_stream) {
@@ -1108,12 +1133,46 @@
       small_n(e, [&](auto& p) { le = phm::launch_narrow_stats(p.br, e->iters_done + n_iters - 1, stream); });
     HIPCHK(le);
   } else if (e->mapping == PHM_MAP_TILES) {
+    const int parts = tiles_sweep_parts(e, n_iters);
+    const int level_launches = (int)(e->nw_up_off.size() + e->nw_down_off.size()) + 2;
     e->phase_iters = 0;
+    e->phase_parts = parts;
     if (e->phase_timing) {
-      while ((int)e->phase_ev.size() < 5 * n_iters) { hipEvent_t ev; HIPCHK(hipEventCreate(&ev)); e->phase_ev.push_back(ev); }
+      while ((int)e->phase_ev.size() < 5 * n_iters * parts) { hipEvent_t ev; HIPCHK(hipEventCreate(&ev)); e->phase_ev.push_back(ev); }
       e->phase_iters = n_iters;
     }
-    for (int i = 0; i < n_iters && le == hipSuccess; ++i) {
+    if (parts > 1) {
+      hipStream_t ps[phm_engine::MAX_PARTS] = {stream, nullptr, nullptr, nullptr};
+      for (int q = 1; q < parts; ++q) {
+        if (!e->part_join[q - 1]) HIPCHK(hipEventCreateWithFlags(&e->part_join[q - 1], hipEventDisableTiming));
+        if (!e->part_stream[q - 1]) HIPCHK(hipStreamCreateWithFlags(&e->part_stream[q - 1], hipStreamNonBlocking));
+        ps[q] = e->part_stream[q - 1];
+      }
+      int forked = 0;
+      hipError_t fe = hipSuccess;
+      for (int q = 1; q < parts && fe == hipSuccess; ++q) { fe = hipStreamWaitEvent(ps[q], e->ev0, 0); if (fe == hipSuccess) forked = q; }
+      le = fe;
+      const int base = e->tiles / parts, extra = e->tiles % parts;
+      for (int i = 0; i < n_iters && le == hipSuccess; ++i) {
+        const int it = e->iters_done + i;
+        for (int q = 0, t0 = 0; q < parts && le == hipSuccess; ++q) {
+          const int nt = base + (q < extra ? 1 : 0);
+          hipEvent_t* pev = e->phase_timing ? &e->phase_ev[5 * ((size_t)q * n_iters + i)] : nullptr;
+          small_n(e, [&](auto& p) {
+            auto part = p.tl;
+            part.tile0 = t0; part.tiles_part = nt;
+            le = phm::launch_tiles_sweep(part, e->nw_up_off, e->nw_node_off, e->nw_tier_off, it, ps[q], pev, nullptr);
+          });
+          launches += level_launches;
+          t0 += nt;
+        }
+      }
+      for (int q = 1; q <= forked; ++q) {
+        hipError_t je = hipEventRecord(e->part_join[q - 1], ps[q]);
+        if (je == hipSuccess) je = hipStreamWaitEvent(stream, e->part_join[q - 1], 0);
+        if (le == hipSuccess) le = je;
+      }
+    } else for (int i = 0; i < n_iters && le == hipSuccess; ++i) {
       const int it = e->iters_done + i;
       hipEvent_t* pev = e->phase_timing ? &e->phase_ev[5 * (size_t)i] : nullptr;
       phm::McmcMapsLaunch ml;
@@ -1127,8 +1186,7 @@
       if (clusters && e->wide())
         launches += (e->pwt.band_up > 0 && !e->wt_sparse.kernel ? tiers : (int)e->nw_up_off.size() - 1) + tiers + 4;
       else
-        launches += clusters ? 2 * tiers + 3
-                             : (int)(e->nw_up_off.size() + e->nw_down_off.size()) + 2;
+        launches += clusters ? 2 * tiers + 3 : level_launches;
     }
     HIPCHK(le);
   } else {
@@ -1203,7 +1261,7 @@
     e->last_ms = ms;
     e->timing_pending = false;
     for (double& v : e->phase_ms) v = 0.0;
-    for (int i = 0; i < e->phase_iters; ++i)
+    for (int i = 0; i < e->phase_iters * e->phase_parts; ++i)
       for (int ph = 0; ph < 4; ++ph) {
         float pm = 0.f;
         HIPCHK(hipEventElapsedTime(&pm, e->phase_ev[5 * (size_t)i + ph], e->phase_ev[5 * (size_t)i + ph + 1]));
diff --git a/phylomap_amd/csrc/phm_internal.h b/phylomap_amd/csrc/phm_internal.h
--- a/phylomap_amd/csrc/phm_internal.h
+++ b/phylomap_amd/csrc/phm_internal.h
@@ -331,7 +331,17 @@
   DevBuf d_wb_cnt;
   phm::WideBranchParams pwb;
   std::vector<int32_t> tl_slot;
-  DevBuf d_tl_slot, d_tl_pdw, d_tl_pchunk, d_tl_cnt, d_tl_estate, d_tl_pseg, d_tl_segprev;
+  DevBuf d_tl_slot, d_tl_pdw, d_tl_pchunk, d_tl_cnt, d_tl_estate, d_tl_pseg, d_tl_segprev, d_tl_gseg;
+  static constexpr int MAX_PARTS = 4;
+  hipStream_t part_stream[MAX_PARTS - 1] = {nullptr, nullptr, nullptr};
+  hipEvent_t part_join[MAX_PARTS - 1] = {nullptr, nullptr, nullptr};
+  int phase_parts = 1;
+  void release_parts() {
+    for (int i = 0; i < MAX_PARTS - 1; ++i) {
+      if (part_stream[i]) { (void)hipStreamDestroy(part_stream[i]); part_stream[i] = nullptr; }
+      if (part_join[i]) { (void)hipEventDestroy(part_join[i]); part_join[i] = nullptr; }
+    }
+  }
   phm::WtParams pwt;
   DevBuf d_wt_dwfx, d_wt_segacc, d_wt_B2, d_wt_totL, d_wt_pair_slot, d_wt_slot_col, d_wt_B2band, d_wt_mstate, d_wt_dwfx_tile, d_wt_cnt_tile;
   phm::WtBand wt_band;
@@ -364,11 +374,13 @@
                      &d_nw_up_order, &d_nw_down_order, &d_nw_node_order, &d_nw_border, &d_nw_off, &d_nw_colL, &d_nw_rowL, &d_nw_maskL, &d_nw_mcount,
                      &d_nw_dwA, &d_nw_dwB, &d_nw_mstate, &d_nw_mlen, &d_nw_estate, &d_nw_part, &d_nw_rowbuf, &d_nw_down_lv, &d_nw_dmap, &d_nw_dmap_edge, &d_nw_walk_off, &d_nw_edge_parent, &d_nw_cl_nodes, &d_nw_cl_item_off, &d_nw_cl_lvl_ptr, &d_nw_cl_lvl_off, &d_ell_col, &d_ell_val,
                      &d_ell2_col, &d_ell2_val, &d_wb_cnt, &d_tl_slot, &d_tl_pdw, &d_tl_pchunk, &d_tl_cnt, &d_tl_estate, &d_tl_pseg,
-                     &d_tl_segprev, &d_wt_dwfx, &d_wt_segacc, &d_wt_B2, &d_wt_totL, &d_wt_pair_slot, &d_wt_slot_col, &d_wt_B2band, &d_wt_mstate, &d_wt_dwfx_tile, &d_wt_cnt_tile, &d_wt_coef};
+                     &d_tl_segprev, &d_tl_gseg, &d_wt_dwfx, &d_wt_segacc, &d_wt_B2, &d_wt_totL, &d_wt_pair_slot, &d_wt_slot_col, &d_wt_B2band, &d_wt_mstate, &d_wt_dwfx_tile, &d_wt_cnt_tile, &d_wt_coef};
     for (DevBuf* b : all) b->reset();
+    release_parts();
   }
   ~phm_engine() {
     delete fwd;
+    release_parts();
     if (ev0) (void)hipEventDestroy(ev0);
     if (ev1) (void)hipEventDestroy(ev1);
     for (hipEvent_t ev : phase_ev) (void)hipEventDestroy(ev);
diff --git a/phylomap_amd/csrc/phm_tiles.h b/phylomap_amd/csrc/phm_tiles.h
--- a/phylomap_amd/csrc/phm_tiles.h
+++ b/phylomap_amd/csrc/phm_tiles.h
@@ -29,6 +29,7 @@
   int32_t klong;
   int32_t group, n_groups;
   int32_t n_chunks;
+  int32_t tile0, tiles_part;
   uint32_t seed_lo, seed_hi;
   int64_t rows;
   double B2[NS * NS], Bc[NS * NS], scale[NS], pid[NS];
@@ -51,6 +52,7 @@
   double* PL;
   uint8_t* nstate;
   double* pdw;
+  uint32_t* gseg;
   double* pchunk;
   uint32_t* cnt;
   int32_t cnt_copies;
diff --git a/phylomap_amd/csrc/phm_tiles.hip b/phylomap_amd/csrc/phm_tiles.hip
--- a/phylomap_amd/csrc/phm_tiles.hip
+++ b/phylomap_amd/csrc/phm_tiles.hip
@@ -99,8 +99,8 @@
   const uint32_t lane = threadIdx.x & 63;
   const int item = blockIdx.x * (TILES_BLOCK / 64) + __builtin_amdgcn_readfirstlane(threadIdx.x >> 6);
   const int n_lvl = end - begin;
-  if (item >= n_lvl * p.n_tiles) return;
-  const int tile = item / n_lvl;
+  if (item >= n_lvl * p.tiles_part) return;
+  const int tile = p.tile0 + item / n_lvl;
   const UpStep st = p.up[p.up_order[begin + item % n_lvl]];
   uint32_t err = 0;
   up_item<NS>(p, tile, st, lane, err);
@@ -169,8 +169,9 @@
 template <int NS>
 __global__ __launch_bounds__(TILES_BLOCK) void tiles_root_kernel(TileParams<NS> p, int it) {
   const int lane = threadIdx.x & 63;
-  const int tile = blockIdx.x * (TILES_BLOCK / 64) + __builtin_amdgcn_readfirstlane(threadIdx.x >> 6);
-  if (tile >= p.n_tiles) return;
+  const int t = blockIdx.x * (TILES_BLOCK / 64) + __builtin_amdgcn_readfirstlane(threadIdx.x >> 6);
+  if (t >= p.tiles_part) return;
+  const int tile = p.tile0 + t;
   uint32_t err = 0;
   draw_root<NS>(p, tile, it, lane, err);
   if (err) atomicOr(p.err, err);
@@ -257,7 +258,7 @@
 
 template <int NS>
 __device__ __forceinline__ void node_record(const TileParams<NS>& p, NodeLoads<NS>& d, int item, int n_lvl, int begin) {
-  d.tile = item / n_lvl;
+  d.tile = p.tile0 + item / n_lvl;
   const int32_t* rec = reinterpret_cast<const int32_t*>(p.up + sched_word(p.node_order, begin + item % n_lvl));
   static_assert(sizeof(UpStep) == 5 * sizeof(int32_t), "UpStep: parent, two children, two edges");
   d.st.parent = sched_word(rec, 0);
@@ -333,7 +334,7 @@
 __global__ __launch_bounds__(TILES_BLOCK) void tiles_down_kernel(TileParams<NS> p, int it, int begin, int end) {
   const uint32_t lane = threadIdx.x & 63;
   const int n_lvl = end - begin;
-  const int n_items = n_lvl * p.n_tiles;
+  const int n_items = n_lvl * p.tiles_part;
   const int stride = gridDim.x * (TILES_BLOCK / 64);
   const bool draw_tips = p.ks && p.tip_masks;
   uint32_t err = 0;
@@ -390,9 +391,9 @@
   if (threadIdx.x < NS * NS) s_B2[threadIdx.x] = p.B2[threadIdx.x];
   if (threadIdx.x < NS) s_scale[threadIdx.x] = p.scale[threadIdx.x];
   __syncthreads();
-  if (item >= p.n_groups * p.n_tiles) return;
-  const int tile = item % p.n_tiles;
-  const int grp = item / p.n_tiles;
+  if (item >= p.n_groups * p.tiles_part) return;
+  const int tile = p.tile0 + item % p.tiles_part;
+  const int grp = item / p.tiles_part;
   double* s_dw = s_dw_all + wave * NS * 64;
   uint16_t* s_cnt = s_cnt_all + wave * NCNT * 64;
   const uint32_t rep = (uint32_t)(p.replica_offset + tile * 64 + lane);
@@ -411,6 +412,7 @@
     }
   };
   uint32_t pending = 0;
+  uint32_t held = 0;
   const int q1 = min((grp + 1) * p.group, p.n_edge);
   for (int q = grp * p.group; q < q1; ++q) {
   const int b = p.branch_order[q];
@@ -605,8 +607,10 @@
   if (mnew > cap) mnew = cap;
   if (mnew > 65535) { err |= DERR_CAPACITY; mnew = 65535; }
   mct[b * 64 + lane] = (uint16_t)mnew;
+  held += (uint32_t)mnew;
   }
   flush_counts();
+  if (p.group > 1) p.gseg[((size_t)tile * p.n_groups + grp) * 64 + lane] = held;
 
   double* pd = p.pdw + (((size_t)tile * p.n_edge + grp) * NS) * 64 + lane;
 #pragma unroll
@@ -618,23 +622,32 @@
 __global__ __launch_bounds__(TILES_BLOCK) void tiles_chunk_kernel(TileParams<NS> p) {
   const int lane = threadIdx.x & 63;
   const int item = blockIdx.x * (TILES_BLOCK / 64) + __builtin_amdgcn_readfirstlane(threadIdx.x >> 6);
-  if (item >= p.n_chunks * p.n_tiles) return;
-  const int tile = item / p.n_chunks, chunk = item % p.n_chunks;
+  if (item >= p.n_chunks * p.tiles_part) return;
+  const int tile = p.tile0 + item / p.n_chunks, chunk = item % p.n_chunks;
   const int b0 = chunk * TILES_CHUNK, b1 = min(b0 + TILES_CHUNK, p.n_groups);
   double s[NS];
 #pragma unroll
   for (int c = 0; c < NS; ++c) s[c] = 0.0;
   const double* src = p.pdw + ((size_t)tile * p.n_edge * NS) * 64 + lane;
-  for (int b = b0; b < b1; ++b)
-#pragma unroll
-    for (int c = 0; c < NS; ++c) s[c] += src[((size_t)b * NS + c) * 64];
+  uint32_t segs = 0;
+  if (p.group > 1) {
+    const uint32_t* gs = p.gseg + ((size_t)tile * p.n_groups) * 64 + lane;
+    for (int b = b0; b < b1; ++b) {
+#pragma unroll
+      for (int c = 0; c < NS; ++c) s[c] += src[((size_t)b * NS + c) * 64];
+      segs += gs[(size_t)b * 64];
+    }
+  } else {
+    for (int b = b0; b < b1; ++b)
+#pragma unroll
+      for (int c = 0; c < NS; ++c) s[c] += src[((size_t)b * NS + c) * 64];
+    const uint16_t* mc = p.mcount + ((size_t)tile * p.n_edge) * 64 + lane;
+    const int per = (p.n_edge + p.n_chunks - 1) / p.n_chunks;
+    for (int b = chunk * per; b < min((chunk + 1) * per, p.n_edge); ++b) segs += mc[(size_t)b * 64];
+  }
   double* dst = p.pchunk + (((size_t)tile * p.n_chunks + chunk) * NS) * 64 + lane;
 #pragma unroll
   for (int c = 0; c < NS; ++c) dst[c * 64] = s[c];
-  uint32_t segs = 0;
-  const uint16_t* mc = p.mcount + ((size_t)tile * p.n_edge) * 64 + lane;
-  const int per = (p.n_edge + p.n_chunks - 1) / p.n_chunks;
-  for (int b = chunk * per; b < min((chunk + 1) * per, p.n_edge); ++b) segs += mc[(size_t)b * 64];
   p.pseg[((size_t)tile * p.n_chunks + chunk) * 64 + lane] = segs;
 }
 
@@ -650,7 +663,7 @@
   __shared__ uint32_t s_sg[SW][64];
   const int lane = threadIdx.x & 63;
   const int wave = threadIdx.x >> 6;
-  const int tile = blockIdx.x;
+  const int tile = p.tile0 + blockIdx.x;
   const int rep_local = tile * 64 + lane;
   const bool valid = rep_local < p.n_rep;
   {
@@ -770,13 +783,13 @@
   } else {
     for (size_t l = 0; l + 1 < up_off.size(); ++l) {
       const int n = up_off[l + 1] - up_off[l];
-      if (n > 0) hipLaunchKernelGGL(tiles_up_kernel<NS>, blocks((int64_t)n * p.n_tiles), dim3(TILES_BLOCK), 0, stream, p, up_off[l], up_off[l + 1]);
+      if (n > 0) hipLaunchKernelGGL(tiles_up_kernel<NS>, blocks((int64_t)n * p.tiles_part), dim3(TILES_BLOCK), 0, stream, p, up_off[l], up_off[l + 1]);
     }
     mark(1);
-    hipLaunchKernelGGL(tiles_root_kernel<NS>, blocks(p.n_tiles), dim3(TILES_BLOCK), 0, stream, p, it);
+    hipLaunchKernelGGL(tiles_root_kernel<NS>, blocks(p.tiles_part), dim3(TILES_BLOCK), 0, stream, p, it);
     for (size_t l = 0; l + 1 < node_off.size(); ++l) {
       const int n = node_off[l + 1] - node_off[l];
-      if (n > 0) hipLaunchKernelGGL(tiles_down_kernel<NS>, pblocks((int64_t)n * p.n_tiles), dim3(TILES_BLOCK), 0, stream, p, it, node_off[l], node_off[l + 1]);
+      if (n > 0) hipLaunchKernelGGL(tiles_down_kernel<NS>, pblocks((int64_t)n * p.tiles_part), dim3(TILES_BLOCK), 0, stream, p, it, node_off[l], node_off[l + 1]);
     }
   }
   mark(2);
@@ -785,16 +798,16 @@
     if (me != hipSuccess) return me;
   }
   if (p.mstate) {
-    if (p.ks) hipLaunchKernelGGL((tiles_branch_kernel<NS, true, true>), blocks((int64_t)p.n_groups * p.n_tiles), dim3(TILES_BLOCK), 0, stream, p, it);
-    else hipLaunchKernelGGL((tiles_branch_kernel<NS, false, true>), blocks((int64_t)p.n_groups * p.n_tiles), dim3(TILES_BLOCK), 0, stream, p, it);
+    if (p.ks) hipLaunchKernelGGL((tiles_branch_kernel<NS, true, true>), blocks((int64_t)p.n_groups * p.tiles_part), dim3(TILES_BLOCK), 0, stream, p, it);
+    else hipLaunchKernelGGL((tiles_branch_kernel<NS, false, true>), blocks((int64_t)p.n_groups * p.tiles_part), dim3(TILES_BLOCK), 0, stream, p, it);
   } else {
-    if (p.ks) hipLaunchKernelGGL((tiles_branch_kernel<NS, true, false>), blocks((int64_t)p.n_groups * p.n_tiles), dim3(TILES_BLOCK), 0, stream, p, it);
-    else hipLaunchKernelGGL((tiles_branch_kernel<NS, false, false>), blocks((int64_t)p.n_groups * p.n_tiles), dim3(TILES_BLOCK), 0, stream, p, it);
+    if (p.ks) hipLaunchKernelGGL((tiles_branch_kernel<NS, true, false>), blocks((int64_t)p.n_groups * p.tiles_part), dim3(TILES_BLOCK), 0, stream, p, it);
+    else hipLaunchKernelGGL((tiles_branch_kernel<NS, false, false>), blocks((int64_t)p.n_groups * p.tiles_part), dim3(TILES_BLOCK), 0, stream, p, it);
   }
   mark(3);
-  hipLaunchKernelGGL(tiles_chunk_kernel<NS>, blocks((int64_t)p.n_chunks * p.n_tiles), dim3(TILES_BLOCK), 0, stream, p);
-  if (p.ks) hipLaunchKernelGGL((tiles_stats_kernel<NS, true>), dim3(p.n_tiles), dim3(64 * TILES_STATS_WAVES), 0, stream, p, it);
-  else hipLaunchKernelGGL((tiles_stats_kernel<NS, false>), dim3(p.n_tiles), dim3(64 * TILES_STATS_WAVES), 0, stream, p, it);
+  hipLaunchKernelGGL(tiles_chunk_kernel<NS>, blocks((int64_t)p.n_chunks * p.tiles_part), dim3(TILES_BLOCK), 0, stream, p);
+  if (p.ks) hipLaunchKernelGGL((tiles_stats_kernel<NS, true>), dim3(p.tiles_part), dim3(64 * TILES_STATS_WAVES), 0, stream, p, it);
+  else hipLaunchKernelGGL((tiles_stats_kernel<NS, false>), dim3(p.tiles_part), dim3(64 * TILES_STATS_WAVES), 0, stream, p, it);
   mark(4);
   return hipGetLastError();
 }
```

Measured after the change: 16.84 billion branch-site realisations/s, median of 6. 4.8% higher.
